# Sreyan88/audio-ssl

Hardware: AMD Instinct MI355X
Metric: upstream clips/sec (1s@16kHz, 64-mel) (higher is better)
Workload: dtype bf16; 1 GPU; delores-m upstream step (log-mel + 2 views + q/k conv encoders + MoCo + 3 Barlow heads + bwd + SGD), 1 s @ 16 kHz, 64 mel, batch 512/GPU, queue 65536; global_batch=512, parallelism=dp1

## Files before the change

### audio-ssl_amd/csrc/bnpool.hip

```cpp
#include "common.h"

namespace {

template <typename T_, bool SQ>
__global__ __launch_bounds__(256) void colstats_kernel(const T_* __restrict__ x, long M, int C, long ld, int rows_per_block,
                                                       double* __restrict__ sum, double* __restrict__ sumsq) {
    __shared__ float red[256][17];
    const int cg = threadIdx.x & 7, r0 = threadIdx.x >> 3;
    const int col0 = blockIdx.y * 64 + cg * 8;
    const long row_begin = (long)blockIdx.x * rows_per_block;
    const long row_end = min(M, row_begin + rows_per_block);
    x += (long)blockIdx.z * M * ld;
    sum += (long)blockIdx.z * C;
    if (SQ) sumsq += (long)blockIdx.z * C;
    float s[8], q[8];
#pragma unroll
    for (int i = 0; i < 8; ++i) { s[i] = 0.f; q[i] = 0.f; }
    if (col0 < C)
        for (long r = row_begin + r0; r < row_end; r += 32) {
            const Vec8<T_> v = Vec8<T_>::load(x + r * ld + col0);
#pragma unroll
            for (int i = 0; i < 8; ++i) { const float f = v.get(i); s[i] += f; if (SQ) q[i] += f * f; }
        }
#pragma unroll
    for (int i = 0; i < 8; ++i) { red[threadIdx.x][i] = s[i]; red[threadIdx.x][8 + i] = q[i]; }
    __syncthreads();
    if (threadIdx.x < 128) {
        const int g = threadIdx.x >> 4, k = threadIdx.x & 15;
        if (SQ || k < 8) {
            double t = 0.0;
            for (int r = 0; r < 32; ++r) t += (double)red[r * 8 + g][k];
            const int c = blockIdx.y * 64 + g * 8 + (k & 7);
            if (c < C) {
                if (k < 8) atomicAdd(&sum[c], t);
                else       atomicAdd(&sumsq[c], t);
            }
        }
    }
}

__global__ void bn_finalize_kernel(const double* __restrict__ sum, const double* __restrict__ sumsq, int groups, double count,
                                   int C, const float* __restrict__ gamma, const float* __restrict__ beta, float* running_mean,
                                   float* running_var, float momentum, float eps, float* scale, float* shift,
                                   float* save_mean, float* save_rstd) {
    const int c = blockIdx.x * blockDim.x + threadIdx.x;
    if (c >= C) return;
    const double g = gamma ? (double)gamma[c] : 1.0, b = beta ? (double)beta[c] : 0.0;
    float rm = running_mean ? running_mean[c] : 0.f, rv = running_mean ? running_var[c] : 0.f;
    for (int k = 0; k < groups; ++k) {
        const int o = k * C + c;
        const double mean = sum[o] / count;
        double var = sumsq[o] / count - mean * mean;
        var = var < 0.0 ? 0.0 : var;
        const double rstd = 1.0 / sqrt(var + (double)eps);
        scale[o] = (float)(g * rstd);
        shift[o] = (float)(b - mean * g * rstd);
        save_mean[o] = (float)mean;
        save_rstd[o] = (float)rstd;
        rm = (1.f - momentum) * rm + momentum * (float)mean;
        const double unb = count > 1.0 ? var * count / (count - 1.0) : var;
        rv = (1.f - momentum) * rv + momentum * (float)unb;
    }
    if (running_mean) { running_mean[c] = rm; running_var[c] = rv; }
}

template <typename TY, typename T_>
__global__ __launch_bounds__(256) void bn_relu_pool_fwd_kernel(const TY* __restrict__ Y, const float* __restrict__ scale,
                                                               const float* __restrict__ shift, T_* __restrict__ P,
                                                               int N, int Ti, int Fi) {
    const int To = Ti / 2, Fo = Fi / 2;
    const long total = (long)N * To * Fo * 8;
    const long idx = (long)blockIdx.x * 256 + threadIdx.x;
    if (idx >= total) return;
    const int c8 = (int)(idx & 7);
    long r = idx >> 3;
    const int fo = (int)(r % Fo); r /= Fo;
    const int to = (int)(r % To);
    const int n = (int)(r / To);
    float sc[8], sh[8], m[8];
#pragma unroll
    for (int i = 0; i < 8; ++i) { sc[i] = scale[c8 * 8 + i]; sh[i] = shift[c8 * 8 + i]; m[i] = 0.f; }
#pragma unroll
    for (int df = 0; df < 2; ++df)
#pragma unroll
        for (int dt = 0; dt < 2; ++dt) {
            const Vec8<TY> v = Vec8<TY>::load(Y + ((((long)n * Ti + 2 * to + dt) * Fi + 2 * fo + df) * 64 + c8 * 8));
#pragma unroll
            for (int i = 0; i < 8; ++i) m[i] = fmaxf(m[i], sc[i] * v.get(i) + sh[i]);
        }
    Vec8<T_> o;
#pragma unroll
    for (int i = 0; i < 8; ++i) o.set(i, m[i]);
    o.store(P + idx * 8);
}

template <typename TY, typename T_>
__global__ __launch_bounds__(256) void bn_relu_pool_train_fwd_kernel(const TY* __restrict__ Y, const double* __restrict__ sum,
                                                                     const double* __restrict__ sumsq, int stat_rep, double count,
                                                                     const float* __restrict__ gamma, const float* __restrict__ beta,
                                                                     float* running_mean, float* running_var, float momentum, float eps,
                                                                     T_* __restrict__ P, float* __restrict__ scale,
                                                                     float* __restrict__ shift, float* __restrict__ save_mean,
                                                                     float* __restrict__ save_rstd, int N, int Ti, int Fi) {
    __shared__ float sc_s[64], sh_s[64];
    if (threadIdx.x < 64) {
        const int c = threadIdx.x;
        const double g = (double)gamma[c], b = (double)beta[c];
        double s1 = 0.0, s2 = 0.0;
        for (int r = 0; r < stat_rep; ++r) { s1 += sum[r * 128 + c]; s2 += sumsq[r * 128 + c]; }
        const double mean = s1 / count;
        double var = s2 / count - mean * mean;
        var = var < 0.0 ? 0.0 : var;
        const double rstd = 1.0 / sqrt(var + (double)eps);
        const float sc = (float)(g * rstd), sh = (float)(b - mean * g * rstd);
        sc_s[c] = sc; sh_s[c] = sh;
        if (blockIdx.x == 0) {
            scale[c] = sc; shift[c] = sh; save_mean[c] = (float)mean; save_rstd[c] = (float)rstd;
            if (running_mean) {
                running_mean[c] = (1.f - momentum) * running_mean[c] + momentum * (float)mean;
                const double unb = count > 1.0 ? var * count / (count - 1.0) : var;
                running_var[c] = (1.f - momentum) * running_var[c] + momentum * (float)unb;
            }
        }
    }
    __syncthreads();
    const int To = Ti / 2, Fo = Fi / 2;
    const long total = (long)N * To * Fo * 8;
    const long idx = (long)blockIdx.x * 256 + threadIdx.x;
    if (idx >= total) return;
    const int c8 = (int)(idx & 7);
    long r = idx >> 3;
    const int fo = (int)(r % Fo); r /= Fo;
    const int to = (int)(r % To);
    const int n = (int)(r / To);
    float sc[8], sh[8], m[8];
#pragma unroll
    for (int i = 0; i < 8; ++i) { sc[i] = sc_s[c8 * 8 + i]; sh[i] = sh_s[c8 * 8 + i]; m[i] = 0.f; }
#pragma unroll
    for (int df = 0; df < 2; ++df)
#pragma unroll
        for (int dt = 0; dt < 2; ++dt) {
            const Vec8<TY> v = Vec8<TY>::load(Y + ((((long)n * Ti + 2 * to + dt) * Fi + 2 * fo + df) * 64 + c8 * 8));
#pragma unroll
            for (int i = 0; i < 8; ++i) m[i] = fmaxf(m[i], sc[i] * v.get(i) + sh[i]);
        }
    Vec8<T_> o;
#pragma unroll
    for (int i = 0; i < 8; ++i) o.set(i, m[i]);
    o.store(P + idx * 8);
}

template <typename T_, typename TO>
__device__ __forceinline__ void tmean_body(const T_* __restrict__ P, TO* __restrict__ xl, int N, int To, int Fo);

template <typename T_, typename TO>
__global__ __launch_bounds__(256) void tmean_fwd_kernel(const T_* __restrict__ P, TO* __restrict__ xl, int N, int To, int Fo) {
    tmean_body<T_, TO>(P, xl, N, To, Fo);
}
struct Tmean3 { const void* P[3]; void* xl[3]; int To[3], Fo[3]; const float* parts; };
template <typename T_, typename TO>
__global__ __launch_bounds__(256) void tmean3_fwd_kernel(Tmean3 a, int N) {
    const int l = blockIdx.z;
    if ((int)blockIdx.x * 64 >= a.Fo[l] * 8) return;
    if (!a.P[l]) {
        if (a.parts && l == 0) {
            const long row = (long)a.Fo[0] * 64, tot = (long)N * row;
            const long i = (long)blockIdx.y * row + blockIdx.x * 512 + threadIdx.x * 2;
            if (blockIdx.x * 512 + threadIdx.x * 2 < row) {
                float2 s = *reinterpret_cast<const float2*>(a.parts + i);
#pragma unroll
                for (int k = 1; k < 4; ++k) {
                    const float2 v = *reinterpret_cast<const float2*>(a.parts + k * tot + i);
                    s.x += v.x; s.y += v.y;
                }
                *reinterpret_cast<float2*>(static_cast<float*>(a.xl[0]) + i) = s;
            }
        }
        return;
    }
    tmean_body<T_, TO>(static_cast<const T_*>(a.P[l]), static_cast<TO*>(a.xl[l]), N, a.To[l], a.Fo[l]);
}

template <typename T_, typename TO>
__device__ __forceinline__ void tmean_body(const T_* __restrict__ P, TO* __restrict__ xl, int N, int To, int Fo) {
    __shared__ float red[4][64][9];
    const int lane = threadIdx.x & 63, w = threadIdx.x >> 6;
    const int nv = Fo * 8;
    const int v = blockIdx.x * 64 + lane;
    const int n = blockIdx.y;
    const bool live = v < nv;
    float s[8];
#pragma unroll
    for (int i = 0; i < 8; ++i) s[i] = 0.f;
    if (live) {
        const T_* p = P + ((long)n * To * nv + v) * 8;
#pragma unroll 4
        for (int t = w; t < To; t += 4) {
            const Vec8<T_> x = Vec8<T_>::load(p + (long)t * nv * 8);
#pragma unroll
            for (int i = 0; i < 8; ++i) s[i] += x.get(i);
        }
    }
#pragma unroll
    for (int i = 0; i < 8; ++i) red[w][lane][i] = s[i];
    __syncthreads();
    if (w == 0 && live) {
        Vec8<TO> o;
        const float inv = 1.f / (float)To;
#pragma unroll
        for (int i = 0; i < 8; ++i) o.set(i, (red[0][lane][i] + red[1][lane][i] + red[2][lane][i] + red[3][lane][i]) * inv);
        o.store(xl + ((long)n * nv + v) * 8);
    }
}

template <typename TY, bool APPLY, typename TG, typename T_>
__global__ __launch_bounds__(256) void bn_relu_pool_bwd_kernel(const TY* __restrict__ Y, const TG* __restrict__ dP,
                                                               const TG* __restrict__ dxl, float inv_To,
                                                               const float* __restrict__ scale, const float* __restrict__ shift,
                                                               const float* __restrict__ mean, const float* __restrict__ rstd,
                                                               float* __restrict__ stat, float inv_count,
                                                               T_* __restrict__ dY, int N, int Ti, int Fi, int fold,
                                                               float* dgamma, float* dbeta) {
    __shared__ float red[256][16];
    __shared__ float folded[128];
    if (APPLY && fold) {
        if (threadIdx.x < 128) {
            float t = 0.f;
            for (int r = 0; r < 32; ++r) t += stat[128 + r * 128 + threadIdx.x];
            folded[threadIdx.x] = t;
        }
        __syncthreads();
        if (blockIdx.x == 0 && threadIdx.x < 64 && dgamma) {
            dbeta[threadIdx.x] += folded[threadIdx.x];
            dgamma[threadIdx.x] += folded[64 + threadIdx.x];
        }
    }
    const int To = Ti / 2, Fo = Fi / 2;
    const int Tq = (Ti + 1) / 2;
    const long total = (long)N * Tq * Fo * 8;
    const long idx = (long)blockIdx.x * 256 + threadIdx.x;
    const bool live = idx < total;
    float db[8], dg[8];
#pragma unroll
    for (int i = 0; i < 8; ++i) { db[i] = 0.f; dg[i] = 0.f; }
    if (live) {
        const int c8 = (int)(idx & 7);
        long r = idx >> 3;
        const int fo = (int)(r % Fo); r /= Fo;
        const int tq = (int)(r % Tq);
        const int n = (int)(r / Tq);
        const bool pooled = tq < To;
        float sc[8], sh[8], mu[8], rs[8], g[8], cb[8], cg[8];
#pragma unroll
        for (int i = 0; i < 8; ++i) {
            const int c = c8 * 8 + i;
            sc[i] = scale[c]; sh[i] = shift[c]; mu[i] = mean[c]; rs[i] = rstd[c]; g[i] = 0.f;
            if (APPLY) { cb[i] = (fold ? folded[c] : stat[c]) * inv_count; cg[i] = (fold ? folded[64 + c] : stat[64 + c]) * inv_count; }
        }
        if (pooled) {
            const Vec8<TG> gp = Vec8<TG>::load(dP + ((((long)n * To + tq) * Fo + fo) * 64 + c8 * 8));
#pragma unroll
            for (int i = 0; i < 8; ++i) g[i] = gp.get(i);
            if (dxl) {
                const Vec8<TG> gx = Vec8<TG>::load(dxl + ((long)n * Fo * 64 + fo * 64 + c8 * 8));
#pragma unroll
                for (int i = 0; i < 8; ++i) g[i] += gx.get(i) * inv_To;
            }
        }
        Vec8<TY> y[4];
        int best[8];
        float bm[8];
#pragma unroll
        for (int i = 0; i < 8; ++i) { best[i] = 0; bm[i] = 0.f; }
#pragma unroll
        for (int p = 0; p < 4; ++p) {
            const int df = p >> 1, dt = p & 1;
            const int t = 2 * tq + dt;
            if (t < Ti) y[p] = Vec8<TY>::load(Y + ((((long)n * Ti + t) * Fi + 2 * fo + df) * 64 + c8 * 8));
            else y[p] = Vec8<TY>::zero();
#pragma unroll
            for (int i = 0; i < 8; ++i) {
                const float a = sc[i] * y[p].get(i) + sh[i];
                if (p == 0 || a > bm[i]) { bm[i] = a; best[i] = p; }
            }
        }
#pragma unroll
        for (int i = 0; i < 8; ++i) {
            const float da = (pooled && bm[i] > 0.f) ? g[i] : 0.f;
            g[i] = da;
            if (!APPLY) {
                float yb = y[0].get(i);
#pragma unroll
                for (int p = 1; p < 4; ++p) yb = best[i] == p ? y[p].get(i) : yb;
                db[i] = da;
                dg[i] = da * (yb - mu[i]) * rs[i];
            }
        }
        if (APPLY) {
#pragma unroll
            for (int p = 0; p < 4; ++p) {
                const int df = p >> 1, dt = p & 1;
                const int t = 2 * tq + dt;
                if (t >= Ti) continue;
                Vec8<T_> o;
#pragma unroll
                for (int i = 0; i < 8; ++i) {
                    const float xhat = (y[p].get(i) - mu[i]) * rs[i];
                    const float da = best[i] == p ? g[i] : 0.f;
                    o.set(i, sc[i] * (da - cb[i] - xhat * cg[i]));
                }
                o.store(dY + ((((long)n * Ti + t) * Fi + 2 * fo + df) * 64 + c8 * 8));
            }
        }
    }
    if (!APPLY) {
#pragma unroll
        for (int i = 0; i < 8; ++i) { red[threadIdx.x][i] = db[i]; red[threadIdx.x][8 + i] = dg[i]; }
        __syncthreads();
        if (threadIdx.x < 128) {
            const int kind = threadIdx.x >> 6, c = threadIdx.x & 63;
            float t = 0.f;
            for (int r = (c >> 3); r < 256; r += 8) t += red[r][kind * 8 + (c & 7)];
            atomicAdd(&stat[128 + (blockIdx.x & 31) * 128 + kind * 64 + c], t);
        }
    }
}

template <typename TP, typename TG>
__global__ __launch_bounds__(256) void bn_pool_bwd_stats_p_kernel(const TP* __restrict__ P, const TG* __restrict__ dP,
                                                                  const TG* __restrict__ dxl, float inv_To,
                                                                  const float* __restrict__ scale, const float* __restrict__ shift,
                                                                  const float* __restrict__ mean, const float* __restrict__ rstd,
                                                                  float* __restrict__ stat, int N, int To, int Fo) {
    __shared__ float red[256][16];
    const long total = (long)N * To * Fo * 8;
    float db[8], dg[8];
#pragma unroll
    for (int i = 0; i < 8; ++i) { db[i] = 0.f; dg[i] = 0.f; }
    const int c8 = threadIdx.x & 7;
    float k1[8], k0[8];
#pragma unroll
    for (int i = 0; i < 8; ++i) {
        const int c = c8 * 8 + i;
        const float sc = scale[c], inv = sc != 0.f ? 1.f / sc : 0.f;
        k1[i] = inv * rstd[c];
        k0[i] = sc != 0.f ? -(shift[c] * inv + mean[c]) * rstd[c] : 0.f;
    }
    for (long idx = (long)blockIdx.x * 256 + threadIdx.x; idx < total; idx += (long)gridDim.x * 256) {
        const long pos = idx >> 3;
        const Vec8<TP> pv = Vec8<TP>::load(P + pos * 64 + c8 * 8);
        const Vec8<TG> gp = Vec8<TG>::load(dP + pos * 64 + c8 * 8);
        float g[8];
#pragma unroll
        for (int i = 0; i < 8; ++i) g[i] = gp.get(i);
        if (dxl) {
            const long n = pos / ((long)To * Fo);
            const int fo = (int)(pos % Fo);
            const Vec8<TG> gx = Vec8<TG>::load(dxl + (n * Fo + fo) * 64 + c8 * 8);
#pragma unroll
            for (int i = 0; i < 8; ++i) g[i] += gx.get(i) * inv_To;
        }
#pragma unroll
        for (int i = 0; i < 8; ++i) {
            const float a = pv.get(i);
            const float da = a > 0.f ? g[i] : 0.f;
            db[i] += da;
            dg[i] += da * (a * k1[i] + k0[i]);
        }
    }
#pragma unroll
    for (int i = 0; i < 8; ++i) { red[threadIdx.x][i] = db[i]; red[threadIdx.x][8 + i] = dg[i]; }
    __syncthreads();
    if (threadIdx.x < 128) {
        const int kind = threadIdx.x >> 6, c = threadIdx.x & 63;
        float t = 0.f;
        for (int r = (c >> 3); r < 256; r += 8) t += red[r][kind * 8 + (c & 7)];
        atomicAdd(&stat[128 + (blockIdx.x & 31) * 128 + kind * 64 + c], t);
    }
}

__global__ void stat_reduce_kernel(float* stat) {
    const int i = threadIdx.x;
    if (i >= 128) return;
    float t = 0.f;
    for (int r = 0; r < 32; ++r) t += stat[128 + r * 128 + i];
    stat[i] = t;
}

template <typename T_>
__global__ __launch_bounds__(256) void im2col_kernel(const T_* __restrict__ X, T_* __restrict__ col, int N, int Ti, int Fi) {
    const long total = (long)N * Ti * Fi * 72;
    const long idx = (long)blockIdx.x * 256 + threadIdx.x;
    if (idx >= total) return;
    const int k8 = (int)(idx % 72);
    long pix = idx / 72;
    const int tap = k8 >> 3, c8 = k8 & 7;
    const int f = (int)(pix % Fi);
    const long r = pix / Fi;
    const int t = (int)(r % Ti);
    const long n = r / Ti;
    const int ff = f + tap / 3 - 1, tt = t + tap % 3 - 1;
    Vec8<T_> v = Vec8<T_>::zero();
    if (ff >= 0 && ff < Fi && tt >= 0 && tt < Ti) v = Vec8<T_>::load(X + (((n * Ti + tt) * Fi + ff) * 64 + c8 * 8));
    v.store(col + idx * 8);
}

template <typename T_>
__global__ void pack_conv_w_kernel(const float* __restrict__ W, T_* __restrict__ Wf, T_* __restrict__ Wd) {
    const int idx = blockIdx.x * 256 + threadIdx.x;
    if (idx >= 64 * 576) return;
    const int row = idx / 576, k = idx % 576, tap = k / 64, c = k % 64;
    Wf[idx] = from_f32<T_>(W[(row * 64 + c) * 9 + tap]);
    Wd[idx] = from_f32<T_>(W[(c * 64 + row) * 9 + (8 - tap)]);
}

template <typename T_>
__global__ void pack_conv_w2_kernel(const float* __restrict__ Wa, T_* __restrict__ Wfa, T_* __restrict__ Wda,
                                    const float* __restrict__ Wb, T_* __restrict__ Wfb, T_* __restrict__ Wdb) {
    const int idx = blockIdx.x * 256 + threadIdx.x;
    if (idx >= 64 * 576) return;
    const float* W = blockIdx.y ? Wb : Wa;
    T_* Wf = blockIdx.y ? Wfb : Wfa;
    T_* Wd = blockIdx.y ? Wdb : Wda;
    const int row = idx / 576, k = idx % 576, tap = k / 64, c = k % 64;
    Wf[idx] = from_f32<T_>(W[(row * 64 + c) * 9 + tap]);
    Wd[idx] = from_f32<T_>(W[(c * 64 + row) * 9 + (8 - tap)]);
}

__global__ void unpack_conv_dw_kernel(const float* __restrict__ dWp, float* __restrict__ dW) {
    const int idx = blockIdx.x * 256 + threadIdx.x;
    if (idx >= 64 * 576) return;
    const int co = idx / 576, k = idx % 576, tap = k / 64, ci = k % 64;
    dW[(co * 64 + ci) * 9 + tap] += dWp[idx];
}

}

#define DISPATCH_T(dtype, CALL_F32, CALL_BF16) do { if ((dtype) == 0) { CALL_F32; } else { CALL_BF16; } } while (0)

extern "C" int audiossl_colstats(int dtype, const void* x, int groups, long M, int C, long ld, int want_sq, double* sum,
                                 double* sumsq, void* stream) {
    ASSL_REQUIRE(x && sum && groups > 0 && M > 0 && C > 0 && (C % 8) == 0 && (ld % 8) == 0);
    ASSL_REQUIRE((dtype == 0 || dtype == 1) && (!want_sq || sumsq));
    hipStream_t s = static_cast<hipStream_t>(stream);
    const size_t nb = sizeof(double) * C * groups;
    if (want_sq && sumsq == sum + (size_t)C * groups) {
        ASSL_ZERO(sum, 2 * nb, s);
    } else {
        ASSL_ZERO(sum, nb, s);
        if (want_sq) ASSL_ZERO(sumsq, nb, s);
    }
    const int slabs = (C + 63) / 64;
    long it = (M * slabs * groups + 32L * 2048 - 1) / (32L * 2048);
    it = it < 1 ? 1 : (it > 128 ? 128 : it);
    const int rpb = 32 * (int)it;
    const dim3 grid(ceil_div(M, rpb), slabs, groups);
#define CS(TT, SQ) hipLaunchKernelGGL((colstats_kernel<TT, SQ>), grid, dim3(256), 0, s, static_cast<const TT*>(x), M, C, ld, rpb, sum, sumsq)
    if (dtype == 0) { if (want_sq) CS(float, true); else CS(float, false); }
    else            { if (want_sq) CS(bf16, true);  else CS(bf16, false); }
#undef CS
    ASSL_LAUNCH_CHECK();
}

extern "C" int audiossl_bn_finalize(const double* sum, const double* sumsq, int groups, double count, int C,
                                    const float* gamma, const float* beta, float* running_mean, float* running_var,
                                    float momentum, float eps, float* scale, float* shift, float* save_mean, float* save_rstd,
                                    void* stream) {
    ASSL_REQUIRE(sum && sumsq && scale && shift && save_mean && save_rstd && C > 0 && count > 0 && groups > 0);
    hipLaunchKernelGGL(bn_finalize_kernel, dim3(ceil_div(C, 256)), dim3(256), 0, static_cast<hipStream_t>(stream), sum, sumsq,
                       groups, count, C, gamma, beta, running_mean, running_var, momentum, eps, scale, shift, save_mean, save_rstd);
    ASSL_LAUNCH_CHECK();
}

extern "C" int audiossl_bn_relu_pool_fwd(int dtype, int ydtype, const void* Y, const float* scale, const float* shift, void* P,
                                         int N, int Ti, int Fi, void* stream) {
    ASSL_REQUIRE(Y && scale && shift && P && N > 0 && Ti >= 2 && Fi >= 2 && (Fi % 2) == 0 && (dtype == 0 || dtype == 1));
    ASSL_REQUIRE(ydtype == 0 || ydtype == dtype);
    const long total = (long)N * (Ti / 2) * (Fi / 2) * 8;
    hipStream_t s = static_cast<hipStream_t>(stream);
#define PF(TY, TO) hipLaunchKernelGGL((bn_relu_pool_fwd_kernel<TY, TO>), dim3(ceil_div(total, 256)), dim3(256), 0, s, \
        static_cast<const TY*>(Y), scale, shift, static_cast<TO*>(P), N, Ti, Fi)
    if (dtype == 0) PF(float, float); else if (ydtype == 0) PF(float, bf16); else PF(bf16, bf16);
#undef PF
    ASSL_LAUNCH_CHECK();
}

extern "C" int audiossl_bn_relu_pool_train_fwd(int dtype, int ydtype, const void* Y, const double* sum, const double* sumsq,
                                               int stat_replicas, double count,
                                               const float* gamma, const float* beta, float* running_mean, float* running_var,
                                               float momentum, float eps, void* P, float* scale, float* shift, float* save_mean,
                                               float* save_rstd, int N, int Ti, int Fi, void* stream) {
    ASSL_REQUIRE(Y && sum && sumsq && gamma && beta && P && scale && shift && save_mean && save_rstd && count > 0.0);
    ASSL_REQUIRE(stat_replicas >= 1 && (stat_replicas == 1 || sumsq == sum + 64));
    ASSL_REQUIRE(N > 0 && Ti >= 2 && Fi >= 2 && (Fi % 2) == 0 && (dtype == 0 || dtype == 1) && (ydtype == 0 || ydtype == dtype));
    const long total = (long)N * (Ti / 2) * (Fi / 2) * 8;
    hipStream_t s = static_cast<hipStream_t>(stream);
#define PF(TY, TO) hipLaunchKernelGGL((bn_relu_pool_train_fwd_kernel<TY, TO>), dim3(ceil_div(total, 256)), dim3(256), 0, s,          \
        static_cast<const TY*>(Y), sum, sumsq, stat_replicas, count, gamma, beta, running_mean, running_var, momentum, eps,      \
        static_cast<TO*>(P),                                                                                                      \
        scale, shift, save_mean, save_rstd, N, Ti, Fi)
    if (dtype == 0) PF(float, float); else if (ydtype == 0) PF(float, bf16); else PF(bf16, bf16);
#undef PF
    ASSL_LAUNCH_CHECK();
}

extern "C" int audiossl_tmean_fwd(int dtype, int out_f32, const void* P, void* xl, int N, int To, int Fo, void* stream) {
    ASSL_REQUIRE(P && xl && N > 0 && To > 0 && Fo > 0 && (dtype == 0 || dtype == 1));
    hipStream_t s = static_cast<hipStream_t>(stream);
#define TM(TI, TO_) hipLaunchKernelGGL((tmean_fwd_kernel<TI, TO_>), dim3(ceil_div(Fo * 8, 64), N), dim3(256), 0, s, \
        static_cast<const TI*>(P), static_cast<TO_*>(xl), N, To, Fo)
    if (dtype == 0) TM(float, float); else if (out_f32) TM(bf16, float); else TM(bf16, bf16);
#undef TM
    ASSL_LAUNCH_CHECK();
}

extern "C" int audiossl_tmean3_fwd(int dtype, int out_f32, const void* P1, void* x1, const float* x1_parts, int To1, int Fo1,
                                   const void* P2, void* x2, int To2, int Fo2, const void* P3, void* x3, int To3, int Fo3, int N,
                                   void* stream) {
    ASSL_REQUIRE(x1 && P2 && x2 && P3 && x3 && N > 0 && To1 > 0 && To2 > 0 && To3 > 0 && Fo1 > 0 && Fo2 > 0 && Fo3 > 0);
    ASSL_REQUIRE((P1 != nullptr) != (x1_parts != nullptr) && (!x1_parts || (out_f32 && dtype == 1)));
    ASSL_REQUIRE(dtype == 0 || dtype == 1);
    hipStream_t s = static_cast<hipStream_t>(stream);
    Tmean3 a{{P1, P2, P3}, {x1, x2, x3}, {To1, To2, To3}, {Fo1, Fo2, Fo3}, x1_parts};
    const int gx = ceil_div(max(Fo1, max(Fo2, Fo3)) * 8, 64);
#define TM3(TI, TO_) hipLaunchKernelGGL((tmean3_fwd_kernel<TI, TO_>), dim3(gx, N, 3), dim3(256), 0, s, a, N)
    if (dtype == 0) TM3(float, float); else if (out_f32) TM3(bf16, float); else TM3(bf16, bf16);
#undef TM3
    ASSL_LAUNCH_CHECK();
}

namespace {
__global__ void add_stat_kernel(const float* __restrict__ stat, float* dgamma, float* dbeta) {
    const int c = threadIdx.x;
    if (c < 64) { dbeta[c] += stat[c]; dgamma[c] += stat[64 + c]; }
}
}

static int bn_relu_pool_bwd_run(int phase, int dtype, int ydtype, int gdtype, const void* Y, const void* P, const void* dP, const void* dxl,
                                const float* scale, const float* shift, const float* mean, const float* rstd, float* stat,
                                const float* gstat, double count, void* dY, float* dgamma, float* dbeta, int N, int Ti, int Fi,
                                void* stream) {
    ASSL_REQUIRE(Y && dP && scale && shift && mean && rstd && stat);
    ASSL_REQUIRE(N > 0 && Ti >= 2 && Fi >= 2 && (Fi % 2) == 0 && (dtype == 0 || dtype == 1) && (gdtype == 0 || gdtype == dtype));
    ASSL_REQUIRE(ydtype == 0 || ydtype == dtype);
    ASSL_REQUIRE(phase == 1 || (dY && dgamma && dbeta));
    hipStream_t s = static_cast<hipStream_t>(stream);
    if (phase != 2) ASSL_ZERO(stat, sizeof(float) * 128 * 33, s);
    const long total = (long)N * ((Ti + 1) / 2) * (Fi / 2) * 8;
    const int grid = ceil_div(total, 256);
    const float inv_To = 1.f / (float)(Ti / 2);
    const float inv_count = (float)(1.0 / (phase == 2 ? count : (double)N * Ti * Fi));
    float* apply_stat = phase == 2 ? const_cast<float*>(gstat) : stat;
    const int fold = phase == 0;
#define BW(TY, AP, TG, TO, ST) hipLaunchKernelGGL((bn_relu_pool_bwd_kernel<TY, AP, TG, TO>), dim3(grid), dim3(256), 0, s,              \
        static_cast<const TY*>(Y), static_cast<const TG*>(dP), static_cast<const TG*>(dxl), inv_To, scale, shift, mean, rstd, ST, \
        inv_count, static_cast<TO*>(dY), N, Ti, Fi, (AP) ? fold : 0, dgamma, dbeta)
#define BWP(TG, TO) hipLaunchKernelGGL((bn_pool_bwd_stats_p_kernel<TO, TG>), dim3(pgrid), dim3(256), 0, s, static_cast<const TO*>(P),          \
        static_cast<const TG*>(dP), static_cast<const TG*>(dxl), inv_To, scale, shift, mean, rstd, stat, N, Ti / 2, Fi / 2)
#define BW2(TY, TG, TO) do { if (phase != 2) { if (P) BWP(TG, TO); else BW(TY, false, TG, TO, stat);                                       \
                                               if (!fold) hipLaunchKernelGGL(stat_reduce_kernel, dim3(1), dim3(128), 0, s, stat); }          \
                             if (phase != 1) BW(TY, true, TG, TO, apply_stat); } while (0)
    const long ptotal = (long)N * (Ti / 2) * (Fi / 2) * 8;
    const int pgrid = (int)min((long)2048, (ptotal + 255) / 256);
    if (dtype == 0) BW2(float, float, float);
    else if (ydtype == 0 && gdtype == 0) BW2(float, float, bf16);
    else if (ydtype == 0) BW2(float, bf16, bf16);
    else if (gdtype == 0) BW2(bf16, float, bf16);
    else BW2(bf16, bf16, bf16);
#undef BW2
#undef BWP
#undef BW
    if (phase == 2) hipLaunchKernelGGL(add_stat_kernel, dim3(1), dim3(64), 0, s, stat, dgamma, dbeta);
    ASSL_LAUNCH_CHECK();
}

extern "C" int audiossl_bn_relu_pool_bwd(int dtype, int ydtype, int gdtype, const void* Y, const void* dP, const void* dxl, const float* scale,
                                         const float* shift, const float* mean, const float* rstd, float* stat, void* dY,
                                         float* dgamma, float* dbeta, int N, int Ti, int Fi, void* stream) {
    return bn_relu_pool_bwd_run(0, dtype, ydtype, gdtype, Y, nullptr, dP, dxl, scale, shift, mean, rstd, stat, nullptr, 0.0, dY, dgamma, dbeta, N,
                                Ti, Fi, stream);
}
extern "C" int audiossl_bn_relu_pool_bwd_p(int dtype, int ydtype, int gdtype, const void* Y, const void* P, const void* dP, const void* dxl,
                                           const float* scale, const float* shift, const float* mean, const float* rstd, float* stat,
                                           void* dY, float* dgamma, float* dbeta, int N, int Ti, int Fi, void* stream) {
    ASSL_REQUIRE(P);
    return bn_relu_pool_bwd_run(0, dtype, ydtype, gdtype, Y, P, dP, dxl, scale, shift, mean, rstd, stat, nullptr, 0.0, dY, dgamma, dbeta, N,
                                Ti, Fi, stream);
}
extern "C" int audiossl_bn_relu_pool_bwd_stats(int dtype, int ydtype, int gdtype, const void* Y, const void* dP, const void* dxl,
                                               const float* scale, const float* shift, const float* mean, const float* rstd,
                                               float* stat, int N, int Ti, int Fi, void* stream) {
    return bn_relu_pool_bwd_run(1, dtype, ydtype, gdtype, Y, nullptr, dP, dxl, scale, shift, mean, rstd, stat, nullptr, 0.0, nullptr, nullptr,
                                nullptr, N, Ti, Fi, stream);
}
extern "C" int audiossl_bn_relu_pool_bwd_apply(int dtype, int ydtype, int gdtype, const void* Y, const void* dP, const void* dxl,
                                               const float* scale, const float* shift, const float* mean, const float* rstd,
                                               float* stat, const float* gstat, double count_global, void* dY, float* dgamma,
                                               float* dbeta, int N, int Ti, int Fi, void* stream) {
    ASSL_REQUIRE(gstat && count_global > 1.0);
    return bn_relu_pool_bwd_run(2, dtype, ydtype, gdtype, Y, nullptr, dP, dxl, scale, shift, mean, rstd, stat, gstat, count_global, dY, dgamma,
                                dbeta, N, Ti, Fi, stream);
}

extern "C" int audiossl_im2col3x3(int dtype, const void* X, void* col, int N, int Ti, int Fi, void* stream) {
    ASSL_REQUIRE(X && col && N > 0 && Ti > 0 && Fi > 0 && (dtype == 0 || dtype == 1));
    const long total = (long)N * Ti * Fi * 72;
    ASSL_REQUIRE((total + 255) / 256 < 2147483647L);
    hipStream_t s = static_cast<hipStream_t>(stream);
    DISPATCH_T(dtype,
        hipLaunchKernelGGL(im2col_kernel<float>, dim3(ceil_div(total, 256)), dim3(256), 0, s, static_cast<const float*>(X),
                           static_cast<float*>(col), N, Ti, Fi),
        hipLaunchKernelGGL(im2col_kernel<bf16>, dim3(ceil_div(total, 256)), dim3(256), 0, s, static_cast<const bf16*>(X),
                           static_cast<bf16*>(col), N, Ti, Fi));
    ASSL_LAUNCH_CHECK();
}

extern "C" int audiossl_pack_conv_w(int dtype, const float* W, void* Wf, void* Wd, void* stream) {
    ASSL_REQUIRE(W && Wf && Wd && (dtype == 0 || dtype == 1));
    hipStream_t s = static_cast<hipStream_t>(stream);
    DISPATCH_T(dtype,
        hipLaunchKernelGGL(pack_conv_w_kernel<float>, dim3(144), dim3(256), 0, s, W, static_cast<float*>(Wf), static_cast<float*>(Wd)),
        hipLaunchKernelGGL(pack_conv_w_kernel<bf16>, dim3(144), dim3(256), 0, s, W, static_cast<bf16*>(Wf), static_cast<bf16*>(Wd)));
    ASSL_LAUNCH_CHECK();
}

extern "C" int audiossl_pack_conv_w2(int dtype, const float* Wa, void* Wfa, void* Wda, const float* Wb, void* Wfb, void* Wdb, void* stream) {
    ASSL_REQUIRE(Wa && Wfa && Wda && Wb && Wfb && Wdb && (dtype == 0 || dtype == 1));
    hipStream_t s = static_cast<hipStream_t>(stream);
    DISPATCH_T(dtype,
        hipLaunchKernelGGL(pack_conv_w2_kernel<float>, dim3(144, 2), dim3(256), 0, s, Wa, static_cast<float*>(Wfa), static_cast<float*>(Wda),
                           Wb, static_cast<float*>(Wfb), static_cast<float*>(Wdb)),
        hipLaunchKernelGGL(pack_conv_w2_kernel<bf16>, dim3(144, 2), dim3(256), 0, s, Wa, static_cast<bf16*>(Wfa), static_cast<bf16*>(Wda),
                           Wb, static_cast<bf16*>(Wfb), static_cast<bf16*>(Wdb)));
    ASSL_LAUNCH_CHECK();
}

extern "C" int audiossl_unpack_conv_dw(const float* dWp, float* dW, void* stream) {
    ASSL_REQUIRE(dWp && dW);
    hipLaunchKernelGGL(unpack_conv_dw_kernel, dim3(144), dim3(256), 0, static_cast<hipStream_t>(stream), dWp, dW);
    ASSL_LAUNCH_CHECK();
}
```

### audio-ssl_amd/csrc/conv.hip

```cpp
#include <cstdlib>
#include "common.h"

namespace {

constexpr int CH = 64, KTOT = 576;
constexpr int WPITCH = KTOT + 8;
constexpr int PIXP = 72;
constexpr int PIXW = 96;

typedef __attribute__((address_space(3))) bf16x4* lds4_t;

struct ConvArgs {
    const bf16* X; const bf16* W; const float* bias; bf16* Y; double* sum; double* sumsq;
    int Ti, rows_total, tiles, out_f32, dbg, stat_rep;
};

template <int FI, int PITCH, int NTH = 256>
struct Halo {
    static constexpr int TT = 256 / FI;
    static constexpr int COLS = FI + 2;
    static constexpr int ELEMS = (TT + 2) * COLS * PITCH;
    static constexpr int NV = ((TT + 2) * FI * 8 + NTH - 1) / NTH;
    static constexpr int NVEC = (TT + 2) * FI * 8;
    Vec8<bf16> r[NV];
    __device__ __forceinline__ void load(const bf16* __restrict__ X, int g0, int rows_total) {
#pragma unroll
        for (int i = 0; i < NV; ++i) {
            const int v = threadIdx.x + i * NTH;
            const int row = v / (FI * 8), rem = v % (FI * 8);
            const int gr = g0 - 1 + row;
            r[i] = (v < NVEC && gr >= 0 && gr < rows_total) ? Vec8<bf16>::load(X + ((long)gr * FI) * CH + rem * 8) : Vec8<bf16>::zero();
        }
    }
    __device__ __forceinline__ void put(bf16* lds) const {
#pragma unroll
        for (int i = 0; i < NV; ++i) {
            const int v = threadIdx.x + i * NTH;
            const int row = v / (FI * 8), rem = v % (FI * 8);
            if (v < NVEC) r[i].store(lds + (row * COLS + (rem >> 3) + 1) * PITCH + (rem & 7) * 8);
        }
    }
    __device__ __forceinline__ static void zero_border(bf16* lds) {
        for (int i = threadIdx.x; i < (TT + 2) * 2 * 8; i += NTH) {
            const int row = i / 16, side = (i >> 3) & 1, c8 = i & 7;
            Vec8<bf16>::zero().store(lds + (row * COLS + side * (FI + 1)) * PITCH + c8 * 8);
        }
    }
};

template <int FI, int NW>
__global__ __launch_bounds__(64 * NW, 1) void conv3x3_kernel(ConvArgs a) {
    using H = Halo<FI, PIXP, 64 * NW>;
    constexpr int RT = 8 / NW;
    constexpr int TT = H::TT, COLS = H::COLS;
    extern __shared__ __attribute__((aligned(16))) char smem[];
    bf16* const wl = reinterpret_cast<bf16*>(smem);
    bf16* const hl = wl + CH * WPITCH;
    float* const red = reinterpret_cast<float*>(hl);

    const int lane = threadIdx.x & 63, wave = threadIdx.x >> 6;
    const int m = lane & 31, h = lane >> 5;
    for (int v = threadIdx.x; v < CH * KTOT / 8; v += 64 * NW) {
        const int row = v / (KTOT / 8), c = v % (KTOT / 8);
        Vec8<bf16>::load(a.W + row * KTOT + c * 8).store(wl + row * WPITCH + c * 8);
    }
    H::zero_border(hl);

    float ssum[2][16], ssq[2][16];
#pragma unroll
    for (int j = 0; j < 2; ++j)
#pragma unroll
        for (int r = 0; r < 16; ++r) { ssum[j][r] = 0.f; ssq[j][r] = 0.f; }
    f32x4 bias4[2][4];
#pragma unroll
    for (int j = 0; j < 2; ++j)
#pragma unroll
        for (int q = 0; q < 4; ++q)
            bias4[j][q] = a.bias ? *reinterpret_cast<const f32x4*>(a.bias + j * 32 + 8 * q + 4 * h) : f32x4{0.f, 0.f, 0.f, 0.f};
    H halo;
    int tile = blockIdx.x;
    if (tile < a.tiles) { halo.load(a.X, tile * TT, a.rows_total); halo.put(hl); }
    __syncthreads();

    for (; tile < a.tiles; tile += gridDim.x) {
        const int g0 = tile * TT;
        const int next = tile + gridDim.x;
        if (next < a.tiles && !(a.dbg & 2)) halo.load(a.X, next * TT, a.rows_total);

        int tl[RT], fcol[RT];
        bool ok[RT][3];
#pragma unroll
        for (int i = 0; i < RT; ++i) {
            const int rt = RT * wave + i;
            tl[i] = FI == 32 ? rt : 2 * rt + (m >> 4);
            fcol[i] = FI == 32 ? m : (m & 15);
            const int g = g0 + tl[i];
            const int ti = g % a.Ti;
#pragma unroll
            for (int dt = 0; dt < 3; ++dt) ok[i][dt] = g < a.rows_total && ti + dt - 1 >= 0 && ti + dt - 1 < a.Ti;
        }
        f32x16 acc[RT][2];
#pragma unroll
        for (int i = 0; i < RT; ++i)
#pragma unroll
            for (int j = 0; j < 2; ++j)
#pragma unroll
                for (int r = 0; r < 16; ++r) acc[i][j][r] = 0.f;

        if (!(a.dbg & 4))
#pragma unroll
        for (int tap = 0; tap < 9; ++tap) {
            const int dt = tap % 3, df = tap / 3;
#pragma unroll
            for (int cc = 0; cc < 4; ++cc) {
                Vec8<bf16> fa[RT], fb[2];
#pragma unroll
                for (int i = 0; i < RT; ++i) {
                    const bf16* p = hl + ((tl[i] + dt) * COLS + fcol[i] + df) * PIXP + cc * 16 + 8 * h;
                    fa[i] = ok[i][dt] ? Vec8<bf16>::load(p) : Vec8<bf16>::zero();
                }
#pragma unroll
                for (int j = 0; j < 2; ++j) fb[j] = Vec8<bf16>::load(wl + (j * 32 + m) * WPITCH + tap * 64 + cc * 16 + 8 * h);
#pragma unroll
                for (int i = 0; i < RT; ++i)
#pragma unroll
                    for (int j = 0; j < 2; ++j)
                        acc[i][j] = __builtin_amdgcn_mfma_f32_32x32x16_bf16(fb[j].v, fa[i].v, acc[i][j], 0, 0, 0);
            }
        }
#pragma unroll
        for (int i = 0; i < RT; ++i) {
            const int g = g0 + tl[i];
            if (g < a.rows_total && !(a.dbg & 1)) {
                const long o = ((long)g * FI + fcol[i]) * CH;
#pragma unroll
                for (int j = 0; j < 2; ++j)
#pragma unroll
                    for (int q = 0; q < 4; ++q) {
                        f32x4 v;
#pragma unroll
                        for (int e = 0; e < 4; ++e) {
                            v[e] = acc[i][j][4 * q + e] + bias4[j][q][e];
                            ssum[j][4 * q + e] += v[e];
                            ssq[j][4 * q + e] += v[e] * v[e];
                        }
                        const int co = j * 32 + 8 * q + 4 * h;
                        if (a.out_f32) *reinterpret_cast<f32x4*>(reinterpret_cast<float*>(a.Y) + o + co) = v;
                        else *reinterpret_cast<bf16x4*>(a.Y + o + co) = bf16x4{(bf16)v[0], (bf16)v[1], (bf16)v[2], (bf16)v[3]};
                    }
            }
        }
        __syncthreads();
        if (next < a.tiles) halo.put(hl);
        __syncthreads();
    }
    if (a.sum) {
#pragma unroll
        for (int j = 0; j < 2; ++j)
#pragma unroll
            for (int r = 0; r < 16; ++r) {
                float s = ssum[j][r], q = ssq[j][r];
#pragma unroll
                for (int o = 16; o > 0; o >>= 1) { s += __shfl_xor(s, o, 64); q += __shfl_xor(q, o, 64); }
                if (m == 0) {
                    const int co = j * 32 + (r & 3) + 8 * (r >> 2) + 4 * h;
                    red[(wave * 64 + co) * 2] = s; red[(wave * 64 + co) * 2 + 1] = q;
                }
            }
        __syncthreads();
        if (threadIdx.x < 128) {
            const int c = threadIdx.x >> 1, k = threadIdx.x & 1;
            double t = 0.0;
#pragma unroll
            for (int w = 0; w < NW; ++w) t += (double)red[(w * 64 + c) * 2 + k];
            const int rep = (blockIdx.x % a.stat_rep) * 128;
            atomicAdd(k == 0 ? &a.sum[rep + c] : &a.sumsq[rep + c], t);
        }
    }
}

template <int FI>
struct WsGeom {
    static constexpr int TT = 256 / FI, COLS = FI + 2, ROWS = TT + 2, SEGS = FI / 8;
    static constexpr int UNITS = ROWS * SEGS;
    static constexpr int UPW = (UNITS + 3) / 4;
    static constexpr int BYTES = ROWS * COLS * 128;
};

template <int FI, bool STATS, bool F32OUT, int PF = 2>
__global__ __launch_bounds__(256, 1) void conv3x3_ws_kernel(ConvArgs a) {
    using G = WsGeom<FI>;
    constexpr int TT = G::TT, COLS = G::COLS;
    typedef __attribute__((address_space(3))) void* lptr_t;
    extern __shared__ __attribute__((aligned(16))) char smem[];
    float* const biasl = reinterpret_cast<float*>(smem + 2 * G::BYTES);
    float* const red = biasl + 64;
    constexpr int OPIX = F32OUT ? 256 : 128;
    char* const stg = reinterpret_cast<char*>(red + 4 * 64 * 2) + (threadIdx.x >> 6) * 64 * OPIX;
    char* const zblk = reinterpret_cast<char*>(red + 4 * 64 * 2) + 4 * 64 * OPIX;
    if (threadIdx.x < 32) *reinterpret_cast<f32x4*>(zblk + threadIdx.x * 16) = f32x4{0.f, 0.f, 0.f, 0.f};

    const int lane = threadIdx.x & 63, wave = __builtin_amdgcn_readfirstlane(threadIdx.x >> 6);
    const int m = lane & 31, h = lane >> 5;
    long* const rts = (!STATS && (a.dbg & 16) && threadIdx.x == 0 && (blockIdx.x == 0 || blockIdx.x == gridDim.x - 1))
                          ? reinterpret_cast<long*>(a.sum) + 64 + (blockIdx.x ? 8 : 0) : nullptr;
    if (rts) rts[0] = __builtin_amdgcn_s_memrealtime();

    {
        bf16* const wl = reinterpret_cast<bf16*>(smem);
        Vec8<bf16> tmp[CH * KTOT / 8 / 256];
#pragma unroll
        for (int k = 0; k < CH * KTOT / 8 / 256; ++k) tmp[k] = Vec8<bf16>::load(a.W + (threadIdx.x + 256 * k) * 8);
#pragma unroll
        for (int k = 0; k < CH * KTOT / 8 / 256; ++k) {
            const int v = threadIdx.x + 256 * k, row = v / (KTOT / 8), c = v % (KTOT / 8);
            tmp[k].store(wl + row * WPITCH + c * 8);
        }
        __syncthreads();
    }
    Vec8<bf16> wr[2][36];
#pragma unroll
    for (int j = 0; j < 2; ++j)
#pragma unroll
        for (int ks = 0; ks < 36; ++ks)
            wr[j][ks] = Vec8<bf16>::load(reinterpret_cast<const bf16*>(smem) + (j * 32 + m) * WPITCH + ks * 16 + 8 * h);
#pragma unroll
    for (int ks = 0; ks < 36; ++ks) {
        asm volatile("" : "+v"(wr[0][ks].v));
        asm volatile("" : "+a"(wr[1][ks].v));
    }

    __syncthreads();
    for (int i = threadIdx.x; i < 2 * G::ROWS * 2 * 8; i += 256) {
        const int b = i / (G::ROWS * 16), r = (i / 16) % G::ROWS, side = (i >> 3) & 1, c8 = i & 7;
        *reinterpret_cast<f32x4*>(smem + b * G::BYTES + (r * COLS + side * (FI + 1)) * 128 + c8 * 16) = f32x4{0.f, 0.f, 0.f, 0.f};
    }
    if (threadIdx.x < 64) biasl[threadIdx.x] = a.bias ? a.bias[threadIdx.x] : 0.f;

    if (rts) { asm volatile("s_waitcnt vmcnt(0)" ::: "memory"); rts[3] = __builtin_amdgcn_s_memrealtime(); }
    const __amdgpu_buffer_rsrc_t rsrc = __builtin_amdgcn_make_buffer_rsrc(const_cast<bf16*>(a.X), 0, (unsigned)((long)a.rows_total * FI * 128), 0x00020000);
    const int pl = lane >> 3, cp = lane & 7;
    const int key0 = ((1 + pl) >> 1) & 7;
    const int voff0 = pl * 128 + ((cp ^ key0) << 4), voff1 = pl * 128 + ((cp ^ key0 ^ 4) << 4);
    auto dma_unit = [&](int g0, char* buf, int i) {
        {
            const int u = wave + 4 * i;
            if (u < G::UNITS) {
                const int row = u / G::SEGS, seg = u % G::SEGS;
                const int gr = g0 - 1 + row;
                const int so = (gr >= 0 && gr < a.rows_total) ? (gr * FI + 8 * seg) * 128 : 0x7FFFFF00;
                __builtin_amdgcn_raw_ptr_buffer_load_lds(rsrc, (lptr_t)(buf + (row * COLS + 1 + 8 * seg) * 128), 16, (seg & 1) ? voff1 : voff0, so, 0, 0);
            }
        }
    };
    auto dma_tile = [&](int g0, char* buf) {
#pragma unroll
        for (int i = 0; i < G::UPW; ++i) dma_unit(g0, buf, i);
    };

    int tl[2];
    const int fcol = FI == 32 ? m : (m & 15);
#pragma unroll
    for (int i = 0; i < 2; ++i) {
        const int rt = 2 * wave + i;
        tl[i] = FI == 32 ? rt : 2 * rt + (m >> 4);
    }
    int hs[3];
#pragma unroll
    for (int df = 0; df < 3; ++df) hs[df] = (h ^ (((fcol + df) >> 1) & 7)) << 4;

    constexpr int NS = F32OUT ? 4 : 8;
    float ssum[NS], ssq[NS];
    if (STATS) {
#pragma unroll
        for (int e = 0; e < NS; ++e) { ssum[e] = 0.f; ssq[e] = 0.f; }
    }

    int tile = blockIdx.x, cur = 0;
    if (tile < a.tiles) dma_tile(tile * TT, smem);
    asm volatile("s_waitcnt vmcnt(0) lgkmcnt(0)" ::: "memory");
    __builtin_amdgcn_s_barrier();

    long* const ts = (!STATS && (a.dbg & 16) && blockIdx.x == 0 && threadIdx.x == 0) ? reinterpret_cast<long*>(a.sum) : nullptr;
    int tsi = 0;
    if (rts) rts[1] = __builtin_amdgcn_s_memrealtime();
    for (; tile < a.tiles; tile += gridDim.x, cur ^= 1) {
        if (ts) ts[tsi++] = __builtin_amdgcn_s_memtime();
        const int g0 = tile * TT;
        const int next = tile + gridDim.x;
        if (next < a.tiles && !(a.dbg & 2)) dma_tile(next * TT, smem + (cur ^ 1) * G::BYTES);
        const char* const hl = smem + cur * G::BYTES;

        int bdt[2][3];
#pragma unroll
        for (int i = 0; i < 2; ++i) {
            const int g = g0 + tl[i];
            const int ti = g % a.Ti;
#pragma unroll
            for (int dt = 0; dt < 3; ++dt) {
                const bool ok = g < a.rows_total && ti + dt - 1 >= 0 && ti + dt - 1 < a.Ti;
                bdt[i][dt] = ok ? (int)(size_t)((lptr_t)const_cast<char*>(hl)) + ((tl[i] + dt) * COLS + fcol) * 128
                                : (int)(size_t)((lptr_t)zblk);
            }
        }
        f32x16 acc[2][2];
#pragma unroll
        for (int j = 0; j < 2; ++j)
#pragma unroll
            for (int q = 0; q < 4; ++q) {
                const f32x4 b4 = *reinterpret_cast<const f32x4*>(biasl + j * 32 + 8 * q + 4 * h);
#pragma unroll
                for (int e = 0; e < 4; ++e) { acc[0][j][4 * q + e] = b4[e]; acc[1][j][4 * q + e] = b4[e]; }
            }

        Vec8<bf16> fa[PF + 1][2];
        auto fetch = [&](int ks, Vec8<bf16> (&f)[2]) {
            const int tap = ks >> 2, cc = ks & 3, dt = tap % 3, df = tap / 3;
#pragma unroll
            for (int i = 0; i < 2; ++i)
                f[i] = Vec8<bf16>::load(reinterpret_cast<const bf16*>((const char*)(lptr_t)(size_t)(bdt[i][dt] + df * 128 + (hs[df] ^ (cc * 32)))));
        };
        if (!(a.dbg & 4)) {
#pragma unroll
        for (int ks = 0; ks < PF; ++ks) fetch(ks, fa[ks]);
#pragma unroll
        for (int ks = 0; ks < 36; ++ks) {
            if (ks + PF < 36) fetch(ks + PF, fa[(ks + PF) % (PF + 1)]);
            __builtin_amdgcn_sched_barrier(0);
            Vec8<bf16> (&f)[2] = fa[ks % (PF + 1)];
#pragma unroll
            for (int i = 0; i < 2; ++i) {
#pragma unroll
                for (int j = 0; j < 2; ++j)
                    acc[i][j] = __builtin_amdgcn_mfma_f32_32x32x16_bf16(wr[j][ks].v, f[i].v, acc[i][j], 0, 0, 0);
            }
            __builtin_amdgcn_sched_barrier(0);
        }
        }
        if (ts) ts[tsi++] = __builtin_amdgcn_s_memtime();
        asm volatile("s_waitcnt vmcnt(0)" ::: "memory");
        if (ts) ts[tsi++] = __builtin_amdgcn_s_memtime();
        if (!(a.dbg & 1)) {
#pragma unroll
            for (int i = 0; i < 2; ++i) {
                char* const st = stg + i * 32 * OPIX;
#pragma unroll
                for (int j = 0; j < 2; ++j)
#pragma unroll
                    for (int q = 0; q < 4; ++q) {
                        const int slot = j * 8 + 2 * q + h;
                        const f32x4 v = f32x4{acc[i][j][4 * q], acc[i][j][4 * q + 1], acc[i][j][4 * q + 2], acc[i][j][4 * q + 3]};
                        if (F32OUT) *reinterpret_cast<f32x4*>(st + m * 256 + ((slot ^ (m & 15)) << 4)) = v;
                        else *reinterpret_cast<bf16x4*>(st + m * 128 + ((slot ^ ((m >> 1) & 15)) << 3)) =
                                 bf16x4{(bf16)v[0], (bf16)v[1], (bf16)v[2], (bf16)v[3]};
                    }
            }
            asm volatile("s_waitcnt lgkmcnt(0)" ::: "memory");
#pragma unroll
            for (int i = 0; i < 2; ++i) {
                const char* const st = stg + i * 32 * OPIX;
                const int grow = g0 + (2 * wave + i) * (32 / FI);
                const int prow_ok = a.rows_total - grow;
                char* const yrow = reinterpret_cast<char*>(a.Y) + (long)grow * FI * 64 * (F32OUT ? 4 : 2);
                if (F32OUT) {
#pragma unroll
                    for (int it = 0; it < 8; ++it) {
                        const int p = it * 4 + (lane >> 4), c = lane & 15;
                        const f32x4 v = *reinterpret_cast<const f32x4*>(st + p * 256 + ((c ^ (p & 15)) << 4));
                        if ((p >> (FI == 32 ? 5 : 4)) < prow_ok) {
                            *reinterpret_cast<f32x4*>(yrow + p * 256 + c * 16) = v;
                            if (STATS) {
#pragma unroll
                                for (int e = 0; e < 4; ++e) { ssum[e] += v[e]; ssq[e] += v[e] * v[e]; }
                            }
                        }
                    }
                } else {
#pragma unroll
                    for (int it = 0; it < 4; ++it) {
                        const int p = it * 8 + (lane >> 3), c = lane & 7, k = (p >> 1) & 15;
                        f32x4 v = *reinterpret_cast<const f32x4*>(st + p * 128 + ((c ^ (k >> 1)) << 4));
                        if (k & 1) v = f32x4{v[2], v[3], v[0], v[1]};
                        if ((p >> (FI == 32 ? 5 : 4)) < prow_ok) {
                            *reinterpret_cast<f32x4*>(yrow + p * 128 + c * 16) = v;
                            if (STATS) {
                                const bf16x8 hv = __builtin_bit_cast(bf16x8, v);
#pragma unroll
                                for (int e = 0; e < 8; ++e) {
                                    const float x = (float)hv[e];
                                    ssum[e] += x; ssq[e] += x * x;
                                }
                            }
                        }
                    }
                }
            }
        }
        if (ts) ts[tsi++] = __builtin_amdgcn_s_memtime();
        asm volatile("s_waitcnt lgkmcnt(0)" ::: "memory");
        __builtin_amdgcn_s_barrier();
    }
    if (rts) rts[2] = __builtin_amdgcn_s_memrealtime();
    if (STATS) {
#pragma unroll
        for (int e = 0; e < NS; ++e) {
            float s = ssum[e], q = ssq[e];
#pragma unroll
            for (int o = 64 / NS; o < 64; o <<= 1) { s += __shfl_xor(s, o, 64); q += __shfl_xor(q, o, 64); }
            if (lane < 64 / NS) {
                const int co = lane * NS + e;
                red[(wave * 64 + co) * 2] = s; red[(wave * 64 + co) * 2 + 1] = q;
            }
        }
        __syncthreads();
        if (threadIdx.x < 128) {
            const int c = threadIdx.x >> 1, k = threadIdx.x & 1;
            double t = 0.0;
#pragma unroll
            for (int w = 0; w < 4; ++w) t += (double)red[(w * 64 + c) * 2 + k];
            const int rep = (blockIdx.x % a.stat_rep) * 128;
            atomicAdd(k == 0 ? &a.sum[rep + c] : &a.sumsq[rep + c], t);
        }
    }
}

__host__ __device__ __forceinline__ int wg_cot(int w, int n) { return n < 8 ? (n & 1) : (w & 1); }
__host__ __device__ __forceinline__ int wg_nt(int w, int n) { return n < 8 ? 4 * w + (n >> 1) : 16 + (w >> 1); }

struct WgradArgs {
    const bf16* dY; const bf16* X; float* dW; int Ti, rows_total, tiles;
    float* partial;
    int dbg;
};

template <int FI, int KG>
__global__ __launch_bounds__(256 * KG, 1) void conv3x3_wgrad_kernel(WgradArgs a) {
    using H = Halo<FI, PIXW, 256 * KG>;
    constexpr int TT = H::TT, COLS = H::COLS;
    constexpr int NTH = 256 * KG;
    constexpr int NVY = 256 * 8 / NTH;
    extern __shared__ __attribute__((aligned(16))) char smem[];
    bf16* const yl = reinterpret_cast<bf16*>(smem);
    bf16* const hl = yl + 256 * PIXW;

    const int lane = threadIdx.x & 63, wave = (threadIdx.x >> 6) & 3, grp = threadIdx.x >> 8;
    const int h = lane >> 5, half = (lane >> 4) & 1, q = (lane & 15) >> 2, p = lane & 3;
    H::zero_border(hl);

    f32x16 acc[9];
#pragma unroll
    for (int n = 0; n < 9; ++n)
#pragma unroll
        for (int r = 0; r < 16; ++r) acc[n][r] = 0.f;

    H halo;
    Vec8<bf16> ry[NVY];
    auto load_y = [&](int g0) {
#pragma unroll
        for (int i = 0; i < NVY; ++i) {
            const int v = threadIdx.x + i * NTH;
            const long pix = (long)g0 * FI + (v >> 3);
            ry[i] = pix < (long)a.rows_total * FI ? Vec8<bf16>::load(a.dY + pix * CH + (v & 7) * 8) : Vec8<bf16>::zero();
        }
    };
    auto put_y = [&]() {
#pragma unroll
        for (int i = 0; i < NVY; ++i) {
            const int v = threadIdx.x + i * NTH;
            ry[i].store(yl + (v >> 3) * PIXW + (v & 7) * 8);
        }
    };
    int tile = blockIdx.x;
    if (tile < a.tiles) { halo.load(a.X, tile * TT, a.rows_total); load_y(tile * TT); halo.put(hl); put_y(); }
    __syncthreads();

    for (; tile < a.tiles; tile += gridDim.x) {
        const int g0 = tile * TT;
        const int next = tile + gridDim.x;
        if (next < a.tiles && !(a.dbg & 2)) { halo.load(a.X, next * TT, a.rows_total); load_y(next * TT); }

#pragma unroll 1
        for (int ks = grp * (16 / KG); ks < (grp + 1) * (16 / KG) && !(a.dbg & 4); ++ks) {
            const int t_local = FI == 32 ? (ks >> 1) : ks;
            const int f0 = FI == 32 ? (ks & 1) * 16 : 0;
            const int g = g0 + t_local;
            if (g >= a.rows_total) break;
            const int ti = g % a.Ti;
            const bool okt[3] = {ti - 1 >= 0, true, ti + 1 < a.Ti};
            bf16x8 fa[2];
#pragma unroll
            for (int c2 = 0; c2 < 2; ++c2) {
                const bf16* ay = yl + (ks * 16 + 8 * h + q) * PIXW + c2 * 32 + 16 * half + 4 * p;
                const bf16x4 a0 = __builtin_amdgcn_ds_read_tr16_b64_v4bf16((lds4_t)ay);
                const bf16x4 a1 = __builtin_amdgcn_ds_read_tr16_b64_v4bf16((lds4_t)(ay + 4 * PIXW));
                fa[c2] = bf16x8{a0[0], a0[1], a0[2], a0[3], a1[0], a1[1], a1[2], a1[3]};
            }
            bf16x8 fb;
#pragma unroll
            for (int n = 0; n < 9; ++n) {
                if (n == 8 || (n & 1) == 0) {
                    const int nt = wg_nt(wave, n), tap = nt >> 1, cih = nt & 1;
                    const int dt = tap % 3, df = tap / 3;
                    const bf16* bx = hl + ((t_local + dt) * COLS + f0 + df + 8 * h + q) * PIXW + cih * 32 + 16 * half + 4 * p;
                    const bf16x4 b0 = __builtin_amdgcn_ds_read_tr16_b64_v4bf16((lds4_t)bx);
                    const bf16x4 b1 = __builtin_amdgcn_ds_read_tr16_b64_v4bf16((lds4_t)(bx + 4 * PIXW));
                    const bf16 z = (bf16)0.f;
                    fb = okt[dt] ? bf16x8{b0[0], b0[1], b0[2], b0[3], b1[0], b1[1], b1[2], b1[3]} : bf16x8{z, z, z, z, z, z, z, z};
                }
                const int c2 = wg_cot(wave, n);
                acc[n] = __builtin_amdgcn_mfma_f32_32x32x16_bf16(c2 ? fa[1] : fa[0], fb, acc[n], 0, 0, 0);
            }
        }
        __syncthreads();
        if (next < a.tiles) { halo.put(hl); put_y(); }
        __syncthreads();
    }
    if (a.partial) {
        if (KG == 2) {
            f32x4* xch = reinterpret_cast<f32x4*>(smem);
            __syncthreads();
            if (grp == 1) {
#pragma unroll
                for (int n = 0; n < 9; ++n)
#pragma unroll
                    for (int r4 = 0; r4 < 4; ++r4)
                        xch[((wave * 9 + n) * 4 + r4) * 64 + lane] = f32x4{acc[n][4 * r4], acc[n][4 * r4 + 1], acc[n][4 * r4 + 2], acc[n][4 * r4 + 3]};
            }
            __syncthreads();
            if (grp == 1) return;
            f32x4* part = reinterpret_cast<f32x4*>(a.partial + (long)blockIdx.x * (CH * KTOT));
#pragma unroll
            for (int n = 0; n < 9; ++n)
#pragma unroll
                for (int r4 = 0; r4 < 4; ++r4) {
                    const f32x4 o = xch[((wave * 9 + n) * 4 + r4) * 64 + lane];
                    part[((wave * 9 + n) * 4 + r4) * 64 + lane] = f32x4{acc[n][4 * r4] + o[0], acc[n][4 * r4 + 1] + o[1], acc[n][4 * r4 + 2] + o[2], acc[n][4 * r4 + 3] + o[3]};
                }
            return;
        }
        f32x4* part = reinterpret_cast<f32x4*>(a.partial + (long)blockIdx.x * (CH * KTOT));
#pragma unroll
        for (int n = 0; n < 9; ++n)
#pragma unroll
            for (int r4 = 0; r4 < 4; ++r4)
                part[((wave * 9 + n) * 4 + r4) * 64 + lane] = f32x4{acc[n][4 * r4], acc[n][4 * r4 + 1], acc[n][4 * r4 + 2], acc[n][4 * r4 + 3]};
        return;
    }
#pragma unroll
    for (int n = 0; n < 9; ++n) {
        const int nt = wg_nt(wave, n), tap = nt >> 1, cih = nt & 1;
        const int col = tap * 64 + cih * 32 + (lane & 31);
#pragma unroll
        for (int r = 0; r < 16; ++r) {
            const int co = wg_cot(wave, n) * 32 + (r & 3) + 8 * (r >> 2) + 4 * h;
            atomicAdd(&a.dW[co * KTOT + col], acc[n][r]);
        }
    }
}

__global__ __launch_bounds__(256) void wgrad_reduce_kernel(const float* __restrict__ partial, int nparts, float* __restrict__ dW) {
    const int i = blockIdx.x * 256 + threadIdx.x;
    if (i >= CH * KTOT) return;
    float s0 = 0.f, s1 = 0.f, s2 = 0.f, s3 = 0.f;
    int w = blockIdx.y;
    const int step = gridDim.y;
    for (; w + 3 * step < nparts; w += 4 * step) {
        s0 += partial[(long)w * (CH * KTOT) + i];
        s1 += partial[(long)(w + step) * (CH * KTOT) + i];
        s2 += partial[(long)(w + 2 * step) * (CH * KTOT) + i];
        s3 += partial[(long)(w + 3 * step) * (CH * KTOT) + i];
    }
    for (; w < nparts; w += step) s0 += partial[(long)w * (CH * KTOT) + i];
    const int e = i & 3, lane = (i >> 2) & 63, r4 = (i >> 8) & 3, wn = i >> 10;
    const int wave = wn / 9, n = wn - wave * 9;
    const int nt = wg_nt(wave, n), tap = nt >> 1, cih = nt & 1;
    const int col = tap * 64 + cih * 32 + (lane & 31);
    const int co = wg_cot(wave, n) * 32 + e + 8 * r4 + 4 * (lane >> 5);
    atomicAdd(&dW[co * KTOT + col], (s0 + s1) + (s2 + s3));
}

template <typename K>
int set_lds(K kernel, size_t bytes) {
    return hipFuncSetAttribute(reinterpret_cast<const void*>(kernel), hipFuncAttributeMaxDynamicSharedMemorySize, (int)bytes) ==
           hipSuccess ? 0 : -1;
}

}

extern "C" int audiossl_conv3x3_fwd(const void* X, const void* W, const float* bias, void* Y, int out_f32, double* sum,
                                    double* sumsq, int stat_replicas, int N, int Ti, int Fi, void* stream) {
    ASSL_REQUIRE(X && W && Y && N > 0 && Ti > 0 && (Fi == 32 || Fi == 16) && (!sum == !sumsq));
    ASSL_REQUIRE(stat_replicas >= 1 && stat_replicas <= 64 && (stat_replicas == 1 || !sum || sumsq == sum + 64));
    if (!ASSL_ALIGNED16(X) || !ASSL_ALIGNED16(W) || !ASSL_ALIGNED16(Y)) return ASSL_EALIGN;
    hipStream_t s = static_cast<hipStream_t>(stream);
#ifdef AUDIOSSL_ABLATE
    static const int conv_dbg = getenv("AUDIOSSL_CONV_DBG") ? atoi(getenv("AUDIOSSL_CONV_DBG")) : 0;
#else
    constexpr int conv_dbg = 0;
#endif
    if (sum && !(conv_dbg & 16)) {
        if (sumsq == sum + 64) {
            ASSL_ZERO(sum, sizeof(double) * 128 * stat_replicas, s);
        } else {
            ASSL_ZERO(sum, sizeof(double) * 64, s);
            ASSL_ZERO(sumsq, sizeof(double) * 64, s);
        }
    }
    const int rows = N * Ti, TT = 256 / Fi, tiles = (rows + TT - 1) / TT;
    ConvArgs a{static_cast<const bf16*>(X), static_cast<const bf16*>(W), bias, static_cast<bf16*>(Y), sum, sumsq, Ti, rows, tiles, out_f32, conv_dbg, stat_replicas};
    const int grid = tiles < 256 ? tiles : 256;
    static const int ws = getenv("AUDIOSSL_CONV_WS") ? atoi(getenv("AUDIOSSL_CONV_WS")) : 1;
    if (ws && (long)rows * Fi * 128 < 0x7FFFFF00L) {
        static bool wattr[8] = {false, false, false, false, false, false, false, false};
#define WS_LAUNCH(FI_, ST_, F32_, SLOT)                                                                    \
    do {                                                                                                  \
        const size_t lds = 2 * WsGeom<FI_>::BYTES + sizeof(float) * (64 + 4 * 64 * 2) + 4 * 64 * (F32_ ? 256 : 128) + 512; \
        if (!wattr[SLOT]) { if (set_lds(conv3x3_ws_kernel<FI_, ST_, F32_>, lds)) return ASSL_ELAUNCH; wattr[SLOT] = true; } \
        hipLaunchKernelGGL((conv3x3_ws_kernel<FI_, ST_, F32_>), dim3(grid), dim3(256), lds, s, a);       \
    } while (0)
        if (Fi == 32) {
            if (sum && !(conv_dbg & 16)) { if (out_f32) WS_LAUNCH(32, true, true, 0); else WS_LAUNCH(32, true, false, 1); }
            else     { if (out_f32) WS_LAUNCH(32, false, true, 2); else WS_LAUNCH(32, false, false, 3); }
        } else {
            if (sum) { if (out_f32) WS_LAUNCH(16, true, true, 4); else WS_LAUNCH(16, true, false, 5); }
            else     { if (out_f32) WS_LAUNCH(16, false, true, 6); else WS_LAUNCH(16, false, false, 7); }
        }
#undef WS_LAUNCH
        ASSL_LAUNCH_CHECK();
    }
    static const int nw = getenv("AUDIOSSL_CONV_WAVES") ? atoi(getenv("AUDIOSSL_CONV_WAVES")) : 8;
    static bool attr[4] = {false, false, false, false};
#define CONV_LAUNCH(FI_, NW_, SLOT)                                                                       \
    do {                                                                                                  \
        const size_t lds = sizeof(bf16) * (CH * WPITCH + Halo<FI_, PIXP>::ELEMS);                         \
        if (!attr[SLOT]) { if (set_lds(conv3x3_kernel<FI_, NW_>, lds)) return ASSL_ELAUNCH; attr[SLOT] = true; } \
        hipLaunchKernelGGL((conv3x3_kernel<FI_, NW_>), dim3(grid), dim3(64 * NW_), lds, s, a);           \
    } while (0)
    if (Fi == 32) { if (nw == 8) CONV_LAUNCH(32, 8, 0); else CONV_LAUNCH(32, 4, 1); }
    else          { if (nw == 8) CONV_LAUNCH(16, 8, 2); else CONV_LAUNCH(16, 4, 3); }
#undef CONV_LAUNCH
    ASSL_LAUNCH_CHECK();
}

extern "C" int audiossl_conv3x3_wgrad(const void* dY, const void* X, float* dWp, float* workspace, long workspace_floats, int N,
                                      int Ti, int Fi, void* stream) {
    ASSL_REQUIRE(dY && X && dWp && N > 0 && Ti > 0 && (Fi == 32 || Fi == 16));
    if (!ASSL_ALIGNED16(X) || !ASSL_ALIGNED16(dY)) return ASSL_EALIGN;
    hipStream_t s = static_cast<hipStream_t>(stream);
    const int rows = N * Ti, TT = 256 / Fi, tiles = (rows + TT - 1) / TT;
    const int grid = tiles < 256 ? tiles : 256;
    const bool two_stage = workspace != nullptr && workspace_floats >= (long)grid * CH * KTOT;
#ifdef AUDIOSSL_ABLATE
    static const int wg_dbg = getenv("AUDIOSSL_CONV_DBG") ? atoi(getenv("AUDIOSSL_CONV_DBG")) : 0;
#else
    constexpr int wg_dbg = 0;
#endif
    WgradArgs a{static_cast<const bf16*>(dY), static_cast<const bf16*>(X), dWp, Ti, rows, tiles, two_stage ? workspace : nullptr, wg_dbg};
    static const int kg_env = getenv("AUDIOSSL_WGRAD_KG") ? atoi(getenv("AUDIOSSL_WGRAD_KG")) : 0;
    const int kg = kg_env ? kg_env : (two_stage ? 2 : 1);
    static bool attr[4] = {false, false, false, false};
#define WGRAD_LAUNCH(FI_, KG_, SLOT)                                                                      \
    do {                                                                                                  \
        const size_t lds = max(sizeof(bf16) * (256 * PIXW + Halo<FI_, PIXW>::ELEMS), (size_t)(KG_ == 2 ? 4 * 9 * 16 * 64 * 4 : 0)); \
        if (!attr[SLOT]) { if (set_lds(conv3x3_wgrad_kernel<FI_, KG_>, lds)) return ASSL_ELAUNCH; attr[SLOT] = true; } \
        hipLaunchKernelGGL((conv3x3_wgrad_kernel<FI_, KG_>), dim3(grid), dim3(256 * KG_), lds, s, a);    \
    } while (0)
    if (Fi == 32) { if (kg == 2) WGRAD_LAUNCH(32, 2, 0); else WGRAD_LAUNCH(32, 1, 1); }
    else          { if (kg == 2) WGRAD_LAUNCH(16, 2, 2); else WGRAD_LAUNCH(16, 1, 3); }
#undef WGRAD_LAUNCH
    if (two_stage)
        hipLaunchKernelGGL(wgrad_reduce_kernel, dim3(CH * KTOT / 256, 8), dim3(256), 0, s, workspace, grid, dWp);
    ASSL_LAUNCH_CHECK();
}
```

### audio-ssl_amd/csrc/conv1.hip

```cpp
#include <cstdlib>
#include "common.h"

namespace {

constexpr int NMOM = 9 + 45;
constexpr int MOM_REPL = 16;

__device__ __forceinline__ int tri(int a, int b) {
    return a * 9 - a * (a - 1) / 2 + (b - a);
}

constexpr int MOM_SLOT = (1 + MOM_REPL) * NMOM;

constexpr int MOM_BAND = 16, MOM_TC = 128;
constexpr int MOM_TILE = (MOM_BAND + 2) * (MOM_TC + 2);
constexpr int MOM_PRE = (MOM_TILE + 255) / 256;
constexpr int MOM_RUN = 32;

typedef __attribute__((ext_vector_type(2))) float f32x2;
constexpr int MOM_NPK = 29;
__device__ __forceinline__ constexpr int mom_pk(int a, int j) {
    int base = 0;
    for (int r = 0; r < a; ++r) base += 5 - r / 2;
    return base + (j - a / 2);
}

struct MomItem { const float* im; int f0, rows, t0, tc; };
__device__ __forceinline__ MomItem mom_item(const float* __restrict__ img, int item, int F, int T, int nband, int nchunk) {
    const int per = nband * nchunk, n = item / per, rem = item - n * per, b = rem / nchunk, ch = rem - b * nchunk;
    MomItem it;
    it.im = img + (long)n * F * T;
    it.f0 = b * MOM_BAND; it.rows = min(MOM_BAND, F - it.f0);
    it.t0 = ch * MOM_TC;  it.tc = min(MOM_TC, T - it.t0);
    return it;
}
struct MomRegs {
    float v[MOM_PRE];
    __device__ __forceinline__ void fetch(const MomItem& it, int F, int T) {
        const int ld = it.tc + 2, total = (it.rows + 2) * ld;
        const float inv = 1.f / (float)ld;
#pragma unroll
        for (int k = 0; k < MOM_PRE; ++k) {
            const int i = threadIdx.x + k * 256;
            const int r = (int)(((float)i + 0.5f) * inv), f = it.f0 - 1 + r, t = it.t0 - 1 + (i - r * ld);
            v[k] = (i < total && f >= 0 && f < F && t >= 0 && t < T) ? it.im[f * T + t] : 0.f;
        }
    }
    __device__ __forceinline__ void put(float* tile, const MomItem& it) const {
        const int total = (it.rows + 2) * (it.tc + 2);
#pragma unroll
        for (int k = 0; k < MOM_PRE; ++k) {
            const int i = threadIdx.x + k * 256;
            if (i < total) tile[i] = v[k];
        }
    }
};

template <int H>
__device__ __forceinline__ void wave_transpose_sum(float (&v)[64], int lane) {
    const bool up = (lane & H) != 0;
#pragma unroll
    for (int k = 0; k < H; ++k) {
        const float send = up ? v[k] : v[k + H], keep = up ? v[k + H] : v[k];
        v[k] = keep + __shfl_xor(send, H, 64);
    }
    if constexpr (H > 1) wave_transpose_sum<H / 2>(v, lane);
}

__global__ __launch_bounds__(256, 4) void conv1_moments_kernel(const float* __restrict__ img_a, const float* __restrict__ img_b,
                                                               double* __restrict__ rep_a, double* __restrict__ rep_b,
                                                               int N, int F, int T, int nband, int nchunk) {
    __shared__ float tile[MOM_TILE];
    __shared__ float sh[4][64];
    const float* __restrict__ img = blockIdx.y ? img_b : img_a;
    double* __restrict__ rep = blockIdx.y ? rep_b : rep_a;
    const int items = N * nband * nchunk;
    f32x2 acc2[MOM_NPK];
#pragma unroll
    for (int i = 0; i < MOM_NPK; ++i) acc2[i] = f32x2{0.f, 0.f};
    MomRegs pre;
    MomItem cur = {}, nx = {};
    int item = blockIdx.x;
    if (item < items) { cur = mom_item(img, item, F, T, nband, nchunk); pre.fetch(cur, F, T); }
    while (item < items) {
        pre.put(tile, cur);
        __syncthreads();
        const int nxt = item + gridDim.x;
        if (nxt < items) { nx = mom_item(img, nxt, F, T, nband, nchunk); pre.fetch(nx, F, T); }
        const int ld = cur.tc + 2, npix = cur.rows * cur.tc;
        const float inv = 1.f / (float)cur.tc;
        for (int p = threadIdx.x; p < npix; p += 256) {
            const int f = (int)(((float)p + 0.5f) * inv), t = p - f * cur.tc;
            const float* c = tile + f * ld + t;
            float x[10];
#pragma unroll
            for (int kh = 0; kh < 3; ++kh)
#pragma unroll
                for (int kw = 0; kw < 3; ++kw) x[kh * 3 + kw] = c[kh * ld + kw];
            x[9] = 1.f;
#pragma unroll
            for (int a = 0; a < 9; ++a) {
                const f32x2 xa = {x[a], x[a]};
#pragma unroll
                for (int j = a / 2; j < 5; ++j)
                    acc2[mom_pk(a, j)] = __builtin_elementwise_fma(xa, f32x2{x[2 * j], x[2 * j + 1]}, acc2[mom_pk(a, j)]);
            }
        }
        __syncthreads();
        item = nxt; cur = nx;
    }
    float acc[64];
#pragma unroll
    for (int i = 0; i < 64; ++i) acc[i] = 0.f;
#pragma unroll
    for (int a = 0; a < 9; ++a) {
        acc[a] = acc2[mom_pk(a, 4)][1];
#pragma unroll
        for (int b = a; b < 9; ++b) acc[9 + tri(a, b)] = acc2[mom_pk(a, b / 2)][b & 1];
    }
    const int lane = threadIdx.x & 63, w = threadIdx.x >> 6;
    wave_transpose_sum<32>(acc, lane);
    sh[w][lane] = acc[0];
    __syncthreads();
    if (threadIdx.x < NMOM) {
        const double v = (double)sh[0][threadIdx.x] + (double)sh[1][threadIdx.x] + (double)sh[2][threadIdx.x] +
                         (double)sh[3][threadIdx.x];
        atomicAdd(&rep[(blockIdx.x & (MOM_REPL - 1)) * NMOM + threadIdx.x], v);
    }
}

struct StemBnLds {
    double tot[NMOM], cov[81], rowv[64 * 9];
    float sc[64], sh[64];
};
struct StemBn {
    double* slot;
    const float *gamma, *beta;
    float *running_mean, *running_var;
    float momentum, eps;
    double count;
    float *scale, *shift, *save_mean, *save_rstd;
};
template <int NT>
__device__ __forceinline__ void stem_bn_finalize(StemBnLds& L, const double* rep, int repl, double* tot_out,
                                                 const float* __restrict__ w, const float* __restrict__ bias, const StemBn& bn,
                                                 bool publish) {
    const double count = bn.count;
    for (int i = threadIdx.x; i < NMOM; i += NT) {
        double t = 0.0;
        for (int r = 0; r < repl; ++r) t += rep[r * NMOM + i];
        L.tot[i] = t;
    }
    __syncthreads();
    if (tot_out)
        for (int i = threadIdx.x; i < NMOM; i += NT) tot_out[i] = L.tot[i];
    for (int i = threadIdx.x; i < 81; i += NT) {
        const int a = i / 9, bb = i - a * 9;
        const double s2 = L.tot[9 + (a <= bb ? tri(a, bb) : tri(bb, a))] / count;
        L.cov[i] = s2 - (L.tot[a] / count) * (L.tot[bb] / count);
    }
    __syncthreads();
    for (int i = threadIdx.x; i < 576; i += NT) {
        const int c = i / 9, a = i - c * 9;
        double r = 0.0;
        for (int bb = 0; bb < 9; ++bb) r += (double)w[c * 9 + bb] * L.cov[a * 9 + bb];
        L.rowv[i] = (double)w[c * 9 + a] * r;
    }
    __syncthreads();
    for (int c = threadIdx.x; c < 64; c += NT) {
        double mean = 0.0, var = 0.0;
        {
#pragma clang fp contract(off)
            for (int k = 0; k < 9; ++k) { mean += (double)w[c * 9 + k] * L.tot[k]; var += L.rowv[c * 9 + k]; }
        }
        mean = mean / count;
        var = var < 0.0 ? 0.0 : var;
        mean += (double)bias[c];
        const double rstd = 1.0 / sqrt(var + (double)bn.eps);
        const float sc = (float)((double)bn.gamma[c] * rstd);
        const float sh = (float)((double)bn.beta[c] - mean * (double)bn.gamma[c] * rstd);
        L.sc[c] = sc;
        L.sh[c] = sh;
        if (publish) {
            bn.scale[c] = sc;
            bn.shift[c] = sh;
            bn.save_mean[c] = (float)mean;
            bn.save_rstd[c] = (float)rstd;
            if (bn.running_mean) {
                bn.running_mean[c] = (1.f - bn.momentum) * bn.running_mean[c] + bn.momentum * (float)mean;
                bn.running_var[c] = (1.f - bn.momentum) * bn.running_var[c] + bn.momentum * (float)(var * count / (count - 1.0));
            }
        }
    }
    __syncthreads();
}

__global__ __launch_bounds__(576) void conv1_finalize_kernel(double* __restrict__ momr, const float* __restrict__ w,
                                                             const float* __restrict__ bias, StemBn bn, int repl) {
    __shared__ StemBnLds L;
    stem_bn_finalize<576>(L, momr, repl, momr, w, bias, bn, true);
}

__device__ __forceinline__ void load_patch(float* patch, const float* __restrict__ img, int n, int tp, int F, int T) {
    const float* im = img + (long)n * F * T;
    for (int i = threadIdx.x; i < (F + 2) * 4; i += 256) {
        const int f = (i >> 2) - 1, t = 2 * tp - 1 + (i & 3);
        patch[i] = (f >= 0 && f < F && t >= 0 && t < T) ? im[f * T + t] : 0.f;
    }
}

struct PatchRegs {
    float v[2];
    __device__ __forceinline__ void fetch(const float* __restrict__ img, int n, int tp, int F, int T) {
        const float* im = img + (long)n * F * T;
#pragma unroll
        for (int j = 0; j < 2; ++j) {
            const int i = threadIdx.x + j * 256;
            const int f = (i >> 2) - 1, t = 2 * tp - 1 + (i & 3);
            v[j] = (i < (F + 2) * 4 && f >= 0 && f < F && t >= 0 && t < T) ? im[f * T + t] : 0.f;
        }
    }
    __device__ __forceinline__ void put(float* patch, int F) const {
#pragma unroll
        for (int j = 0; j < 2; ++j) {
            const int i = threadIdx.x + j * 256;
            if (i < (F + 2) * 4) patch[i] = v[j];
        }
    }
};

__device__ __forceinline__ void conv4(const float* patch, int fp, const float* w, float bias, float* y, float (*x)[4]) {
#pragma unroll
    for (int r = 0; r < 4; ++r) {
        const f32x4 row = *reinterpret_cast<const f32x4*>(patch + (2 * fp + r) * 4);
#pragma unroll
        for (int k = 0; k < 4; ++k) x[r][k] = row[k];
    }
#pragma unroll
    for (int df = 0; df < 2; ++df)
#pragma unroll
        for (int dt = 0; dt < 2; ++dt) {
            float s = bias;
#pragma unroll
            for (int kh = 0; kh < 3; ++kh)
#pragma unroll
                for (int kw = 0; kw < 3; ++kw) s += w[kh * 3 + kw] * x[df + kh][dt + kw];
            y[2 * df + dt] = s;
        }
}

template <typename T_>
__global__ __launch_bounds__(256) void conv1_fwd_kernel(const float* __restrict__ img, const float* __restrict__ w,
                                                        const float* __restrict__ bias, const float* __restrict__ scale,
                                                        const float* __restrict__ shift, T_* __restrict__ out,
                                                        int N, int F, int T) {
    extern __shared__ __attribute__((aligned(16))) float patch[];
    const int lane = threadIdx.x & 63, wv = threadIdx.x >> 6;
    const int To = T / 2, Fo = F / 2;
    float wr[9];
#pragma unroll
    for (int i = 0; i < 9; ++i) wr[i] = w[lane * 9 + i];
    const float b = bias[lane], sc = scale[lane], sh = shift[lane];
    PatchRegs pre;
    int item = blockIdx.x;
    if (item < N * To) { pre.fetch(img, item / To, item % To, F, T); pre.put(patch, F); }
    __syncthreads();
    for (; item < N * To; item += gridDim.x) {
        const int n = item / To, tp = item - n * To;
        const int nxt = item + gridDim.x;
        if (nxt < N * To) pre.fetch(img, nxt / To, nxt % To, F, T);
        for (int fp = wv; fp < Fo; fp += 4) {
            float y[4], x[4][4];
            conv4(patch, fp, wr, b, y, x);
            float m = fmaxf(sc * y[0] + sh, 0.f);
#pragma unroll
            for (int p = 1; p < 4; ++p) m = fmaxf(m, fmaxf(sc * y[p] + sh, 0.f));
            out[(((long)n * To + tp) * Fo + fp) * 64 + lane] = from_f32<T_>(m);
        }
        __syncthreads();
        if (nxt < N * To) pre.put(patch, F);
        __syncthreads();
    }
}

template <typename T_>
__global__ __launch_bounds__(256) void conv1_bwd_kernel(const float* __restrict__ img, const float* __restrict__ w,
                                                        const float* __restrict__ bias, const float* __restrict__ scale,
                                                        const float* __restrict__ shift, const float* __restrict__ mean,
                                                        const float* __restrict__ rstd, const T_* __restrict__ dP,
                                                        const T_* __restrict__ dxl, float inv_To, float* __restrict__ acc,
                                                        int N, int F, int T) {
    extern __shared__ __attribute__((aligned(16))) float patch[];
    __shared__ float red[4][64][11];
    const int lane = threadIdx.x & 63, wv = threadIdx.x >> 6;
    const int To = T / 2, Fo = F / 2;
    float wr[9], G[9];
#pragma unroll
    for (int i = 0; i < 9; ++i) { wr[i] = w[lane * 9 + i]; G[i] = 0.f; }
    const float b = bias[lane], sc = scale[lane], sh = shift[lane], mu = mean[lane], rs = rstd[lane];
    float dbeta = 0.f, dgamma = 0.f;
    PatchRegs pre;
    int item = blockIdx.x;
    if (item < N * To) { pre.fetch(img, item / To, item % To, F, T); pre.put(patch, F); }
    __syncthreads();
    for (; item < N * To; item += gridDim.x) {
        const int n = item / To, tp = item - n * To;
        const int nxt = item + gridDim.x;
        if (nxt < N * To) pre.fetch(img, nxt / To, nxt % To, F, T);
        float gin[8];
#pragma unroll
        for (int i = 0; i < 8; ++i) {
            const int fp = wv + 4 * i;
            gin[i] = 0.f;
            if (fp < Fo) {
                gin[i] = to_f32(dP[(((long)n * To + tp) * Fo + fp) * 64 + lane]);
                if (dxl) gin[i] += to_f32(dxl[(long)n * Fo * 64 + fp * 64 + lane]) * inv_To;
            }
        }
#pragma unroll
        for (int i = 0; i < 8; ++i) {
            const int fp = wv + 4 * i;
            if (fp >= Fo) break;
            float y[4], x[4][4];
            conv4(patch, fp, wr, b, y, x);
            int best = 0;
            float m = sc * y[0] + sh;
#pragma unroll
            for (int p = 1; p < 4; ++p) { const float a = sc * y[p] + sh; if (a > m) { m = a; best = p; } }
            const float g = gin[i];
            const float da = m > 0.f ? g : 0.f;
            const float ybest = best == 0 ? y[0] : best == 1 ? y[1] : best == 2 ? y[2] : y[3];
            dbeta += da;
            dgamma += da * (ybest - mu) * rs;
#pragma unroll
            for (int p = 0; p < 4; ++p) {
                const float dm = (best == p) ? da : 0.f;
                const int df = p >> 1, dt = p & 1;
#pragma unroll
                for (int kh = 0; kh < 3; ++kh)
#pragma unroll
                    for (int kw = 0; kw < 3; ++kw) G[kh * 3 + kw] += dm * x[df + kh][dt + kw];
            }
        }
        __syncthreads();
        if (nxt < N * To) pre.put(patch, F);
        __syncthreads();
    }
#pragma unroll
    for (int i = 0; i < 9; ++i) red[wv][lane][i] = G[i];
    red[wv][lane][9] = dbeta;
    red[wv][lane][10] = dgamma;
    __syncthreads();
    for (int i = threadIdx.x; i < 64 * 11; i += 256) {
        const int c = i / 11, k = i - c * 11;
        atomicAdd(&acc[(blockIdx.x & 31) * 704 + i], red[0][c][k] + red[1][c][k] + red[2][c][k] + red[3][c][k]);
    }
}

__device__ __forceinline__ Vec8<bf16> stem_taps(const float* patch, int f, int dt, int half) {
    Vec8<bf16> a;
    if (half == 0) {
        a.v[0] = (bf16)patch[(f + 0) * 4 + dt + 0]; a.v[1] = (bf16)patch[(f + 0) * 4 + dt + 1]; a.v[2] = (bf16)patch[(f + 0) * 4 + dt + 2];
        a.v[3] = (bf16)patch[(f + 1) * 4 + dt + 0]; a.v[4] = (bf16)patch[(f + 1) * 4 + dt + 1]; a.v[5] = (bf16)patch[(f + 1) * 4 + dt + 2];
        a.v[6] = (bf16)patch[(f + 2) * 4 + dt + 0]; a.v[7] = (bf16)patch[(f + 2) * 4 + dt + 1];
    } else {
        a = Vec8<bf16>::zero();
        a.v[0] = (bf16)patch[(f + 2) * 4 + dt + 2];
    }
    return a;
}
__device__ __forceinline__ Vec8<bf16> stem_weights(const float* w, int c, int half) {
    Vec8<bf16> b = Vec8<bf16>::zero();
    if (half == 0) {
#pragma unroll
        for (int jj = 0; jj < 8; ++jj) b.v[jj] = (bf16)w[c * 9 + jj];
    } else {
        b.v[0] = (bf16)w[c * 9 + 8];
    }
    return b;
}

template <bool TRAIN>
__global__ __launch_bounds__(256) void conv1_fwd_mfma_kernel(const float* __restrict__ img, const float* __restrict__ w,
                                                             const float* __restrict__ bias, const float* __restrict__ scale,
                                                             const float* __restrict__ shift, bf16* __restrict__ out,
                                                             float* __restrict__ xl, int XS, int N, int F, int T, StemBn bn) {
    extern __shared__ __attribute__((aligned(16))) float patch[];
    const int lane = threadIdx.x & 63, wv = threadIdx.x >> 6, half = lane >> 5, l31 = lane & 31;
    const int To = T / 2, Fo = F / 2;
    bf16* const stage = reinterpret_cast<bf16*>(patch + (((F + 2) * 4 + 3) & ~3));
    Vec8<bf16> wb[2];
    float b[2], sc[2], sh[2];
    if (TRAIN) {
        StemBnLds& L = *reinterpret_cast<StemBnLds*>(patch);
        stem_bn_finalize<256>(L, bn.slot + NMOM, MOM_REPL, blockIdx.x == 0 ? bn.slot : nullptr, w, bias, bn, blockIdx.x == 0);
#pragma unroll
        for (int j = 0; j < 2; ++j) { sc[j] = L.sc[32 * j + l31]; sh[j] = L.sh[32 * j + l31]; }
        __syncthreads();
    }
#pragma unroll
    for (int j = 0; j < 2; ++j) {
        const int c = 32 * j + l31;
        wb[j] = stem_weights(w, c, half);
        b[j] = bias[c];
        if (!TRAIN) { sc[j] = scale[c]; sh[j] = shift[c]; }
    }
    const int pp = l31 >> 2, df = (l31 >> 1) & 1, dt = l31 & 1;
    PatchRegs pre;
    int item, step, end;
    if (xl) {
        const int n = blockIdx.x / XS, s4 = blockIdx.x - n * XS, per = (To + XS - 1) / XS;
        item = n * To + s4 * per; step = 1; end = n * To + min(To, (s4 + 1) * per);
    } else {
        item = blockIdx.x; step = gridDim.x; end = N * To;
    }
    float xs[2][2][4];
#pragma unroll
    for (int u = 0; u < 2; ++u)
#pragma unroll
        for (int j = 0; j < 2; ++j)
#pragma unroll
            for (int q = 0; q < 4; ++q) xs[u][j][q] = 0.f;
    if (item < end) { pre.fetch(img, item / To, item % To, F, T); pre.put(patch, F); }
    __syncthreads();
    for (; item < end; item += step) {
        const int n = item / To, tp = item - n * To;
        const int nxt = item + step;
        if (nxt < end) pre.fetch(img, nxt / To, nxt % To, F, T);
#pragma unroll
        for (int u = 0; u < 2; ++u) {
            const int tile = wv + 4 * u;
            if (tile * 8 >= Fo) break;
            const int fp = min(tile * 8 + pp, Fo - 1);
            const Vec8<bf16> a = stem_taps(patch, 2 * fp + df, dt, half);
#pragma unroll
            for (int j = 0; j < 2; ++j) {
                f32x16 acc;
#pragma unroll
                for (int r = 0; r < 16; ++r) acc[r] = 0.f;
                acc = __builtin_amdgcn_mfma_f32_32x32x16_bf16(a.v, wb[j].v, acc, 0, 0, 0);
#pragma unroll
                for (int q = 0; q < 4; ++q) {
                    float m = 0.f;
#pragma unroll
                    for (int r3 = 0; r3 < 4; ++r3) m = fmaxf(m, sc[j] * (acc[4 * q + r3] + b[j]) + sh[j]);
                    const int fpo = tile * 8 + 2 * q + half;
                    if (fpo < Fo) {
                        const bf16 mb = (bf16)m;
                        stage[fpo * 64 + 32 * j + l31] = mb;
                        xs[u][j][q] += (float)mb;
                    }
                }
            }
        }
        __syncthreads();
        if (nxt < end) pre.put(patch, F);
        bf16* o = out + (((long)n * To + tp) * Fo) * 64;
        for (int v = threadIdx.x; v < Fo * 8; v += 256) Vec8<bf16>::load(stage + v * 8).store(o + v * 8);
        __syncthreads();
    }
    if (xl) {
        const int n = blockIdx.x / XS, s4 = blockIdx.x - n * XS;
        const float inv = 1.f / (float)To;
#pragma unroll
        for (int u = 0; u < 2; ++u)
#pragma unroll
            for (int j = 0; j < 2; ++j)
#pragma unroll
                for (int q = 0; q < 4; ++q) {
                    const int fpo = (wv + 4 * u) * 8 + 2 * q + half;
                    if (fpo < Fo) {
                        xl[((long)s4 * N + n) * Fo * 64 + fpo * 64 + 32 * j + l31] = xs[u][j][q] * inv;
                    }
                }
    }
}

template <bool SLAB, typename TP>
__global__ __launch_bounds__(256, 3) void conv1_bwd_mfma_kernel(const float* __restrict__ img, const float* __restrict__ w,
                                                             const float* __restrict__ bias, const float* __restrict__ scale,
                                                             const float* __restrict__ shift, const float* __restrict__ mean,
                                                             const float* __restrict__ rstd, const TP* __restrict__ dP,
                                                             const float* __restrict__ dxl, float inv_To, float* __restrict__ accg,
                                                             int N, int F, int T) {
    extern __shared__ __attribute__((aligned(1024))) float dyn[];
    float* const patch = dyn + (SLAB ? 2 * 2048 : 0);
    __shared__ float red[4][64][11];
    const int lane = threadIdx.x & 63, wv = threadIdx.x >> 6, half = lane >> 5, l31 = lane & 31;
    const int To = T / 2, Fo = F / 2;
    Vec8<bf16> wb[2];
    float b[2], sc[2], sh[2], mu[2], rs[2], dbeta[2] = {0.f, 0.f}, dgamma[2] = {0.f, 0.f};
    f32x16 G[2];
    auto slab_dma = [&](int it, int slot) {
        typedef __attribute__((address_space(1))) const void* gptr_t;
        typedef __attribute__((address_space(3))) void* lptr_t;
        const char* src = reinterpret_cast<const char*>(dP + (long)it * Fo * 64);
        char* dst = reinterpret_cast<char*>(dyn + slot * 2048);
#pragma unroll
        for (int k = 0; k < (int)sizeof(TP) / 2; ++k)
            __builtin_amdgcn_global_load_lds((gptr_t)(src + ((k * 4 + wv) * 64 + lane) * 16),
                                             (lptr_t)(dst + (k * 4 + wv) * 1024), 16, 0, 0);
    };
#pragma unroll
    for (int j = 0; j < 2; ++j) {
        const int c = 32 * j + l31;
        wb[j] = stem_weights(w, c, half);
        b[j] = bias[c]; sc[j] = scale[c]; sh[j] = shift[c]; mu[j] = mean[c]; rs[j] = rstd[c];
#pragma unroll
        for (int r = 0; r < 16; ++r) G[j][r] = 0.f;
    }
    const int pp = l31 >> 2, df = (l31 >> 1) & 1, dt = l31 & 1;
    const int tap = l31, kh = tap / 3, kw = tap - 3 * kh;
    const float dxs = dxl ? inv_To : 0.f;
    auto fetch_dxl = [&](int it, int tile, float (&gx)[2][4]) {
        const int n = it / To;
#pragma unroll
        for (int q = 0; q < 4; ++q) {
            const int fpo = min(tile * 8 + 2 * q + half, Fo - 1);
#pragma unroll
            for (int j = 0; j < 2; ++j) gx[j][q] = dxl ? dxl[(long)n * Fo * 64 + fpo * 64 + 32 * j + l31] : 0.f;
        }
    };
    auto fetch_gp = [&](int it, int tile, int slot, const float (&gx)[2][4], float (&gp)[2][4]) {
        const int n = it / To, tp = it - n * To;
#pragma unroll
        for (int q = 0; q < 4; ++q) {
            const int fpo = tile * 8 + 2 * q + half;
#pragma unroll
            for (int j = 0; j < 2; ++j) {
                float g = 0.f;
                if (fpo < Fo)
                    g = (float)(SLAB ? reinterpret_cast<const TP*>(dyn + slot * 2048)[fpo * 64 + 32 * j + l31]
                                     : dP[(((long)n * To + tp) * Fo + fpo) * 64 + 32 * j + l31]) + gx[j][q] * dxs;
                gp[j][q] = g;
            }
        }
    };
    PatchRegs pre;
    int item = blockIdx.x;
    float gp[2][4], gx[2][4], gxn[2][4];
    if (item < N * To) {
        pre.fetch(img, item / To, item % To, F, T);
        pre.put(patch, F);
        if (SLAB) { fetch_dxl(item, wv, gx); slab_dma(item, 0); }
    }
    __syncthreads();
    int slot = 0;
    for (; item < N * To; item += gridDim.x, slot ^= 1) {
        const int nxt = item + gridDim.x;
        if (nxt < N * To) {
            pre.fetch(img, nxt / To, nxt % To, F, T);
            if (SLAB) { fetch_dxl(nxt, wv, gxn); slab_dma(nxt, slot ^ 1); }
        }
        for (int tile = wv; tile * 8 < Fo; tile += 4) {
            if (!SLAB) fetch_dxl(item, tile, gx);
            fetch_gp(item, tile, slot, gx, gp);
            const int fp = min(tile * 8 + pp, Fo - 1);
            const Vec8<bf16> a = stem_taps(patch, 2 * fp + df, dt, half);
            Vec8<bf16> xh[2];
#pragma unroll
            for (int st = 0; st < 2; ++st) {
                xh[st] = Vec8<bf16>::zero();
                if (tap < 9) {
#pragma unroll
                    for (int jj = 0; jj < 8; ++jj) {
                        const int pix = 16 * st + (jj & 3) + 8 * (jj >> 2) + 4 * half;
                        const int fpx = min(tile * 8 + (pix >> 2), Fo - 1), wp = pix & 3;
                        xh[st].v[jj] = (bf16)patch[(2 * fpx + (wp >> 1) + kh) * 4 + (wp & 1) + kw];
                    }
                }
            }
#pragma unroll
            for (int j = 0; j < 2; ++j) {
                f32x16 acc;
#pragma unroll
                for (int r = 0; r < 16; ++r) acc[r] = 0.f;
                acc = __builtin_amdgcn_mfma_f32_32x32x16_bf16(a.v, wb[j].v, acc, 0, 0, 0);
#pragma unroll
                for (int q = 0; q < 4; ++q) {
                    int best = 0;
                    float ybest = acc[4 * q] + b[j];
                    float m = sc[j] * ybest + sh[j];
#pragma unroll
                    for (int r3 = 1; r3 < 4; ++r3) {
                        const float y = acc[4 * q + r3] + b[j], z = sc[j] * y + sh[j];
                        if (z > m) { m = z; best = r3; ybest = y; }
                    }
                    const float da = m > 0.f ? gp[j][q] : 0.f;
                    dbeta[j] += da;
                    dgamma[j] += da * (ybest - mu[j]) * rs[j];
#pragma unroll
                    for (int r3 = 0; r3 < 4; ++r3) acc[4 * q + r3] = (r3 == best) ? da : 0.f;
                }
#pragma unroll
                for (int st = 0; st < 2; ++st) {
                    Vec8<bf16> gh;
#pragma unroll
                    for (int jj = 0; jj < 8; ++jj) gh.v[jj] = (bf16)acc[8 * st + jj];
                    G[j] = __builtin_amdgcn_mfma_f32_32x32x16_bf16(xh[st].v, gh.v, G[j], 0, 0, 0);
                }
            }
        }
        __syncthreads();
        if (nxt < N * To) pre.put(patch, F);
        if (SLAB) {
#pragma unroll
            for (int j = 0; j < 2; ++j)
#pragma unroll
                for (int q = 0; q < 4; ++q) gx[j][q] = gxn[j][q];
        }
        __syncthreads();
    }
#pragma unroll
    for (int j = 0; j < 2; ++j) {
        const int c = 32 * j + l31;
#pragma unroll
        for (int r = 0; r < 16; ++r) {
            const int t = (r & 3) + 8 * (r >> 2) + 4 * half;
            if (t < 9) red[wv][c][t] = G[j][r];
        }
        const float db = dbeta[j] + __shfl_xor(dbeta[j], 32, 64), dg = dgamma[j] + __shfl_xor(dgamma[j], 32, 64);
        if (half == 0) { red[wv][c][9] = db; red[wv][c][10] = dg; }
    }
    __syncthreads();
    for (int i = threadIdx.x; i < 64 * 11; i += 256) {
        const int c = i / 11, k = i - c * 11;
        atomicAdd(&accg[(blockIdx.x & 31) * 704 + i], red[0][c][k] + red[1][c][k] + red[2][c][k] + red[3][c][k]);
    }
}

__global__ __launch_bounds__(704) void conv1_bwd_finalize_kernel(const float* __restrict__ acc, const double* __restrict__ mom,
                                          const float* __restrict__ w, const float* __restrict__ bias,
                                          const float* __restrict__ gamma, const float* __restrict__ mean,
                                          const float* __restrict__ rstd, double count, float* dW, float* dbias,
                                          float* dgamma, float* dbeta, const float* __restrict__ gstat, float* lstat) {
    __shared__ double s11[704];
    const int i = threadIdx.x;
    if (i < 704) {
        double t = 0.0;
        for (int r = 0; r < 32; ++r) t += (double)acc[r * 704 + i];
        s11[i] = t;
    }
    __syncthreads();
    if (lstat) {
        if (i < 64) { lstat[i] = (float)s11[i * 11 + 9]; lstat[64 + i] = (float)s11[i * 11 + 10]; }
        return;
    }
    if (i < 576) {
        const int c = i / 9, t = i - c * 9;
        const double db = gstat ? (double)gstat[c] : s11[c * 11 + 9], dg = gstat ? (double)gstat[64 + c] : s11[c * 11 + 10];
        const double rs = rstd[c], mu = mean[c], gm = gamma[c];
        double wS2 = 0.0;
        for (int a = 0; a < 9; ++a) wS2 += (double)w[c * 9 + a] * mom[9 + (a <= t ? tri(a, t) : tri(t, a))];
        const double yhat_x = rs * (wS2 + ((double)bias[c] - mu) * mom[t]);
        const double v = gm * rs * (s11[c * 11 + t] - db / count * mom[t] - dg / count * yhat_x);
        dW[c * 9 + t] += (float)v;
    }
    if (i < 64) {
        dgamma[i] += (float)s11[i * 11 + 10];
        dbeta[i] += (float)s11[i * 11 + 9];
    }
    (void)dbias;
}

int launch_moments(const float* img_a, const float* img_b, double* rep_a, double* rep_b, int N, int F, int T, hipStream_t s) {
    const int nband = ceil_div(F, MOM_BAND), nchunk = ceil_div(T, MOM_TC), items = N * nband * nchunk, views = img_b ? 2 : 1;
    static const int resident = getenv("AUDIOSSL_MOM_GRID") ? atoi(getenv("AUDIOSSL_MOM_GRID")) : 1024;
    const int grid = min(items, max(max(resident / views, 1), ceil_div(items, MOM_RUN)));
    hipLaunchKernelGGL(conv1_moments_kernel, dim3(grid, views), dim3(256), 0, s, img_a, img_b, rep_a, rep_b, N, F, T, nband, nchunk);
    return hipGetLastError() == hipSuccess ? ASSL_OK : ASSL_ELAUNCH;
}

bool moments_shape_ok(int N, int F, int T) {
    return N > 0 && F >= 2 && F <= 120 && T >= 2 && (long)N * F * T < 0x7FFFFFFFL - 0x1000000L;
}

}

extern "C" int audiossl_conv1_stats(const float* img, int N, int F, int T, const float* w, const float* bias,
                                    const float* gamma, const float* beta, float* running_mean, float* running_var,
                                    float momentum, float eps, double* mom, float* scale, float* shift,
                                    float* save_mean, float* save_rstd, void* stream) {
    ASSL_REQUIRE(img && w && bias && gamma && beta && mom && scale && shift && save_mean && save_rstd);
    ASSL_REQUIRE(moments_shape_ok(N, F, T));
    hipStream_t s = static_cast<hipStream_t>(stream);
    ASSL_ZERO(mom, sizeof(double) * NMOM * MOM_REPL, s);
    if (launch_moments(img, nullptr, mom, nullptr, N, F, T, s) != ASSL_OK) return ASSL_ELAUNCH;
    const StemBn bn = {nullptr, gamma, beta, running_mean, running_var, momentum, eps, (double)((long)N * F * T),
                       scale, shift, save_mean, save_rstd};
    hipLaunchKernelGGL(conv1_finalize_kernel, dim3(1), dim3(576), 0, s, mom, w, bias, bn, MOM_REPL);
    ASSL_LAUNCH_CHECK();
}

extern "C" int audiossl_conv1_moments_pair(const float* img_a, const float* img_b, int N, int F, int T, double* mom, void* stream) {
    ASSL_REQUIRE(img_a && mom && moments_shape_ok(N, F, T));
    hipStream_t s = static_cast<hipStream_t>(stream);
    ASSL_ZERO(mom, sizeof(double) * MOM_SLOT * (img_b ? 2 : 1), s);
    return launch_moments(img_a, img_b, mom + NMOM, mom + MOM_SLOT + NMOM, N, F, T, s);
}

__global__ void conv1_fold_kernel(double* __restrict__ momr) {
    __shared__ double tot[NMOM];
    const int c = threadIdx.x;
    if (c < NMOM) {
        double t = 0.0;
        for (int r = 0; r < MOM_REPL; ++r) t += momr[r * NMOM + c];
        tot[c] = t;
    }
    __syncthreads();
    if (c < NMOM) momr[c] = tot[c];
}
extern "C" int audiossl_conv1_moments(const float* img, int N, int F, int T, double* mom, void* stream) {
    ASSL_REQUIRE(img && mom && moments_shape_ok(N, F, T));
    hipStream_t s = static_cast<hipStream_t>(stream);
    ASSL_ZERO(mom, sizeof(double) * NMOM * MOM_REPL, s);
    if (launch_moments(img, nullptr, mom, nullptr, N, F, T, s) != ASSL_OK) return ASSL_ELAUNCH;
    hipLaunchKernelGGL(conv1_fold_kernel, dim3(1), dim3(64), 0, s, mom);
    ASSL_LAUNCH_CHECK();
}
extern "C" int audiossl_conv1_finalize(double* mom_totals, const float* w, const float* bias, const float* gamma, const float* beta,
                                       float* running_mean, float* running_var, float momentum, float eps, double count,
                                       float* scale, float* shift, float* save_mean, float* save_rstd, void* stream) {
    ASSL_REQUIRE(mom_totals && w && bias && gamma && beta && scale && shift && save_mean && save_rstd && count > 1.0);
    const StemBn bn = {nullptr, gamma, beta, running_mean, running_var, momentum, eps, count, scale, shift, save_mean, save_rstd};
    hipLaunchKernelGGL(conv1_finalize_kernel, dim3(1), dim3(576), 0, static_cast<hipStream_t>(stream), mom_totals, w, bias, bn, 1);
    ASSL_LAUNCH_CHECK();
}

extern "C" int audiossl_conv1_fwd(int dtype, const float* img, int N, int F, int T, const float* w, const float* bias,
                                  const float* scale, const float* shift, void* out, float* xl, void* stream) {
    ASSL_REQUIRE(img && w && bias && scale && shift && out && N > 0 && F >= 2 && F <= 126 && T >= 2 && (F % 2) == 0);
    ASSL_REQUIRE(dtype == 0 || dtype == 1 || dtype == 2);
    ASSL_REQUIRE(!xl || dtype == 1);
    hipStream_t s = static_cast<hipStream_t>(stream);
    const int xs_split = 4;
    const int grid = xl ? N * xs_split : min(N * (T / 2), 2048);
    size_t lds = sizeof(float) * (F + 2) * 4;
    if (dtype == 1) lds = sizeof(float) * (((F + 2) * 4 + 3) & ~3) + sizeof(bf16) * (F / 2) * 64;
    if (dtype == 0)
        hipLaunchKernelGGL(conv1_fwd_kernel<float>, dim3(grid), dim3(256), lds, s, img, w, bias, scale, shift,
                           static_cast<float*>(out), N, F, T);
    else if (dtype == 2)
        hipLaunchKernelGGL(conv1_fwd_kernel<bf16>, dim3(grid), dim3(256), lds, s, img, w, bias, scale, shift,
                           static_cast<bf16*>(out), N, F, T);
    else
        hipLaunchKernelGGL(conv1_fwd_mfma_kernel<false>, dim3(grid), dim3(256), lds, s, img, w, bias, scale, shift,
                           static_cast<bf16*>(out), xl, xs_split, N, F, T, StemBn{});
    ASSL_LAUNCH_CHECK();
}

extern "C" int audiossl_conv1_fwd_train(const float* img, int N, int F, int T, double* mom, double count, const float* w,
                                        const float* bias, const float* gamma, const float* beta, float* running_mean,
                                        float* running_var, float momentum, float eps, float* scale, float* shift,
                                        float* save_mean, float* save_rstd, void* out, float* xl, void* stream) {
    ASSL_REQUIRE(img && mom && w && bias && gamma && beta && scale && shift && save_mean && save_rstd && out && count > 1.0);
    ASSL_REQUIRE(N > 0 && F >= 2 && F <= 126 && T >= 2 && (F % 2) == 0 && (!running_mean == !running_var));
    hipStream_t s = static_cast<hipStream_t>(stream);
    const int xs_split = 4;
    const int grid = xl ? N * xs_split : min(N * (T / 2), 2048);
    const size_t lds = max(sizeof(float) * (((F + 2) * 4 + 3) & ~3) + sizeof(bf16) * (F / 2) * 64, sizeof(StemBnLds));
    const StemBn bn = {mom, gamma, beta, running_mean, running_var, momentum, eps, count, scale, shift, save_mean, save_rstd};
    hipLaunchKernelGGL(conv1_fwd_mfma_kernel<true>, dim3(grid), dim3(256), lds, s, img, w, bias, (const float*)nullptr,
                       (const float*)nullptr, static_cast<bf16*>(out), xl, xs_split, N, F, T, bn);
    ASSL_LAUNCH_CHECK();
}

static int conv1_bwd_main(int dtype, int conv_dtype, const float* img, int N, int F, int T, const float* w, const float* bias,
                                  const float* gamma, const float* scale, const float* shift, const float* mean,
                                  const float* rstd, const double* mom, const void* dP, const void* dxl, float* acc,
                                  void* stream) {
    ASSL_REQUIRE(img && w && bias && gamma && scale && shift && mean && rstd && mom && dP && acc);
    ASSL_REQUIRE(N > 0 && F >= 2 && F <= 64 && T >= 2 && (F % 2) == 0 && (dtype == 0 || dtype == 1));
    hipStream_t s = static_cast<hipStream_t>(stream);
    ASSL_ZERO(acc, sizeof(float) * 32 * 64 * 11, s);
    static const int bwd_grid = getenv("AUDIOSSL_CONV1_BWD_GRID") ? atoi(getenv("AUDIOSSL_CONV1_BWD_GRID")) : 2048;
    const int grid = min(N * (T / 2), bwd_grid);
    const size_t lds = sizeof(float) * (F + 2) * 4;
    const float inv_To = 1.f / (float)(T / 2);
    if (conv_dtype == 1 && F == 64 && dtype == 0)
        hipLaunchKernelGGL((conv1_bwd_mfma_kernel<true, float>), dim3(grid), dim3(256), lds + 2 * 2048 * sizeof(float), s, img, w, bias, scale,
                           shift, mean, rstd, static_cast<const float*>(dP), static_cast<const float*>(dxl), inv_To, acc, N, F, T);
    else if (conv_dtype == 1 && F == 64)
        hipLaunchKernelGGL((conv1_bwd_mfma_kernel<true, bf16>), dim3(grid), dim3(256), lds + 2 * 2048 * sizeof(float), s, img, w, bias, scale,
                           shift, mean, rstd, static_cast<const bf16*>(dP), static_cast<const float*>(dxl), inv_To, acc, N, F, T);
    else if (conv_dtype == 1 && dtype == 0)
        hipLaunchKernelGGL((conv1_bwd_mfma_kernel<false, float>), dim3(grid), dim3(256), lds, s, img, w, bias, scale, shift, mean, rstd,
                           static_cast<const float*>(dP), static_cast<const float*>(dxl), inv_To, acc, N, F, T);
    else if (conv_dtype == 1)
        hipLaunchKernelGGL((conv1_bwd_mfma_kernel<false, bf16>), dim3(grid), dim3(256), lds, s, img, w, bias, scale, shift, mean, rstd,
                           static_cast<const bf16*>(dP), static_cast<const float*>(dxl), inv_To, acc, N, F, T);
    else if (dtype == 0)
        hipLaunchKernelGGL(conv1_bwd_kernel<float>, dim3(grid), dim3(256), lds, s, img, w, bias, scale, shift, mean, rstd,
                           static_cast<const float*>(dP), static_cast<const float*>(dxl), inv_To, acc, N, F, T);
    else
        hipLaunchKernelGGL(conv1_bwd_kernel<bf16>, dim3(grid), dim3(256), lds, s, img, w, bias, scale, shift, mean, rstd,
                           static_cast<const bf16*>(dP), static_cast<const bf16*>(dxl), inv_To, acc, N, F, T);
    return ASSL_OK;
}

extern "C" int audiossl_conv1_bwd(int dtype, int conv_dtype, const float* img, int N, int F, int T, const float* w, const float* bias,
                                  const float* gamma, const float* scale, const float* shift, const float* mean,
                                  const float* rstd, const double* mom, const void* dP, const void* dxl, float* acc,
                                  float* dW, float* dbias, float* dgamma, float* dbeta, void* stream) {
    ASSL_REQUIRE(dW && dgamma && dbeta);
    const int rc = conv1_bwd_main(dtype, conv_dtype, img, N, F, T, w, bias, gamma, scale, shift, mean, rstd, mom, dP, dxl, acc, stream);
    if (rc != ASSL_OK) return rc;
    hipLaunchKernelGGL(conv1_bwd_finalize_kernel, dim3(1), dim3(704), 0, static_cast<hipStream_t>(stream), acc, mom, w, bias, gamma, mean,
                       rstd, (double)N * F * T, dW, dbias, dgamma, dbeta, (const float*)nullptr, (float*)nullptr);
    ASSL_LAUNCH_CHECK();
}

extern "C" int audiossl_conv1_bwd_sums(int dtype, int conv_dtype, const float* img, int N, int F, int T, const float* w,
                                       const float* bias, const float* gamma, const float* scale, const float* shift,
                                       const float* mean, const float* rstd, const double* mom, const void* dP, const void* dxl,
                                       float* acc, float* lstat, void* stream) {
    ASSL_REQUIRE(lstat);
    const int rc = conv1_bwd_main(dtype, conv_dtype, img, N, F, T, w, bias, gamma, scale, shift, mean, rstd, mom, dP, dxl, acc, stream);
    if (rc != ASSL_OK) return rc;
    hipLaunchKernelGGL(conv1_bwd_finalize_kernel, dim3(1), dim3(704), 0, static_cast<hipStream_t>(stream), acc, mom, w, bias, gamma, mean,
                       rstd, 1.0, (float*)nullptr, (float*)nullptr, (float*)nullptr, (float*)nullptr, (const float*)nullptr, lstat);
    ASSL_LAUNCH_CHECK();
}
extern "C" int audiossl_conv1_bwd_finalize(const float* acc, const double* mom, const float* w, const float* bias, const float* gamma,
                                           const float* mean, const float* rstd, double count_global, const float* gstat, float* dW,
                                           float* dbias, float* dgamma, float* dbeta, void* stream) {
    ASSL_REQUIRE(acc && mom && w && bias && gamma && mean && rstd && gstat && dW && dgamma && dbeta && count_global > 1.0);
    hipLaunchKernelGGL(conv1_bwd_finalize_kernel, dim3(1), dim3(704), 0, static_cast<hipStream_t>(stream), acc, mom, w, bias, gamma, mean,
                       rstd, count_global, dW, dbias, dgamma, dbeta, gstat, (float*)nullptr);
    ASSL_LAUNCH_CHECK();
}
```

### audio-ssl_amd/src/engine.py

```python
import os

import torch

from src import _native as N

import os as _os
_STEM_VALU = _os.environ.get("AUDIOSSL_STEM_VALU") == "1"
BN_MOMENTUM = 0.1
BN_EPS = 1e-5
_BN_FUSED = _os.environ.get("AUDIOSSL_BN_FUSED", "1") != "0"


ONE_STREAM = os.environ.get("AUDIOSSL_ONE_STREAM", "0") == "1"


_CAPTURE_ORIGIN = []


class capture_scope:

    def __enter__(self):
        _CAPTURE_ORIGIN.append(torch.cuda.current_stream())
        return self

    def __exit__(self, *exc):
        _CAPTURE_ORIGIN.pop()
        return False


def fork(side, parent=None, device=None):
    parent = parent if parent is not None else torch.cuda.current_stream(device)
    if _CAPTURE_ORIGIN and parent.cuda_stream != _CAPTURE_ORIGIN[-1].cuda_stream and side.cuda_stream != _CAPTURE_ORIGIN[-1].cuda_stream \
            and os.environ.get("AUDIOSSL_ALLOW_NESTED_FORK", "0") != "1":
        raise RuntimeError("nested stream fork inside a hipGraph capture: a side stream may only be forked from the capture's origin "
                           "stream (a fork from an already forked stream crashed hipStreamEndCapture on ROCm 7.2 - engine.py, "
                           "DESIGN.md section 7); restructure the step or set AUDIOSSL_ALLOW_NESTED_FORK=1 to experiment")
    side.wait_stream(parent)


class SideStream:

    def __init__(self):
        self._streams = {}

    def stream(self, device):
        if ONE_STREAM:
            return torch.cuda.current_stream(device)
        key = str(device)
        if key not in self._streams:
            self._streams[key] = torch.cuda.Stream(device=device)
        return self._streams[key]

    def run(self, device, fn):
        if ONE_STREAM:
            return fn()
        s = self.stream(device)
        fork(s, torch.cuda.current_stream(device))
        with torch.cuda.stream(s):
            return fn()

    def join(self, device):
        if not ONE_STREAM:
            torch.cuda.current_stream(device).wait_stream(self.stream(device))


WGRAD = SideStream()


def _empty(shape, dtype, like=None, device=None):
    return torch.empty(shape, dtype=dtype, device=device if device is not None else like.device)


class ZeroArena:

    def __init__(self, nbytes=8 << 20):
        self.nbytes, self.buf, self.off, self.active = nbytes, None, 0, False

    def step(self, device):
        arena = self

        class _Ctx:
            def __enter__(self_):
                if arena.buf is None or arena.buf.device != device:
                    arena.buf = torch.empty(arena.nbytes, dtype=torch.uint8, device=device)
                arena.off, arena.active = 0, True
                arena.buf.zero_()
                N.call_host("set_prezeroed", 1)

            def __exit__(self_, *exc):
                arena.active = False
                N.call_host("set_prezeroed", 0)
                return False
        return _Ctx()

    def zeros(self, shape, dtype, like=None, device=None):
        dev = device if device is not None else like.device
        if self.active and self.buf.device == dev:
            n = 1
            for d in (shape if isinstance(shape, (tuple, list)) else (shape,)):
                n *= int(d)
            nb = n * torch.empty((), dtype=dtype).element_size()
            if self.off + nb <= self.nbytes:
                t = self.buf[self.off:self.off + nb].view(dtype).view(shape)
                self.off += (nb + 255) // 256 * 256
                return t
        return torch.zeros(shape, dtype=dtype, device=dev)

    def scratch(self, shape, dtype, like):
        return self.zeros(shape, dtype, like=like) if self.active else _empty(shape, dtype, like=like)


ARENA = ZeroArena()


def fast_copy(dst, src):
    n = src.numel()
    if src.dtype == torch.float32 and dst.dtype == torch.float32 and src.is_contiguous() and dst.is_contiguous() and n % 1024 == 0 \
            and n // 1024 < (1 << 31) and src.data_ptr() % 16 == 0 and dst.data_ptr() % 16 == 0:
        N.call("tile_rows", src, dst, n // 1024, n // 1024, 1, 1.0, 1024)
    else:
        dst.copy_(src)
    return dst


def _ksplit(M, Nn, K, target=512):
    tiles = ((M + 127) // 128) * ((Nn + 127) // 128)
    return int(max(1, min(target // max(tiles, 1), (K // 64) // 32)))


def gemm(dtype, ta, tb, M, Nn, K, A, lda, B, ldb, C, ldc, alpha=1.0, bias=None, relu=0, keep=None, ldk=0, keep_scale=1.0,
         gate=None, ldg=0, out_f32=0, atomic=0, ksplit=1, resid=None, ldr=0):
    N.call("gemm", dtype, ta, tb, M, Nn, K, float(alpha), A, lda, B, ldb, C, ldc, bias, relu, keep, ldk, float(keep_scale),
           gate, ldg, out_f32, atomic, ksplit, resid, ldr)


def linear_fwd(dtype, X, W, M, Nout, K, bias=None, relu=0, keep=None, keep_scale=1.0, out=None, out_f32=0):
    if out is None and dtype == N.BF16 and out_f32 and not relu and keep is None and M * Nout <= (1 << 16) and K >= 1024 and K % 512 == 0:
        out = ARENA.zeros((M, Nout), torch.float32, like=X)
        gemm(dtype, 0, 0, M, Nout, K, X, K, W, K, out, Nout, bias=bias, out_f32=1, atomic=1, ksplit=min(8, K // 256))
        return out
    if out is None:
        out = _empty((M, Nout), torch.float32 if (out_f32 or dtype == 0) else torch.bfloat16, like=X)
    gemm(dtype, 0, 0, M, Nout, K, X, K, W, K, out, Nout, bias=bias, relu=relu, keep=keep, ldk=Nout, keep_scale=keep_scale,
         out_f32=out_f32)
    return out


def linear_bwd_w(dtype, dY, X, dW, M, Nout, K, dw_zero=False):
    ks = _ksplit(Nout, K, M)
    atomic = 1 if (ks > 1 or dtype != N.BF16) else (0 if dw_zero else 2)
    gemm(dtype, 1, 1, Nout, K, M, dY, Nout, X, K, dW, K, out_f32=1, atomic=atomic, ksplit=ks)


def linear_bwd_x(dtype, dY, W, M, Nout, K, alpha=1.0, gate=None, out=None, out_f32=0):
    if out is None:
        out = _empty((M, K), torch.float32 if (out_f32 or dtype == N.F32) else torch.bfloat16, like=dY)
    gemm(dtype, 0, 1, M, K, Nout, dY, Nout, W, K, out, K, alpha=alpha, gate=gate, ldg=K, out_f32=out_f32)
    return out


GD = N.F32

HP = False


def set_high_precision(flag):
    global HP
    HP = bool(flag)


SYNC_BN = None


class SyncBN:
    def __init__(self, group=None):
        import torch.distributed as dist
        self.dist, self.group = dist, group
        self.world = dist.get_world_size(group)

    def all_reduce(self, t):
        self.dist.all_reduce(t, group=self.group)
        return t


def set_sync_bn(sync):
    global SYNC_BN
    SYNC_BN = sync if (sync is not None and sync.world > 1) else None


def _ad(dtype):
    return N.F32 if (HP or dtype == N.F32) else dtype


def pooled_dtype(dtype):
    return torch.float32


def center_cast(Y, groups, B):
    C = Y.shape[1]
    yc = _empty((groups * B, C), torch.bfloat16, like=Y)
    cmean = _empty((groups, C), torch.float32, like=Y)
    N.call("center_cast", Y, yc, cmean, groups, B, C)
    return yc, cmean


def colsum_add(dtype, X, M, C, dst, tmp=None):
    tmp = tmp if tmp is not None else ARENA.scratch((C,), torch.float64, X)
    N.call("colstats", dtype, X, 1, M, C, C, 0, tmp, None)
    N.call("add_d2f", tmp, dst, C)


def cast(dtype, src, n=None):
    if dtype == N.F32:
        return src
    out = torch.empty(src.shape, dtype=torch.bfloat16, device=src.device)
    N.call("cast", dtype, src, out, src.numel())
    return out


class EncoderCtx:
    pass


def _bn_train(dtype, Y, M, C, gamma, beta, rm, rv, update_running, groups=1):
    sq = ARENA.scratch((2, groups * C), torch.float64, Y)
    N.call("colstats", dtype, Y, groups, M, C, C, 1, sq[0], sq[1])
    if SYNC_BN is not None:
        SYNC_BN.all_reduce(sq)
        M = M * SYNC_BN.world
    st = _empty((4, groups * C), torch.float32, like=Y)
    N.call("bn_finalize", sq[0], sq[1], groups, float(M), C, gamma, beta, rm if update_running else None,
           rv if update_running else None, BN_MOMENTUM, BN_EPS, st[0], st[1], st[2], st[3])
    return st[0], st[1], st[2], st[3]


def bn_train_apply(dtype, ad, a, M, C, gamma, beta, rm, rv, update_running, groups, relu, out):
    if M <= 1024 and C % 32 == 0 and _BN_FUSED and SYNC_BN is None:
        st = _empty((4, groups * C), torch.float32, like=a)
        N.call("colbn_train_fwd", dtype, ad, a, gamma, beta, rm if update_running else None, rv if update_running else None,
               BN_MOMENTUM, BN_EPS, relu, groups, M, C, out, st[0], st[1], st[2], st[3])
        return st[0], st[1], st[2], st[3]
    st = _bn_train(ad, a, M, C, gamma, beta, rm, rv, update_running, groups)
    N.call("colbn_fwd", dtype, ad, a, st[0], st[1], relu, out, groups, M, C)
    return st


def _bn_eval(like, C, gamma, beta, rm, rv):
    scale, shift = _empty((C,), torch.float32, like=like), _empty((C,), torch.float32, like=like)
    N.call("bn_eval_affine", gamma, beta, rm, rv, BN_EPS, C, scale, shift)
    return scale, shift


_WGRAD_WS = {}


def _wgrad_workspace(device):
    key = device.index if device.index is not None else torch.cuda.current_device()
    ws = _WGRAD_WS.get(key)
    if ws is None:
        ws = _WGRAD_WS[key] = torch.empty(256 * 64 * 576, dtype=torch.float32, device=device)
    return ws


STAT_REPLICAS = 8
LOSS_REPLICAS = 32
_BN_STATS_P = os.environ.get("AUDIOSSL_BN_STATS_P", "1") != "0"
_DP1_BF16 = os.environ.get("AUDIOSSL_DP1_BF16", "1") != "0"


def _conv_block_fwd(dtype, Pin, Nimg, Ti, Fi, W, bias, bn, train, update_running, col, packed=None):
    td = N.torch_dtype(dtype)
    if packed is not None:
        Wf, Wd = packed
    else:
        Wf, Wd = _empty((64, 576), td, like=Pin), _empty((64, 576), td, like=Pin)
        N.call("pack_conv_w", dtype, W, Wf, Wd)
    M = Nimg * Ti * Fi
    ad = _ad(dtype)
    Y = _empty((M, 64), N.torch_dtype(ad), like=Pin)
    gamma, beta, rm, rv = bn
    fused = dtype == N.BF16 and Fi in (16, 32)
    rep = STAT_REPLICAS if (fused and train and SYNC_BN is None) else 1
    sq = ARENA.scratch((rep, 2, 64), torch.float64, Pin) if (fused and train) else None
    if fused:
        N.call("conv3x3_fwd", Pin, Wf, bias, Y, int(ad == N.F32), None if sq is None else sq[0, 0], None if sq is None else sq[0, 1],
               rep, Nimg, Ti, Fi)
    else:
        N.call("im2col3x3", dtype, Pin, col, Nimg, Ti, Fi)
        gemm(dtype, 0, 0, M, 64, 576, col, 576, Wf, 576, Y, 64, bias=bias, out_f32=int(ad == N.F32))
    Pout = _empty((Nimg, Ti // 2, Fi // 2, 64), td, like=Pin)
    if train and fused and SYNC_BN is None:
        st = _empty((4, 64), torch.float32, like=Pin)
        N.call("bn_relu_pool_train_fwd", dtype, ad, Y, sq[0, 0], sq[0, 1], rep, float(M), gamma, beta, rm if update_running else None,
               rv if update_running else None, BN_MOMENTUM, BN_EPS, Pout, st[0], st[1], st[2], st[3], Nimg, Ti, Fi)
        return Y, Pout, (st[0], st[1], st[2], st[3]), Wf, Wd
    if train and fused:
        st = _empty((4, 64), torch.float32, like=Pin)
        sq = sq[0]
        SYNC_BN.all_reduce(sq)
        N.call("bn_finalize", sq[0], sq[1], 1, float(M * SYNC_BN.world), 64, gamma, beta, rm if update_running else None,
               rv if update_running else None, BN_MOMENTUM, BN_EPS, st[0], st[1], st[2], st[3])
        scale, shift, mean, rstd = st[0], st[1], st[2], st[3]
    elif train:
        scale, shift, mean, rstd = _bn_train(ad, Y, M, 64, gamma, beta, rm, rv, update_running)
    else:
        scale, shift = _bn_eval(Y, 64, gamma, beta, rm, rv)
        mean = rstd = None
    N.call("bn_relu_pool_fwd", dtype, ad, Y, scale, shift, Pout, Nimg, Ti, Fi)
    return Y, Pout, (scale, shift, mean, rstd), Wf, Wd


def _col_buffer(dtype, Nimg, T1, F1, like):
    if dtype == N.BF16 and F1 in (16, 32):
        return None
    return _empty((Nimg * T1 * F1, 576), N.torch_dtype(dtype), like=like)


MOM_SLOT = 17 * 54


def stem_fused(dtype, train=True):
    return bool(train) and dtype == N.BF16 and not HP and not _STEM_VALU and SYNC_BN is None


def stem_moments_pair(xa, xb=None):
    Nimg, _, F, T = xa.shape
    assert xb is None or xb.shape == xa.shape
    mom = ARENA.scratch((1 if xb is None else 2, MOM_SLOT), torch.float64, xa)
    N.call("conv1_moments_pair", xa.reshape(Nimg, F, T).contiguous(), None if xb is None else xb.reshape(Nimg, F, T).contiguous(),
           Nimg, F, T, mom)
    return mom


def encoder_forward(P, x, dtype, keep=None, p_drop=0.3, train=True, update_running=True, want_layers=True, Wc=None,
                    layer_out=None, before_fc=None, stem_moments=None):
    Nimg, _, F, T = x.shape
    assert F == 64, "the HIP encoder is built for n_mels = 64 (the reference's only setting)"
    td = N.torch_dtype(dtype)
    c = EncoderCtx()
    c.P = P
    c.dtype, c.N, c.F, c.T, c.train, c.p_drop = dtype, Nimg, F, T, train, p_drop
    img = x.reshape(Nimg, F, T).contiguous()
    c.img = img
    w1 = P["features_1.0.weight"].reshape(64, 9)
    b1 = P["features_1.0.bias"]
    g1, be1 = P["features_1.1.weight"], P["features_1.1.bias"]
    c.stem_mfma = dtype == N.BF16 and not HP and not _STEM_VALU
    fused = stem_fused(dtype, train)
    assert stem_moments is None or fused, "precomputed stem moments are for the fused bf16 training stem only"
    rm1 = rv1 = None
    if train:
        c.sc1, c.sh1, c.mean1, c.rstd1 = (_empty((64,), torch.float32, like=x) for _ in range(4))
        rm1 = P["features_1.1.running_mean"] if update_running else None
        rv1 = P["features_1.1.running_var"] if update_running else None
    if fused:
        c.mom1 = stem_moments if stem_moments is not None else stem_moments_pair(x)[0]
    elif train:
        c.mom1 = ARENA.scratch((16 * 54,), torch.float64, x)
        if SYNC_BN is None:
            N.call("conv1_stats", img, Nimg, F, T, w1, b1, g1, be1, rm1, rv1, BN_MOMENTUM, BN_EPS, c.mom1, c.sc1, c.sh1, c.mean1, c.rstd1)
        else:
            N.call("conv1_moments", img, Nimg, F, T, c.mom1)
            mom_g = SYNC_BN.all_reduce(c.mom1[:54].clone())
            N.call("conv1_finalize", mom_g, w1, b1, g1, be1, rm1, rv1, BN_MOMENTUM, BN_EPS, float(Nimg * F * T * SYNC_BN.world),
                   c.sc1, c.sh1, c.mean1, c.rstd1)
    else:
        c.sc1, c.sh1 = _bn_eval(x, 64, g1, be1, P["features_1.1.running_mean"], P["features_1.1.running_var"])
    T1, F1 = T // 2, F // 2
    c.P1 = _empty((Nimg, T1, F1, 64), td, like=x)
    x1 = x2 = x3 = None
    if want_layers:
        x1, x2, x3 = layer_out if layer_out is not None else (_empty((Nimg, f * 64), td, like=x) for f in (F // 2, F // 4, F // 8))
    x1_fused = c.stem_mfma and x1 is not None and x1.dtype == torch.float32 and x1.is_contiguous()
    x1_parts = _empty((4, Nimg, (F // 2) * 64), torch.float32, like=x) if x1_fused else None
    if fused:
        N.call("conv1_fwd_train", img, Nimg, F, T, c.mom1, float(Nimg * F * T), w1, b1, g1, be1, rm1, rv1, BN_MOMENTUM, BN_EPS,
               c.sc1, c.sh1, c.mean1, c.rstd1, c.P1, x1_parts)
    else:
        N.call("conv1_fwd", dtype if (dtype == N.F32 or c.stem_mfma) else 2, img, Nimg, F, T, w1, b1, c.sc1, c.sh1, c.P1, x1_parts)
    col = _col_buffer(dtype, Nimg, T1, F1, x)
    bn2 = (P["features_2.1.weight"], P["features_2.1.bias"], P["features_2.1.running_mean"], P["features_2.1.running_var"])
    packs = [_empty((64, 576), td, like=x) for _ in range(4)]
    N.call("pack_conv_w2", dtype, P["features_2.0.weight"], packs[0], packs[1], P["features_3.0.weight"], packs[2], packs[3])
    c.Y2, c.P2, c.st2, c.W2f, c.W2d = _conv_block_fwd(dtype, c.P1, Nimg, T1, F1, P["features_2.0.weight"],
                                                       P["features_2.0.bias"], bn2, train, update_running, col, packed=packs[:2])
    T2, F2 = T1 // 2, F1 // 2
    bn3 = (P["features_3.1.weight"], P["features_3.1.bias"], P["features_3.1.running_mean"], P["features_3.1.running_var"])
    c.Y3, c.P3, c.st3, c.W3f, c.W3d = _conv_block_fwd(dtype, c.P2, Nimg, T2, F2, P["features_3.0.weight"],
                                                       P["features_3.0.bias"], bn3, train, update_running, col, packed=packs[2:])
    del col
    T3, F3 = T2 // 2, F2 // 2
    c.dims = (T1, F1, T2, F2, T3, F3)
    if want_layers:
        o32 = int(x1.dtype == torch.float32)
        N.call("tmean3_fwd", dtype, o32, None if x1_fused else c.P1, x1, x1_parts, T1, F1, c.P2, x2, T2, F2, c.P3, x3, T3, F3, Nimg)
    d = P["fc.0.weight"].shape[0]
    kin = F3 * 64
    M = Nimg * T3
    c.d, c.kin, c.M = d, kin, M
    if before_fc is not None:
        before_fc()
    if Wc is not None:
        c.fw1, c.fw2 = Wc["fc.0.weight"], Wc["fc.3.weight"]
    else:
        c.fw1, c.fw2 = cast(dtype, P["fc.0.weight"]), cast(dtype, P["fc.3.weight"])
    if keep is not None and not isinstance(keep, torch.Tensor) and (dtype != N.BF16 or not train):
        keep = keep.materialise()
    c.keep = keep if train else None
    scale = 1.0 / (1.0 - p_drop) if c.keep is not None else 1.0
    if c.keep is not None and not isinstance(c.keep, torch.Tensor):
        vk = c.keep
        c.H1 = torch.empty(M, d, dtype=torch.bfloat16, device=c.P3.device)
        N.call("gemm_dropout", 0, 0, M, d, kin, 1.0, c.P3, kin, c.fw1, kin, c.H1, d, P["fc.0.bias"], 1, vk.seed, float(vk.p), vk.counter,
               float(scale))
    else:
        c.H1 = linear_fwd(dtype, c.P3, c.fw1, M, d, kin, bias=P["fc.0.bias"], relu=1, keep=c.keep, keep_scale=scale)
    c.H2 = linear_fwd(dtype, c.H1, c.fw2, M, d, d, bias=P["fc.3.bias"], relu=1)
    return x1, x2, x3, c.H2.view(Nimg, T3, d), c


def _conv_block_bwd(dtype, Y, dP, dxl, st, Nimg, Ti, Fi, Pin, Wd, G_w, G_gamma, G_beta, need_dx, col, keep, dx_bf16=False, Pout=None):
    td = N.torch_dtype(dtype)
    scale, shift, mean, rstd = st
    M = Nimg * Ti * Fi
    dY = torch.empty((M, 64), dtype=td, device=Y.device)
    stat = ARENA.scratch((33 * 128,), torch.float32, Y)
    yd = N.F32 if Y.dtype == torch.float32 else dtype
    if SYNC_BN is None and Pout is not None and _BN_STATS_P and Pout.dtype == td:
        N.call("bn_relu_pool_bwd_p", dtype, yd, GD, Y, Pout, dP, dxl, scale, shift, mean, rstd, stat, dY, G_gamma, G_beta, Nimg, Ti, Fi)
    elif SYNC_BN is None:
        N.call("bn_relu_pool_bwd", dtype, yd, GD, Y, dP, dxl, scale, shift, mean, rstd, stat, dY, G_gamma, G_beta, Nimg, Ti, Fi)
    else:
        N.call("bn_relu_pool_bwd_stats", dtype, yd, GD, Y, dP, dxl, scale, shift, mean, rstd, stat, Nimg, Ti, Fi)
        gstat = SYNC_BN.all_reduce(stat[:128].clone())
        N.call("bn_relu_pool_bwd_apply", dtype, yd, GD, Y, dP, dxl, scale, shift, mean, rstd, stat, gstat, float(M * SYNC_BN.world), dY,
               G_gamma, G_beta, Nimg, Ti, Fi)
    fused = dtype == N.BF16 and Fi in (16, 32)
    if fused:
        def wg():
            dWp = ARENA.zeros((64, 576), torch.float32, device=Y.device)
            ws = _wgrad_workspace(Y.device)
            N.call("conv3x3_wgrad", dY, Pin, dWp, ws, ws.numel(), Nimg, Ti, Fi)
            N.call("unpack_conv_dw", dWp, G_w)
            return dWp
        keep.append((dY, WGRAD.run(Y.device, wg)))
    else:
        dWp = ARENA.zeros((64, 576), torch.float32, device=Y.device)
        N.call("im2col3x3", dtype, Pin, col, Nimg, Ti, Fi)
        gemm(dtype, 1, 1, 64, 576, M, dY, 64, col, 576, dWp, 576, out_f32=1, atomic=1, ksplit=_ksplit(64, 576, M, 1024))
        N.call("unpack_conv_dw", dWp, G_w)
    if not need_dx:
        return None
    dx_bf16 = dx_bf16 and fused
    dPin = _empty((Nimg, Ti, Fi, 64), torch.bfloat16 if dx_bf16 else torch.float32, like=Y)
    if fused:
        N.call("conv3x3_fwd", dY, Wd, None, dPin, 0 if dx_bf16 else 1, None, None, 1, Nimg, Ti, Fi)
    else:
        N.call("im2col3x3", dtype, dY, col, Nimg, Ti, Fi)
        gemm(dtype, 0, 0, M, 64, 576, col, 576, Wd, 576, dPin, 64)
    return dPin


def encoder_backward(c, G, dA2=None, dH2=None, dx1=None, dx2=None, dx3=None, dx_late=None, grads_zero=False):
    dtype, Nimg, M, d, kin = c.dtype, c.N, c.M, c.d, c.kin
    T1, F1, T2, F2, T3, F3 = c.dims
    td = N.torch_dtype(dtype)
    assert c.train, "backward needs a train-mode forward (batch statistics)"
    if dA2 is None:
        dA2 = _empty((M, d), td, like=c.H2)
        N.call("relu_bwd", dtype, dH2.contiguous(), c.H2, dA2, M * d)
    dev = c.H2.device
    def w2():
        linear_bwd_w(dtype, dA2, c.H1, G["fc.3.weight"], M, d, d, dw_zero=grads_zero)
        colsum_add(dtype, dA2, M, d, G["fc.3.bias"])
    WGRAD.run(dev, w2)
    scale = 1.0 / (1.0 - c.p_drop) if c.keep is not None else 1.0
    dA1 = linear_bwd_x(dtype, dA2, c.fw2, M, d, d, alpha=scale, gate=c.H1)
    def w1():
        linear_bwd_w(dtype, dA1, c.P3, G["fc.0.weight"], M, d, kin, dw_zero=grads_zero)
        colsum_add(dtype, dA1, M, d, G["fc.0.bias"])
    WGRAD.run(dev, w1)
    dP3 = linear_bwd_x(dtype, dA1, c.fw1, M, d, kin, out_f32=1)
    if dx_late is not None:
        dx1, dx2, dx3 = dx_late()
    col = _col_buffer(dtype, Nimg, T1, F1, c.H2)
    keep = []
    dP2 = _conv_block_bwd(dtype, c.Y3, dP3, dx3, c.st3, Nimg, T2, F2, c.P2, c.W3d, G["features_3.0.weight"],
                          G["features_3.1.weight"], G["features_3.1.bias"], True, col, keep, Pout=c.P3)
    dP1 = _conv_block_bwd(dtype, c.Y2, dP2, dx2, c.st2, Nimg, T1, F1, c.P1, c.W2d, G["features_2.0.weight"],
                          G["features_2.1.weight"], G["features_2.1.bias"], True, col, keep, dx_bf16=bool(c.stem_mfma) and _DP1_BF16,
                          Pout=c.P2)
    gd1 = N.BF16 if dP1.dtype == torch.bfloat16 else GD
    acc = ARENA.scratch((32 * 64 * 11,), torch.float32, c.H2)
    P = c.P
    w1, b1, g1 = P["features_1.0.weight"].reshape(64, 9), P["features_1.0.bias"], P["features_1.1.weight"]
    gw, gb = G["features_1.0.weight"].view(64, 9), G["features_1.0.bias"]
    if SYNC_BN is None:
        N.call("conv1_bwd", gd1, int(c.stem_mfma), c.img, Nimg, c.F, c.T, w1, b1, g1, c.sc1, c.sh1, c.mean1, c.rstd1, c.mom1, dP1, dx1,
               acc, gw, gb, G["features_1.1.weight"], G["features_1.1.bias"])
    else:
        lstat = _empty((128,), torch.float32, like=c.H2)
        N.call("conv1_bwd_sums", gd1, int(c.stem_mfma), c.img, Nimg, c.F, c.T, w1, b1, g1, c.sc1, c.sh1, c.mean1, c.rstd1, c.mom1, dP1,
               dx1, acc, lstat)
        gstat = SYNC_BN.all_reduce(lstat.clone())
        N.call("conv1_bwd_finalize", acc, c.mom1, w1, b1, g1, c.mean1, c.rstd1, float(Nimg * c.F * c.T * SYNC_BN.world), gstat, gw, gb,
               G["features_1.1.weight"], G["features_1.1.bias"])
    WGRAD.join(dev)


def maxmean_forward(dtype, H2, out=None):
    Nimg, T3, d = H2.shape
    y = out if out is not None else _empty((Nimg, d), N.torch_dtype(dtype), like=H2)
    arg = _empty((Nimg, d), torch.uint8, like=H2)
    N.call("maxmean_fwd", dtype, int(y.dtype == torch.float32), H2, y, arg, Nimg, T3, d)
    return y, arg


def maxmean_backward(dtype, dy, arg, H2):
    Nimg, T3, d = H2.shape
    dA2 = _empty((Nimg * T3, d), N.torch_dtype(dtype), like=H2)
    N.call("maxmean_bwd", dtype, GD, dy, arg, H2, dA2, Nimg, T3, d)
    return dA2


class ProjCtx:
    pass


def projector_forward(PP, Y, dtype, groups, B, update_running=True, Wc=None):
    kin = Y.shape[1]
    c = ProjCtx()
    c.dtype, c.B, c.groups, c.kin, c.y = dtype, B, groups, kin, Y
    W = Wc if Wc is not None else tuple(cast(dtype, PP[f"projector.{i}.weight"]) for i in (0, 3, 6))
    c.W = W
    D = W[0].shape[0]
    c.D = D
    M = groups * B

    def bn(a, prefix, affine, relu, out, adt=None):
        g = PP[prefix + ".weight"] if affine else None
        b = PP[prefix + ".bias"] if affine else None
        return bn_train_apply(dtype, ad if adt is None else adt, a, B, D, g, b, PP[prefix + ".running_mean"], PP[prefix + ".running_var"],
                              update_running, groups, relu, out)
    td = N.torch_dtype(dtype)
    ad = _ad(dtype)
    c.ad = ad
    o32 = int(ad == N.F32)
    c.cmean = None
    if dtype == N.BF16 and Y.dtype == torch.float32 and not HP and B <= 1024 and kin % 32 == 0 and SYNC_BN is None:
        c.y_hi, c.cmean = center_cast(Y, groups, B)
        c.y_lo = None
        c.a1 = linear_fwd(dtype, c.y_hi, W[0], M, D, kin, out_f32=o32)
    elif dtype == N.BF16 and Y.dtype == torch.float32:
        c.y_hi, c.y_lo = _empty((M, kin), td, like=Y), _empty((M, kin), td, like=Y)
        N.call("split_bf16", Y, c.y_hi, c.y_lo, M * kin)
        c.a1 = torch.zeros(M, D, dtype=torch.float32, device=Y.device)
        gemm(dtype, 0, 0, M, D, kin, c.y_hi, kin, W[0], kin, c.a1, D, out_f32=1, atomic=1)
        gemm(dtype, 0, 0, M, D, kin, c.y_lo, kin, W[0], kin, c.a1, D, out_f32=1, atomic=1)
    else:
        c.y_hi, c.y_lo = Y, None
        c.a1 = linear_fwd(dtype, Y, W[0], M, D, kin, out_f32=o32)
    c.ad1 = N.F32 if c.a1.dtype == torch.float32 else ad
    c.h1 = _empty((M, D), td, like=Y)
    c.st1 = bn(c.a1, "projector.1", True, 1, c.h1, adt=c.ad1)
    if c.cmean is not None and update_running:
        N.call("shift_running_mean", W[0], c.cmean, PP["projector.1.running_mean"], D, kin, groups, BN_MOMENTUM)
    c.a2 = linear_fwd(dtype, c.h1, W[1], M, D, D, out_f32=o32)
    c.h2 = _empty((M, D), td, like=Y)
    c.st2 = bn(c.a2, "projector.4", True, 1, c.h2)
    c.z = linear_fwd(dtype, c.h2, W[2], M, D, D, out_f32=o32)
    c.zn = _empty((M, D), td, like=Y)
    c.st0 = bn(c.z, "bn", False, 0, c.zn)
    return c.zn, c


def projector_backward(c, PP, G, dzn, dy_rows=None):
    dtype, B, D, kin, groups = c.dtype, c.B, c.D, c.kin, c.groups
    M = groups * B
    td = N.torch_dtype(dtype)

    def bn_bwd(a, dh, st, relu, da, g_gamma, g_beta, adt=None):
        adt = c.ad if adt is None else adt
        """BatchNorm1d(train) backward per group (view).  SyncBatchNorm (`extras/delores-s/main.py:79` converts every BatchNorm of
        the model, the projector's included): the two means of the backward are over the GLOBAL batch of the view - this rank's
        sums are all-reduced between the statistics pass and the apply pass; the parameter gradients stay this rank's own sums
        (the data-parallel gradient all-reduce adds the ranks up afterwards)."""
        t = ARENA.scratch((2 * groups * D,), torch.float64, dzn)
        if SYNC_BN is None:
            N.call("colbn_bwd", dtype, adt, GD, a, dh, *st, relu, groups, B, D, t, da, g_gamma, g_beta)
            return
        N.call("colbn_bwd_stats", dtype, adt, GD, a, dh, *st, relu, groups, B, D, t)
        tg = SYNC_BN.all_reduce(t.clone())
        N.call("colbn_bwd_apply", dtype, adt, GD, a, dh, *st, relu, groups, B, D, tg, float(B * SYNC_BN.world), da)
        if g_gamma is not None:
            for g in range(groups):
                N.call("add_d2f", t[g * D:(g + 1) * D], g_beta, D)
                N.call("add_d2f", t[(groups + g) * D:(groups + g + 1) * D], g_gamma, D)
    dz = _empty((M, D), td, like=c.zn)
    bn_bwd(c.z, dzn, c.st0, 0, dz, None, None)
    linear_bwd_w(dtype, dz, c.h2, G["projector.6.weight"], M, D, D)
    dh2 = linear_bwd_x(dtype, dz, c.W[2], M, D, D, out_f32=1)
    da2 = _empty((M, D), td, like=c.zn)
    bn_bwd(c.a2, dh2, c.st2, 1, da2, G["projector.4.weight"], G["projector.4.bias"])
    linear_bwd_w(dtype, da2, c.h1, G["projector.3.weight"], M, D, D)
    dh1 = linear_bwd_x(dtype, da2, c.W[1], M, D, D, out_f32=1)
    da1 = _empty((M, D), td, like=c.zn)
    bn_bwd(c.a1, dh1, c.st1, 1, da1, G["projector.1.weight"], G["projector.1.bias"], adt=c.ad1)
    linear_bwd_w(dtype, da1, c.y_hi, G["projector.0.weight"], M, D, kin)
    if c.y_lo is not None:
        linear_bwd_w(dtype, da1, c.y_lo, G["projector.0.weight"], M, D, kin)
    rows = M if dy_rows is None else dy_rows
    if rows == 0:
        return None
    return linear_bwd_x(dtype, da1, c.W[0], rows, D, kin, out_f32=1)


def barlow_forward_backward(PP, G, Y, dtype, lambd, scale_loss, loss_out, need_dy1=True, need_dy2=True,
                            update_running=True, all_reduce=None, global_batch=None, backward=True, Wc=None):
    B = Y.shape[0] // 2
    zn, c = projector_forward(PP, Y, dtype, 2, B, update_running, Wc)
    D = c.D
    zn1, zn2 = zn[:B], zn[B:]
    denom = float(global_batch if global_batch else B)
    cmat = _empty((D, D), torch.float32, like=Y)
    gemm(dtype, 1, 1, D, D, B, zn1, D, zn2, D, cmat, D, alpha=1.0 / denom, out_f32=1)
    if all_reduce is not None:
        all_reduce(cmat)
    coef = (lambd if lambd else 1.0) * scale_loss
    dc = _empty((D, D), N.torch_dtype(dtype), like=Y)
    N.call("barlow_loss", dtype, cmat, D, coef, 2.0 * coef / denom, dc, loss_out)
    if not backward:
        return None
    dzn = _empty((2 * B, D), torch.float32, like=Y)
    gemm(dtype, 0, 0, B, D, D, zn2, D, dc, D, dzn[:B], D, out_f32=1)
    gemm(dtype, 0, 1, B, D, D, zn1, D, dc, D, dzn[B:], D, out_f32=1)
    rows = 2 * B if need_dy2 else (B if need_dy1 else 0)
    return projector_backward(c, PP, G, dzn, rows)


def _harr(ctype, xs):
    import ctypes
    vals = [x.data_ptr() if isinstance(x, torch.Tensor) else x for x in xs]
    return (ctype * len(vals))(*vals)


def _multi_check(*lists):
    for ts in lists:
        for t in ts:
            if t is not None and (not t.is_cuda or not t.is_contiguous()):
                raise RuntimeError("multi-problem launches need contiguous device tensors")


def gemm_multi(ta, tb, M, Nn, Ks, As, ldas, Bs, ldbs, Cs, ldc, alpha=1.0, out_f32=0, atomic=0, ksplit=1):
    import ctypes
    n = len(As)
    _multi_check(As, Bs, Cs)
    Ns = [Nn] * n if isinstance(Nn, int) else list(Nn)
    ldcs = [ldc] * n if isinstance(ldc, int) else list(ldc)
    adr = ctypes.addressof
    arrs = (_harr(ctypes.c_int, Ns), _harr(ctypes.c_int, Ks), _harr(ctypes.c_void_p, As), _harr(ctypes.c_long, ldas),
            _harr(ctypes.c_void_p, Bs), _harr(ctypes.c_long, ldbs), _harr(ctypes.c_void_p, Cs), _harr(ctypes.c_long, ldcs))
    N_, K_, A_, la_, B_, lb_, C_, lc_ = arrs
    if N.PROFILE is not None:
        N.PROFILE_NOTE = float(sum(2.0 * M * nn * kk for nn, kk in zip(Ns, Ks)))
    N.call("gemm_multi", n, ta, tb, M, adr(N_), adr(K_), float(alpha), adr(A_), adr(la_), adr(B_), adr(lb_), adr(C_), adr(lc_),
           out_f32, atomic, ksplit)


def gemm_multi_sgd(ta, tb, M, Nn, Ks, As, ldas, Bs, ldbs, Ps, Moms, Shadows, ldp, hyper, alpha=1.0):
    import ctypes
    n = len(As)
    _multi_check(As, Bs, Ps, Moms, [] if Shadows is None else Shadows)
    Ns = [Nn] * n if isinstance(Nn, int) else list(Nn)
    ldps = [ldp] * n if isinstance(ldp, int) else list(ldp)
    adr = ctypes.addressof
    vp = ctypes.c_void_p
    arrs = (_harr(ctypes.c_int, Ns), _harr(ctypes.c_int, Ks), _harr(vp, As), _harr(ctypes.c_long, ldas), _harr(vp, Bs),
            _harr(ctypes.c_long, ldbs), _harr(vp, Ps), _harr(vp, Moms), _harr(vp, Shadows if Shadows is not None else [None] * n),
            _harr(ctypes.c_long, ldps))
    if N.PROFILE is not None:
        N.PROFILE_NOTE = (float(sum(2.0 * M * nn * kk for nn, kk in zip(Ns, Ks))),
                          float(sum(2.0 * kk * (M + nn) + M * nn * (16.0 + (2.0 if Shadows is not None else 0.0)) for nn, kk in zip(Ns, Ks))))
    lr, mu, wd, gs, gs_dev = hyper
    N.call("gemm_multi_sgd", n, ta, tb, M, adr(arrs[0]), adr(arrs[1]), float(alpha), adr(arrs[2]), adr(arrs[3]), adr(arrs[4]), adr(arrs[5]),
           adr(arrs[6]), adr(arrs[7]), adr(arrs[8]), adr(arrs[9]), float(lr), float(mu), float(wd), float(gs), gs_dev)


def _heads_wgrad_split(D, kmax, M, nh):
    return _ksplit(D, kmax, M, max(256 // nh, 1))


def heads_wgrads_store(D, kins, M, grads_zero=True):
    nh = len(kins)
    return bool(grads_zero) and all(_heads_wgrad_split(D, k, M, nh) == 1 for k in (D, max(kins)))


def barlow_heads_forward_backward(PPs, Gs, Ys, dtype, lambds, scale_losses, loss_outs, update_running=True, backward=True,
                                  Wcs=None, grads_zero=False, dy_ready=None, sgd=None):
    import ctypes
    nh = len(Ys)
    B = Ys[0].shape[0] // 2
    M = 2 * B
    td = N.torch_dtype(dtype)
    dev = Ys[0].device
    W = Wcs if Wcs is not None else [tuple(cast(dtype, PP[f"projector.{i}.weight"]) for i in (0, 3, 6)) for PP in PPs]
    D = W[0][0].shape[0]
    kins = [Y.shape[1] for Y in Ys]
    ad = _ad(dtype)
    if dtype != N.BF16 or ad != N.BF16 or B > 1024 or D % 32:
        raise RuntimeError("grouped Barlow heads: bf16 path with B <= 1024 only")
    H = range(nh)
    vp, fl, adr = ctypes.c_void_p, ctypes.c_float, ctypes.addressof
    new = lambda rows, cols, t: [torch.empty(rows, cols, dtype=t, device=dev) for _ in H]

    def layer(xs, ws, ks, prefix, affine, relu):
        a = new(M, D, td)
        gemm_multi(0, 0, M, D, ks, xs, ks, ws, ks, a, D)
        out, st = new(M, D, td), new(4, 2 * D, torch.float32)
        par = lambda suffix, on=True: _harr(vp, [PP[prefix + suffix] if on else None for PP in PPs])
        arrs = (_harr(vp, a), par(".weight", affine), par(".bias", affine), par(".running_mean", update_running),
                par(".running_var", update_running), _harr(vp, out), _harr(vp, st))
        _multi_check(a, out, st)
        N.call("colbn_train_fwd_multi", nh, ad, adr(arrs[0]), adr(arrs[1]), adr(arrs[2]), adr(arrs[3]), adr(arrs[4]),
               BN_MOMENTUM, BN_EPS, relu, 2, B, D, adr(arrs[5]), adr(arrs[6]))
        return a, st, out
    ycs = [torch.empty(M, k, dtype=torch.bfloat16, device=dev) for k in kins]
    cms = [torch.empty(2, k, dtype=torch.float32, device=dev) for k in kins]
    _multi_check(list(Ys), ycs, cms)
    if any(Y.dtype != torch.float32 or k % 32 for Y, k in zip(Ys, kins)):
        raise RuntimeError("grouped Barlow heads: fp32 inputs with width % 32 == 0")
    arrs = (_harr(vp, list(Ys)), _harr(vp, ycs), _harr(vp, cms), _harr(ctypes.c_int, kins))
    N.call("center_cast_multi", nh, adr(arrs[0]), adr(arrs[1]), adr(arrs[2]), adr(arrs[3]), 2, B)
    a1, st1, h1 = layer(ycs, [W[h][0] for h in H], kins, "projector.1", True, 1)

    def shift_running():
        rms = [PP["projector.1.running_mean"] for PP in PPs]
        w0 = [W[h][0] for h in H]
        _multi_check(w0, rms)
        arrs = (_harr(vp, w0), _harr(vp, cms), _harr(vp, rms), _harr(ctypes.c_int, kins))
        N.call("shift_running_mean_multi", nh, adr(arrs[0]), adr(arrs[1]), adr(arrs[2]), D, adr(arrs[3]), 2, BN_MOMENTUM)
    shift_late = update_running and backward and dy_ready is not None
    if update_running and not shift_late:
        shift_running()
    a2, st2, h2 = layer(h1, [W[h][1] for h in H], [D] * nh, "projector.4", True, 1)
    z, st0, zn = layer(h2, [W[h][2] for h in H], [D] * nh, "bn", False, 0)
    dc = new(D, D, td)
    coefs = [(lambds[h] if lambds[h] else 1.0) * scale_losses[h] for h in H]
    dsc = [2.0 * c / B for c in coefs]
    if all(l.numel() == LOSS_REPLICAS for l in loss_outs) and D % 64 == 0:
        _multi_check([zn[h] for h in H], dc, list(loss_outs))
        arrs = (_harr(ctypes.c_int, [B] * nh), _harr(vp, [zn[h][:B] for h in H]), _harr(ctypes.c_long, [D] * nh),
                _harr(vp, [zn[h][B:] for h in H]), _harr(ctypes.c_long, [D] * nh), _harr(vp, dc), _harr(fl, coefs), _harr(fl, dsc),
                _harr(vp, list(loss_outs)))
        if N.PROFILE is not None:
            N.PROFILE_NOTE = float(nh * 2.0 * D * D * B)
        N.call("gemm_multi_barlow", nh, D, adr(arrs[0]), 1.0 / B, adr(arrs[1]), adr(arrs[2]), adr(arrs[3]), adr(arrs[4]), adr(arrs[5]),
               adr(arrs[6]), adr(arrs[7]), adr(arrs[8]))
    else:
        cm = new(D, D, torch.float32)
        gemm_multi(1, 1, D, D, [B] * nh, [zn[h][:B] for h in H], [D] * nh, [zn[h][B:] for h in H], [D] * nh, cm, D,
                   alpha=1.0 / B, out_f32=1)
        arrs = (_harr(vp, cm), _harr(fl, coefs), _harr(fl, dsc), _harr(vp, dc), _harr(vp, list(loss_outs)))
        _multi_check(list(loss_outs))
        N.call("barlow_loss_multi", nh, adr(arrs[0]), D, adr(arrs[1]), adr(arrs[2]), adr(arrs[3]), adr(arrs[4]))
    if not backward:
        return [None] * nh
    dzn = new(M, D, torch.float32)
    gemm_multi(0, 0, B, D, [D] * nh, [zn[h][B:] for h in H], [D] * nh, dc, [D] * nh, [dzn[h][:B] for h in H], D, out_f32=1)
    gemm_multi(0, 1, B, D, [D] * nh, [zn[h][:B] for h in H], [D] * nh, dc, [D] * nh, [dzn[h][B:] for h in H], D, out_f32=1)

    def bn_bwd(a, dh, st, relu, names):
        out = new(M, D, td)
        grads = lambda k: _harr(vp, [Gs[h][names[k]] if names else None for h in H])
        arrs = (_harr(vp, a), _harr(vp, dh), _harr(vp, st), _harr(vp, out), grads(0), grads(1))
        _multi_check(a, dh, st)
        N.call("colbn_bwd_multi", nh, ad, GD, adr(arrs[0]), adr(arrs[1]), adr(arrs[2]), relu, 2, B, D, adr(arrs[3]),
               adr(arrs[4]), adr(arrs[5]))
        return out

    def wgrad(dys, xs, name, ks):
        split = _heads_wgrad_split(D, max(ks), M, nh)
        if sgd is not None:
            if split != 1 or Wcs is None:
                raise RuntimeError("fused SGD needs unsplit weight gradients and the flat weight shadows")
            li = {"projector.0.weight": 0, "projector.3.weight": 1, "projector.6.weight": 2}[name]
            gemm_multi_sgd(1, 1, D, ks, [M] * nh, dys, [D] * nh, xs, ks, [PPs[h][name] for h in H], [sgd["momentum"][h][name] for h in H],
                           [W[h][li] for h in H], ks, sgd["hyper"])
            return
        gemm_multi(1, 1, D, ks, [M] * nh, dys, [D] * nh, xs, ks, [Gs[h][name] for h in H], ks, out_f32=1,
                   atomic=1 if split > 1 else (0 if grads_zero else 2), ksplit=split)

    def dgrad(dys, ws, Ks, rows):
        out = [torch.empty(rows, k, dtype=torch.float32, device=dev) for k in Ks]
        gemm_multi(0, 1, rows, Ks, [D] * nh, [dy[:rows] for dy in dys], [D] * nh, ws, Ks, out, Ks, out_f32=1)
        return out
    later = []
    defer = (lambda fn: later.append(fn)) if dy_ready is not None else (lambda fn: fn())
    dz = bn_bwd(z, dzn, st0, 0, None)
    defer(lambda: wgrad(dz, h2, "projector.6.weight", [D] * nh))
    dh2 = dgrad(dz, [W[h][2] for h in H], [D] * nh, M)
    da2 = bn_bwd(a2, dh2, st2, 1, ("projector.4.weight", "projector.4.bias"))
    defer(lambda: wgrad(da2, h1, "projector.3.weight", [D] * nh))
    dh1 = dgrad(da2, [W[h][1] for h in H], [D] * nh, M)
    da1 = bn_bwd(a1, dh1, st1, 1, ("projector.1.weight", "projector.1.bias"))
    defer(lambda: wgrad(da1, ycs, "projector.0.weight", kins))
    dy = dgrad(da1, [W[h][0] for h in H], kins, B)
    if dy_ready is not None:
        dy_ready()
    if shift_late:
        shift_running()
    for fn in later:
        fn()
    return dy


def moco_forward_backward(dtype, q, k, queue, queue_shadow, temperature, loss_out, backward=True):
    B, dim = q.shape
    K = queue.shape[1]
    td = N.torch_dtype(dtype)
    qn, kn = _empty((B, dim), td, like=q), _empty((B, dim), td, like=q)
    qn32, kn32 = _empty((B, dim), torch.float32, like=q), _empty((B, dim), torch.float32, like=q)
    qinv, kinv = _empty((B,), torch.float32, like=q), _empty((B,), torch.float32, like=q)
    lpos = _empty((B,), torch.float32, like=q)
    N.call("moco_prep", dtype, q, k, B, dim, 1.0 / temperature, qn, qn32, qinv, kn, kn32, kinv, lpos)
    lse = _empty((B,), torch.float32, like=q)
    dlpos = _empty((B,), torch.float32, like=q)
    Pm = None
    if dtype == N.BF16 and K % 8 == 0 and dim % 8 == 0:
        nslot = (K + 63) // 64
        part = _empty((B, nslot, 2), torch.float32, like=q)
        N.call("moco_logits", 1, qn, queue_shadow, B, K, dim, 1.0 / temperature, part, None, 0.0, None)
        N.call("moco_lse_merge", lpos, part, B, nslot, 1.0 / (B * temperature), lse, loss_out, dlpos)
        if not backward:
            return None, kn32
        Pm = _empty((B, K), td, like=q)
        N.call("moco_logits", 2, qn, queue_shadow, B, K, dim, 1.0 / temperature, None, lse, 1.0 / (B * temperature), Pm)
    else:
        lneg = _empty((B, K), torch.float32, like=q)
        gemm(dtype, 0, 1, B, K, dim, qn, dim, queue_shadow, K, lneg, K, alpha=1.0 / temperature, out_f32=1)
        N.call("moco_ce_fwd", lpos, lneg, B, K, lse, loss_out)
        if not backward:
            return None, kn32
        Pm = _empty((B, K), td, like=q)
        N.call("moco_ce_bwd", dtype, lpos, lneg, lse, B, K, 1.0 / (B * temperature), Pm, dlpos)
    dqn = ARENA.zeros((B, dim), torch.float32, device=q.device)
    gemm(dtype, 0, 0, B, dim, K, Pm, K, queue_shadow, K, dqn, dim, out_f32=1, atomic=1, ksplit=_ksplit(B, dim, K, 256))
    dq = _empty((B, dim), td, like=q)
    N.call("l2norm_bwd", dtype, dqn, dlpos, kn32, qn32, qinv, B, dim, dq)
    return dq, kn32
```

### include/audiossl_hip.h

```cpp
#ifndef AUDIOSSL_HIP_H
#define AUDIOSSL_HIP_H

#include <stdint.h>

#ifdef __cplusplus
extern "C" {
#endif

#define AUDIOSSL_OK 0
#define AUDIOSSL_EINVAL (-1)
#define AUDIOSSL_ELAUNCH (-2)
#define AUDIOSSL_EALIGN (-3)

int audiossl_logmel_fwd(const float* wave, float* out, int B, int L, int T, int n_fft, int hop, int n_mels, int taps,
                        const float* win, const float* tw, const float* melw, const int* mel_start, float eps_pow,
                        float eps_log, int apply_log, void* stream);

int audiossl_fbank_fwd(const float* wave, const int* lens, const int* partner, const float* lam, float* clip_mean,
                       const int* bands, const int* bands_host, float* out, int B, int Lmax, int win_len, int shift, int n_fft, int n_mels,
                       int taps, int T_target, const float* win, const float* tw, const float* melw, const int* mel_start,
                       float preemph, float eps_log, float mean, float std, int skip_norm, int time_major, void* stream);

int audiossl_clip_moments(const float* x, double* mom, int B, int n, void* stream);
int audiossl_runnorm_scan(const double* mom, int B, int n_elem, long long* state_i, float* state_f, float* mu_out,
                          float* sd_out, void* stream);
int audiossl_aug_normalize(const float* x, const float* mu, const float* sd, float* bank, long slot0, int R, int B, int n,
                           void* stream);
int audiossl_aug_views(const float* bank, int R, const int* ip, const float* fp, float* out1, float* out2, int B, int F,
                       int T, int canvas_h, int canvas_w, int log_mix, void* stream);
int audiossl_aug_plan_host(uint32_t* np_key, int* np_pos, uint32_t* py_key, int* py_pos, int B, int F, int T,
                           long long clips_seen, long long* n_entries, int R, int n_memory, int use_mix, double ratio,
                           int use_rrc, double fs_lo, double fs_hi, double ts_lo, double ts_hi, int canvas_h,
                           int canvas_w, int use_spec, int spec_F, int spec_T, int spec_nf, int spec_nt, const int* lens,
                           int unit, int* starts, int* ip, float* fp, int* masks);

int audiossl_resample_sinc(const float* x, float* y, int clips, int n_orig, int n_out, const int* n, const int* off_l,
                           const int* off_r, const double* eta_l, const double* eta_r, const double* win, const double* delta,
                           int nwin, int index_step, void* stream);

int audiossl_pcm_window(const void* pcm, long pcm_bytes, const long long* tab, const long long* tab_host, float* out, int B,
                        int unit, int align, void* stream);

int audiossl_kmix_cluster(const float* views, const float* centroids, int n_views, int F, int T, int K, int* cluster,
                          void* stream);
int audiossl_kmix_apply(const float* views, const float* ring, const int* slot, const float* coef, int n_views, int n,
                        int log_mix, float* out, void* stream);
int audiossl_mask_fill(float* x, const int* tab, int n_img, int max_masks, int F, int T, int zero_fill, void* stream);

int audiossl_conv1_stats(const float* img, int N, int F, int T, const float* w, const float* bias, const float* gamma,
                         const float* beta, float* running_mean, float* running_var, float momentum, float eps,
                         double* mom, float* scale, float* shift, float* save_mean, float* save_rstd, void* stream);
#define AUDIOSSL_CONV1_XL_PARTS 4
int audiossl_conv1_fwd(int dtype, const float* img, int N, int F, int T, const float* w, const float* bias,
                       const float* scale, const float* shift, void* out, float* xl, void* stream);
#define AUDIOSSL_CONV1_MOM_SLOT (17 * 54)
int audiossl_conv1_moments_pair(const float* img_a, const float* img_b, int N, int F, int T, double* mom, void* stream);
int audiossl_conv1_fwd_train(const float* img, int N, int F, int T, double* mom, double count, const float* w, const float* bias,
                             const float* gamma, const float* beta, float* running_mean, float* running_var, float momentum,
                             float eps, float* scale, float* shift, float* save_mean, float* save_rstd, void* out, float* xl,
                             void* stream);
int audiossl_conv1_bwd(int dtype, int conv_dtype, const float* img, int N, int F, int T, const float* w, const float* bias,
                       const float* gamma, const float* scale, const float* shift, const float* mean, const float* rstd,
                       const double* mom, const void* dP, const void* dxl, float* acc, float* dW, float* dbias,
                       float* dgamma, float* dbeta, void* stream);

int audiossl_colstats(int dtype, const void* x, int groups, long M, int C, long ld, int want_sq, double* sum,
                      double* sumsq, void* stream);
int audiossl_bn_finalize(const double* sum, const double* sumsq, int groups, double count, int C, const float* gamma,
                         const float* beta, float* running_mean, float* running_var, float momentum, float eps,
                         float* scale, float* shift, float* save_mean, float* save_rstd, void* stream);
int audiossl_bn_relu_pool_fwd(int dtype, int ydtype, const void* Y, const float* scale, const float* shift, void* P, int N,
                              int Ti, int Fi, void* stream);
int audiossl_bn_relu_pool_train_fwd(int dtype, int ydtype, const void* Y, const double* sum, const double* sumsq, int stat_replicas,
                                    double count, const float* gamma, const float* beta, float* running_mean, float* running_var,
                                    float momentum, float eps, void* P, float* scale, float* shift, float* save_mean, float* save_rstd,
                                    int N, int Ti, int Fi, void* stream);
int audiossl_tmean_fwd(int dtype, int out_f32, const void* P, void* xl, int N, int To, int Fo, void* stream);
int audiossl_tmean3_fwd(int dtype, int out_f32, const void* P1, void* x1, const float* x1_parts, int To1, int Fo1, const void* P2,
                        void* x2, int To2, int Fo2, const void* P3, void* x3, int To3, int Fo3, int N, void* stream);
int audiossl_bn_relu_pool_bwd(int dtype, int ydtype, int gdtype, const void* Y, const void* dP, const void* dxl, const float* scale,
                              const float* shift, const float* mean, const float* rstd, float* stat, void* dY,
                              float* dgamma, float* dbeta, int N, int Ti, int Fi, void* stream);
int audiossl_bn_relu_pool_bwd_p(int dtype, int ydtype, int gdtype, const void* Y, const void* P, const void* dP, const void* dxl,
                                const float* scale, const float* shift, const float* mean, const float* rstd, float* stat, void* dY,
                                float* dgamma, float* dbeta, int N, int Ti, int Fi, void* stream);
int audiossl_conv1_moments(const float* img, int N, int F, int T, double* mom, void* stream);
int audiossl_conv1_finalize(double* mom_totals, const float* w, const float* bias, const float* gamma, const float* beta,
                            float* running_mean, float* running_var, float momentum, float eps, double count, float* scale,
                            float* shift, float* save_mean, float* save_rstd, void* stream);
int audiossl_conv1_bwd_sums(int dtype, int conv_dtype, const float* img, int N, int F, int T, const float* w, const float* bias,
                            const float* gamma, const float* scale, const float* shift, const float* mean, const float* rstd,
                            const double* mom, const void* dP, const void* dxl, float* acc, float* lstat, void* stream);
int audiossl_conv1_bwd_finalize(const float* acc, const double* mom, const float* w, const float* bias, const float* gamma,
                                const float* mean, const float* rstd, double count_global, const float* gstat, float* dW,
                                float* dbias, float* dgamma, float* dbeta, void* stream);
int audiossl_bn_relu_pool_bwd_stats(int dtype, int ydtype, int gdtype, const void* Y, const void* dP, const void* dxl,
                                    const float* scale, const float* shift, const float* mean, const float* rstd, float* stat,
                                    int N, int Ti, int Fi, void* stream);
int audiossl_bn_relu_pool_bwd_apply(int dtype, int ydtype, int gdtype, const void* Y, const void* dP, const void* dxl,
                                    const float* scale, const float* shift, const float* mean, const float* rstd, float* stat,
                                    const float* gstat, double count_global, void* dY, float* dgamma, float* dbeta, int N, int Ti,
                                    int Fi, void* stream);
int audiossl_colbn_bwd_stats(int dtype, int adtype, int gdtype, const void* a, const void* dh, const float* scale,
                             const float* shift, const float* mean, const float* rstd, int relu, int groups, long M, int C,
                             double* tmp, void* stream);
int audiossl_colbn_bwd_apply(int dtype, int adtype, int gdtype, const void* a, const void* dh, const float* scale,
                             const float* shift, const float* mean, const float* rstd, int relu, int groups, long M, int C,
                             const double* sums, double count, void* da, void* stream);
int audiossl_im2col3x3(int dtype, const void* X, void* col, int N, int Ti, int Fi, void* stream);
int audiossl_pack_conv_w(int dtype, const float* W, void* Wf, void* Wd, void* stream);
int audiossl_pack_conv_w2(int dtype, const float* Wa, void* Wfa, void* Wda, const float* Wb, void* Wfb, void* Wdb, void* stream);
int audiossl_unpack_conv_dw(const float* dWp, float* dW, void* stream);

int audiossl_conv3x3_fwd(const void* X, const void* W, const float* bias, void* Y, int out_f32, double* sum,
                         double* sumsq, int stat_replicas, int N, int Ti, int Fi, void* stream);
int audiossl_conv3x3_wgrad(const void* dY, const void* X, float* dWp, float* workspace, long workspace_floats, int N, int Ti,
                           int Fi, void* stream);

int audiossl_gemm(int dtype, int trans_a, int trans_b, int M, int N, int K, float alpha, const void* A, long lda,
                  const void* B, long ldb, void* C, long ldc, const float* bias, int relu, const uint8_t* keep, long ldk,
                  float keep_scale, const void* gate, long ldg, int out_f32, int atomic, int ksplit, const float* resid,
                  long ldr, void* stream);

int audiossl_gemm_dropout(int trans_a, int trans_b, int M, int N, int K, float alpha, const void* A, long lda, const void* B,
                          long ldb, void* C, long ldc, const float* bias, int relu, unsigned long long seed, float p,
                          const long long* counter, float keep_scale, void* stream);

int audiossl_gemm_multi(int count, int trans_a, int trans_b, int M, const int* N, const int* K, float alpha,
                        const void* const* A, const long* lda, const void* const* B, const long* ldb, void* const* C,
                        const long* ldc, int out_f32, int atomic, int ksplit, void* stream);
int audiossl_gemm_multi_sgd(int count, int trans_a, int trans_b, int M, const int* Nv, const int* K, float alpha,
                            const void* const* A, const long* lda, const void* const* B, const long* ldb, float* const* P,
                            float* const* Mom, void* const* Shadow, const long* ldp, float lr, float momentum, float weight_decay,
                            float grad_scale, const float* grad_scale_dev, void* stream);
int audiossl_gemm_multi_barlow(int count, int D, const int* K, float alpha, const void* const* A, const long* lda,
                               const void* const* B, const long* ldb, void* const* dc, const float* coef, const float* dscale,
                               float* const* loss_rep, void* stream);

int audiossl_maxmean_fwd(int dtype, int out_f32, const void* H, void* y, uint8_t* arg, int N, int Tt, int D, void* stream);
int audiossl_maxmean_bwd(int dtype, int gdtype, const void* dy, const uint8_t* arg, const void* H, void* dA, int N, int Tt,
                         int D, void* stream);

int audiossl_colbn_fwd(int dtype, int adtype, const void* a, const float* scale, const float* shift, int relu, void* h,
                       int groups, long M, int C, void* stream);
int audiossl_colbn_train_fwd(int dtype, int adtype, const void* a, const float* gamma, const float* beta,
                             float* running_mean, float* running_var, float momentum, float eps, int relu, int groups,
                             long M, int C, void* h, float* scale, float* shift, float* save_mean, float* save_rstd,
                             void* stream);
int audiossl_colbn_bwd(int dtype, int adtype, int gdtype, const void* a, const void* dh, const float* scale, const float* shift, const float* mean,
                       const float* rstd, int relu, int groups, long M, int C, double* tmp, void* da, float* dgamma,
                       float* dbeta, void* stream);
int audiossl_colbn_train_fwd_multi(int count, int adtype, const void* const* a, const float* const* gamma,
                                   const float* const* beta, float* const* running_mean, float* const* running_var,
                                   float momentum, float eps, int relu, int groups, long M, int C, void* const* h,
                                   float* const* stats, void* stream);
int audiossl_colbn_bwd_multi(int count, int adtype, int gdtype, const void* const* a, const void* const* dh,
                             const float* const* stats, int relu, int groups, long M, int C, void* const* da,
                             float* const* dgamma, float* const* dbeta, void* stream);
int audiossl_barlow_loss_multi(int count, const float* const* c, int D, const float* coef, const float* dscale,
                               void* const* dc, float* const* loss_out, void* stream);
int audiossl_add_d2f(const double* src, float* dst, int n, void* stream);
int audiossl_barlow_loss(int dtype, const float* c, int D, float coef, float dscale, void* dc, float* loss_out,
                         void* stream);

int audiossl_l2norm_fwd(int dtype, const float* q, int B, int D, void* qn, float* qn32, float* inv_norm, void* stream);
int audiossl_moco_prep(int dtype, const float* q, const float* k, int B, int D, float scale, void* qn, float* qn32, float* qinv,
                       void* kn, float* kn32, float* kinv, float* lpos, void* stream);
int audiossl_rowdot(const float* a, const float* b, int B, int D, float scale, float* out, void* stream);
int audiossl_moco_ce_fwd(const float* lpos, const float* lneg, int B, int K, float* lse, float* loss_out, void* stream);
int audiossl_moco_ce_bwd(int dtype, const float* lpos, const float* lneg, const float* lse, int B, int K, float gscale,
                         void* P, float* dlpos, void* stream);
int audiossl_moco_logits(int mode, const void* qn, const void* queue, int B, int K, int dim, float inv_t, float* part,
                         const float* lse, float gscale, void* P, void* stream);
int audiossl_moco_lse_merge(const float* lpos, const float* part, int B, int nslot, float gscale, float* lse,
                            float* loss_out, float* dlpos, void* stream);
int audiossl_l2norm_bwd(int dtype, const float* dqn, const float* dlpos, const float* kn32, const float* qn32,
                        const float* inv_norm, int B, int D, void* dq, void* stream);
int audiossl_enqueue(int dtype, const float* keys, int B, int D, int K, int ptr, long long* ptr_dev, float* queue, void* shadow,
                     void* stream);
int audiossl_ema_update(float* pk, const float* pq, long n, float m, void* shadow, void* stream);

int audiossl_set_prezeroed(int on);
int audiossl_last_kernel(char* name, int capacity);

int audiossl_sgd_momentum(float* p, float* g, float* buf, long n, float lr, float momentum, float weight_decay,
                          int first, float grad_scale, const float* grad_scale_dev, void* shadow_bf16, int zero_grad,
                          void* stream);
int audiossl_sgd_momentum_segments(float* p, float* g, float* buf, const long* segs, int nseg, long max_n, float lr, float momentum,
                                   float weight_decay, int first, float grad_scale, const float* grad_scale_dev, void* shadow_bf16,
                                   int zero_grad, void* stream);
int audiossl_zero_segments(float* g, const long* segs, int nseg, long max_n, void* stream);
int audiossl_cast(int dtype, const float* src, void* dst, long n, void* stream);
int audiossl_cast_back(int dtype, const void* src, float* dst, long n, void* stream);
int audiossl_dropout_mask(uint8_t* keep, long n, unsigned long long seed, float p, const long long* counter, void* stream);
int audiossl_relu_bwd(int dtype, const void* g, const void* h, void* out, long n, void* stream);
int audiossl_bn_eval_affine(const float* gamma, const float* beta, const float* running_mean, const float* running_var,
                            float eps, int C, float* scale, float* shift, void* stream);
int audiossl_axpy(float* y, const float* x, float a, long n, void* stream);
int audiossl_split_bf16(const float* x, void* hi, void* lo, long n, void* stream);
int audiossl_center_cast(const float* y, void* yc, float* cmean, int groups, long M, int C, void* stream);
int audiossl_shift_running_mean(const void* W, const float* cmean, float* running_mean, int D, int K, int groups,
                                float momentum, void* stream);
int audiossl_center_cast_multi(int count, const float* const* y, void* const* yc, float* const* cmean, const int* C, int groups,
                               long M, void* stream);
int audiossl_shift_running_mean_multi(int count, const void* const* W, const float* const* cmean, float* const* running_mean,
                                      int D, const int* K, int groups, float momentum, void* stream);

int audiossl_ntxent_fwd(const float* sim, int N, int B, float* lse, float* loss_out, void* stream);
int audiossl_ntxent_bwd(int dtype, const float* sim, const float* lse, int N, int B, float gscale, void* dsim, void* stream);

int audiossl_row_argmax(const float* dot, long N, int K, long long* assign, void* stream);
int audiossl_kmeans_accumulate(const float* x, const long long* assign, long N, int K, int D, float* sums, int* counts,
                               void* stream);
int audiossl_kmeans_update(const float* sums, const int* counts, int K, int D, float* centroids, void* stream);
int audiossl_kmeans_update_mean(const float* sums, const int* counts, int K, int D, float* centroids, void* stream);
int audiossl_row_sqnorm(const float* x, int rows, int D, float scale, float* out, void* stream);
int audiossl_ce_rows(int dtype, const float* logits, const long long* target, int B, int K, int ignore_index, int* cnt,
                     float* loss_out, void* dlogits, void* stream);

int audiossl_softmax_rows_fwd(const float* x, float* y, int M, int C, void* stream);
int audiossl_softmax_rows_bwd(const float* y, const float* gy, float* gx, int M, int C, void* stream);

int audiossl_attn_fwd(const void* qkv, void* out, float* lse, int B, int S, int H, float scale, void* stream);
int audiossl_attn_bwd(const void* qkv, const void* out, const void* dout, const float* lse, void* dqkv, int B, int S, int H,
                      float scale, void* stream);
int audiossl_layernorm_fwd(const float* x, const float* gamma, const float* beta, void* y, float* y32, float* mean, float* rstd,
                           int M, int C, float eps, void* stream);
int audiossl_layernorm_bwd(const float* dy, const float* x, const float* mean, const float* rstd, const float* gamma,
                           float* dres, float* dgamma, float* dbeta, int M, int C, void* stream);
int audiossl_gelu_fwd(const void* a, void* h, long n, void* stream);
int audiossl_gelu_bwd(const void* a, const void* dh, void* da, long n, void* stream);
int audiossl_patch_unfold(const float* x, void* out, int B, int F, int T, int fstride, int tstride, void* stream);
int audiossl_tile_rows(const float* src, float* out, long rows, int period, int group, float scale, int C, void* stream);
int audiossl_adamw(float* p, const float* g, float* m, float* v, long n, float lr, float beta1, float beta2, float eps,
                   float weight_decay, float grad_scale, const long long* step, void* stream);

int audiossl_mvit_pool_fwd(const void* qkv, int ldq, int col0, const float* w, const float* gamma, const float* beta, float* out,
                           float* z, float* mean, float* rstd, int B, int heads, int d, int H, int W, int Ho, int Wo, int sh, int sw,
                           float eps, void* stream);
int audiossl_mvit_pool_bwd(const void* qkv, int ldq, int col0, const float* w, const float* gamma, const float* dout, const float* z,
                           const float* mean, const float* rstd, float* dz, float* dw, float* dgamma, float* dbeta, void* dqkv, int B,
                           int heads, int d, int H, int W, int Ho, int Wo, int sh, int sw, void* stream);
int audiossl_mvit_attn_fwd(const float* q, const float* k, const float* v, const float* rh, const float* rw, const int* ih,
                           const int* iw, void* out, float* lse, int B, int heads, int d, int qh, int qw, int kh, int kw, int nrh,
                           int nrw, int residual, float scale, void* stream);
int audiossl_mvit_attn_bwd(const float* q, const float* k, const float* v, const float* rh, const float* rw, const int* ih,
                           const int* iw, const void* dout, const float* lse, float* dq, float* dk, float* dv, float* drh, float* drw,
                           int B, int heads, int d, int qh, int qw, int kh, int kw, int nrh, int nrw, int residual, float scale,
                           void* stream);
int audiossl_tokpool_max_fwd(const float* x, float* y, void* arg, int B, int H, int W, int C, int kh, int kw, int sh, int sw,
                             void* stream);
int audiossl_tokpool_max_bwd(const float* dy, const void* arg, float* dx, int B, int H, int W, int C, int kh, int kw, int sh, int sw,
                             void* stream);

int audiossl_lars_step(float* p, const float* g, float* mu, const void* seg, int n_seg, const float* lr, float weight_decay,
                       float momentum, float eta, float grad_scale, double* norms, void* stream);
int audiossl_larc_step(float* p, const float* g, float* mu, const void* seg, int n_seg, float lr, float weight_decay,
                       float momentum, float trust_coefficient, float eps, int clip, float grad_scale, double* norms,
                       void* stream);

#ifdef __cplusplus
}
#endif
#endif
```

Before: 273,900 clips/s.

## Fold BN backward stats into conv dgrad epilogue and fuse stem bwd finalize

The third-block dgrad conv kernel gains an epilogue that computes the BatchNorm-backward sums for the layer below. It reads the pooled activations and the extra dxl gradient while the fp32 data gradient is still in LDS. The second block then runs a new apply-only BN/ReLU/pool backward kernel that skips its own statistics pass. Separately, the stem conv1 backward kernel uses a last-block ticket counter to run the finalize step itself, removing a single-block kernel launch. These changes trade extra register and LDS pressure in the conv kernel, plus a global atomic handshake, for fewer memory passes and launches.

```diff
diff --git a/audio-ssl_amd/csrc/bnpool.hip b/audio-ssl_amd/csrc/bnpool.hip
--- a/audio-ssl_amd/csrc/bnpool.hip
+++ b/audio-ssl_amd/csrc/bnpool.hip
@@ -587,6 +587,29 @@
     return bn_relu_pool_bwd_run(0, dtype, ydtype, gdtype, Y, P, dP, dxl, scale, shift, mean, rstd, stat, nullptr, 0.0, dY, dgamma, dbeta, N,
                                 Ti, Fi, stream);
 }
+extern "C" int audiossl_bn_relu_pool_bwd_apply_folded(int dtype, int ydtype, int gdtype, const void* Y, const void* dP, const void* dxl,
+                                                      const float* scale, const float* shift, const float* mean, const float* rstd,
+                                                      float* stat, void* dY, float* dgamma, float* dbeta, int N, int Ti, int Fi,
+                                                      void* stream) {
+    ASSL_REQUIRE(Y && dP && scale && shift && mean && rstd && stat && dY && dgamma && dbeta);
+    ASSL_REQUIRE(N > 0 && Ti >= 2 && Fi >= 2 && (Fi % 2) == 0 && (dtype == 0 || dtype == 1) && (gdtype == 0 || gdtype == dtype));
+    ASSL_REQUIRE(ydtype == 0 || ydtype == dtype);
+    hipStream_t s = static_cast<hipStream_t>(stream);
+    const long total = (long)N * ((Ti + 1) / 2) * (Fi / 2) * 8;
+    const int grid = ceil_div(total, 256);
+    const float inv_To = 1.f / (float)(Ti / 2);
+    const float inv_count = (float)(1.0 / ((double)N * Ti * Fi));
+#define BWA(TY, TG, TO) hipLaunchKernelGGL((bn_relu_pool_bwd_kernel<TY, true, TG, TO>), dim3(grid), dim3(256), 0, s,                     \
+        static_cast<const TY*>(Y), static_cast<const TG*>(dP), static_cast<const TG*>(dxl), inv_To, scale, shift, mean, rstd, stat, \
+        inv_count, static_cast<TO*>(dY), N, Ti, Fi, 1, dgamma, dbeta)
+    if (dtype == 0) BWA(float, float, float);
+    else if (ydtype == 0 && gdtype == 0) BWA(float, float, bf16);
+    else if (ydtype == 0) BWA(float, bf16, bf16);
+    else if (gdtype == 0) BWA(bf16, float, bf16);
+    else BWA(bf16, bf16, bf16);
+#undef BWA
+    ASSL_LAUNCH_CHECK();
+}
 extern "C" int audiossl_bn_relu_pool_bwd_stats(int dtype, int ydtype, int gdtype, const void* Y, const void* dP, const void* dxl,
                                                const float* scale, const float* shift, const float* mean, const float* rstd,
                                                float* stat, int N, int Ti, int Fi, void* stream) {
diff --git a/audio-ssl_amd/csrc/conv.hip b/audio-ssl_amd/csrc/conv.hip
--- a/audio-ssl_amd/csrc/conv.hip
+++ b/audio-ssl_amd/csrc/conv.hip
@@ -1,4 +1,5 @@
 #include <cstdlib>
+#include <type_traits>
 #include "common.h"
 
 namespace {
@@ -13,6 +14,10 @@
 struct ConvArgs {
     const bf16* X; const bf16* W; const float* bias; bf16* Y; double* sum; double* sumsq;
     int Ti, rows_total, tiles, out_f32, dbg, stat_rep;
+};
+
+struct BnBwdArgs {
+    const bf16* P; const float* dxl; const float *scale, *shift, *mean, *rstd; float* stat; float inv_To;
 };
 
 template <int FI, int PITCH, int NTH = 256>
@@ -187,8 +192,9 @@
     static constexpr int BYTES = ROWS * COLS * 128;
 };
 
-template <int FI, bool STATS, bool F32OUT, int PF = 2>
-__global__ __launch_bounds__(256, 1) void conv3x3_ws_kernel(ConvArgs a) {
+template <int FI, bool STATS, bool F32OUT, int PF = 2, bool BNBWD = false>
+__global__ __launch_bounds__(256, 1) void conv3x3_ws_kernel(ConvArgs a, BnBwdArgs bb) {
+    static_assert(!BNBWD || (F32OUT && !STATS && FI == 16), "the BatchNorm-backward sums ride on the fp32 data gradient of the 16-wide layer");
     using G = WsGeom<FI>;
     constexpr int TT = G::TT, COLS = G::COLS;
     typedef __attribute__((address_space(3))) void* lptr_t;
@@ -271,9 +277,19 @@
 
     constexpr int NS = F32OUT ? 4 : 8;
     float ssum[NS], ssq[NS];
-    if (STATS) {
+    if (STATS || BNBWD) {
 #pragma unroll
         for (int e = 0; e < NS; ++e) { ssum[e] = 0.f; ssq[e] = 0.f; }
+    }
+    float bk1[4], bk0[4];
+    if (BNBWD) {
+#pragma unroll
+        for (int e = 0; e < 4; ++e) {
+            const int c = (lane & 15) * 4 + e;
+            const float sc = bb.scale[c], inv = sc != 0.f ? 1.f / sc : 0.f;
+            bk1[e] = inv * bb.rstd[c];
+            bk0[e] = sc != 0.f ? -(bb.shift[c] * inv + bb.mean[c]) * bb.rstd[c] : 0.f;
+        }
     }
 
     int tile = blockIdx.x, cur = 0;
@@ -356,6 +372,46 @@
                     }
             }
             asm volatile("s_waitcnt lgkmcnt(0)" ::: "memory");
+            if (BNBWD) {
+                auto sums = [&](auto with_dxl) {
+                    constexpr bool DXL = decltype(with_dxl)::value;
+                    const int c = lane & 15;
+#pragma unroll
+                    for (int i = 0; i < 2; ++i) {
+                        const char* const st = stg + i * 32 * OPIX;
+                        const int grow = g0 + (2 * wave + i) * (32 / FI);
+#pragma unroll
+                        for (int hb = 0; hb < 2; ++hb) {
+                            const bool stored = grow + hb < a.rows_total;
+                            const int row = min(grow + hb, a.rows_total - 1);
+                            const bf16* const prow = bb.P + (long)row * (FI * CH) + 4 * lane;
+                            const float* const xrow = DXL ? bb.dxl + (long)(row / a.Ti) * (FI * CH) + 4 * lane : nullptr;
+                            bf16x4 pa[4];
+                            f32x4 gx[4];
+#pragma unroll
+                            for (int k = 0; k < 4; ++k) {
+                                pa[k] = *reinterpret_cast<const bf16x4*>(prow + 256 * k);
+                                if (DXL) gx[k] = *reinterpret_cast<const f32x4*>(xrow + 256 * k);
+                            }
+#pragma unroll
+                            for (int k = 0; k < 4; ++k) {
+                                const int p = (hb * 4 + k) * 4 + (lane >> 4);
+                                const f32x4 v = *reinterpret_cast<const f32x4*>(st + p * 256 + ((c ^ (p & 15)) << 4));
+#pragma unroll
+                                for (int e = 0; e < 4; ++e) {
+                                    float g = v[e];
+                                    if (DXL) g += gx[k][e] * bb.inv_To;
+                                    const float av = (float)pa[k][e];
+                                    const float da = (stored && av > 0.f) ? g : 0.f;
+                                    ssum[e] += da;
+                                    ssq[e] += da * (av * bk1[e] + bk0[e]);
+                                }
+                            }
+                        }
+                    }
+                };
+                if (bb.dxl) sums(std::true_type{}); else sums(std::false_type{});
+            }
 #pragma unroll
             for (int i = 0; i < 2; ++i) {
                 const char* const st = stg + i * 32 * OPIX;
@@ -401,6 +457,24 @@
         __builtin_amdgcn_s_barrier();
     }
     if (rts) rts[2] = __builtin_amdgcn_s_memrealtime();
+    if (BNBWD) {
+#pragma unroll
+        for (int e = 0; e < NS; ++e) {
+            float s = ssum[e], q = ssq[e];
+#pragma unroll
+            for (int o = 64 / NS; o < 64; o <<= 1) { s += __shfl_xor(s, o, 64); q += __shfl_xor(q, o, 64); }
+            if (lane < 64 / NS) {
+                const int co = lane * NS + e;
+                red[(wave * 64 + co) * 2] = s; red[(wave * 64 + co) * 2 + 1] = q;
+            }
+        }
+        __syncthreads();
+        if (threadIdx.x < 128) {
+            const int kind = threadIdx.x >> 6, c = threadIdx.x & 63;
+            const float t = (red[c * 2 + kind] + red[(64 + c) * 2 + kind]) + (red[(128 + c) * 2 + kind] + red[(192 + c) * 2 + kind]);
+            atomicAdd(&bb.stat[128 + (blockIdx.x & 31) * 128 + kind * 64 + c], t);
+        }
+    }
     if (STATS) {
 #pragma unroll
         for (int e = 0; e < NS; ++e) {
@@ -616,7 +690,7 @@
     do {                                                                                                  \
         const size_t lds = 2 * WsGeom<FI_>::BYTES + sizeof(float) * (64 + 4 * 64 * 2) + 4 * 64 * (F32_ ? 256 : 128) + 512; \
         if (!wattr[SLOT]) { if (set_lds(conv3x3_ws_kernel<FI_, ST_, F32_>, lds)) return ASSL_ELAUNCH; wattr[SLOT] = true; } \
-        hipLaunchKernelGGL((conv3x3_ws_kernel<FI_, ST_, F32_>), dim3(grid), dim3(256), lds, s, a);       \
+        hipLaunchKernelGGL((conv3x3_ws_kernel<FI_, ST_, F32_>), dim3(grid), dim3(256), lds, s, a, BnBwdArgs{}); \
     } while (0)
         if (Fi == 32) {
             if (sum && !(conv_dbg & 16)) { if (out_f32) WS_LAUNCH(32, true, true, 0); else WS_LAUNCH(32, true, false, 1); }
@@ -639,6 +713,25 @@
     if (Fi == 32) { if (nw == 8) CONV_LAUNCH(32, 8, 0); else CONV_LAUNCH(32, 4, 1); }
     else          { if (nw == 8) CONV_LAUNCH(16, 8, 2); else CONV_LAUNCH(16, 4, 3); }
 #undef CONV_LAUNCH
+    ASSL_LAUNCH_CHECK();
+}
+
+extern "C" int audiossl_conv3x3_dgrad_bnstats(const void* dY, const void* Wd, void* dPin, const void* P, const float* dxl,
+                                              const float* scale, const float* shift, const float* mean, const float* rstd,
+                                              float* stat, int N, int Ti, int Fi, void* stream) {
+    ASSL_REQUIRE(dY && Wd && dPin && P && scale && shift && mean && rstd && stat && N > 0 && Ti > 0 && Fi == 16);
+    if (!ASSL_ALIGNED16(dY) || !ASSL_ALIGNED16(Wd) || !ASSL_ALIGNED16(dPin) || !ASSL_ALIGNED16(P) || !ASSL_ALIGNED16(dxl)) return ASSL_EALIGN;
+    const long rows_l = (long)N * Ti;
+    ASSL_REQUIRE(rows_l * Fi * 128 < 0x7FFFFF00L);
+    hipStream_t s = static_cast<hipStream_t>(stream);
+    const int rows = (int)rows_l, TT = 256 / 16, tiles = (rows + TT - 1) / TT;
+    ConvArgs a{static_cast<const bf16*>(dY), static_cast<const bf16*>(Wd), nullptr, static_cast<bf16*>(dPin), nullptr, nullptr, Ti, rows, tiles, 1, 0, 1};
+    BnBwdArgs bb{static_cast<const bf16*>(P), dxl, scale, shift, mean, rstd, stat, 1.f / (float)Ti};
+    const int grid = tiles < 256 ? tiles : 256;
+    const size_t lds = 2 * WsGeom<16>::BYTES + sizeof(float) * (64 + 4 * 64 * 2) + 4 * 64 * 256 + 512;
+    static bool attr = false;
+    if (!attr) { if (set_lds(conv3x3_ws_kernel<16, false, true, 2, true>, lds)) return ASSL_ELAUNCH; attr = true; }
+    hipLaunchKernelGGL((conv3x3_ws_kernel<16, false, true, 2, true>), dim3(grid), dim3(256), lds, s, a, bb);
     ASSL_LAUNCH_CHECK();
 }
 
diff --git a/audio-ssl_amd/csrc/conv1.hip b/audio-ssl_amd/csrc/conv1.hip
--- a/audio-ssl_amd/csrc/conv1.hip
+++ b/audio-ssl_amd/csrc/conv1.hip
@@ -1,3 +1,4 @@
+#include <atomic>
 #include <cstdlib>
 #include "common.h"
 
@@ -476,16 +477,56 @@
     }
 }
 
-template <bool SLAB, typename TP>
+template <int NT, bool SC1>
+__device__ __forceinline__ void stem_bwd_finalize(double* s11, const float* acc, const double* __restrict__ mom,
+                                                  const float* __restrict__ w, const float* __restrict__ bias,
+                                                  const float* __restrict__ gamma, const float* __restrict__ mean,
+                                                  const float* __restrict__ rstd, double count, float* dW, float* dgamma,
+                                                  float* dbeta, const float* __restrict__ gstat, float* lstat) {
+    for (int i = threadIdx.x; i < 704; i += NT) {
+        double t = 0.0;
+        for (int r = 0; r < 32; ++r)
+            t += (double)(SC1 ? __hip_atomic_load(const_cast<float*>(acc) + r * 704 + i, __ATOMIC_RELAXED, __HIP_MEMORY_SCOPE_AGENT)
+                              : acc[r * 704 + i]);
+        s11[i] = t;
+    }
+    __syncthreads();
+    if (lstat) {
+        for (int i = threadIdx.x; i < 64; i += NT) { lstat[i] = (float)s11[i * 11 + 9]; lstat[64 + i] = (float)s11[i * 11 + 10]; }
+        return;
+    }
+    for (int i = threadIdx.x; i < 576; i += NT) {
+        const int c = i / 9, t = i - c * 9;
+        const double db = gstat ? (double)gstat[c] : s11[c * 11 + 9], dg = gstat ? (double)gstat[64 + c] : s11[c * 11 + 10];
+        const double rs = rstd[c], mu = mean[c], gm = gamma[c];
+        double wS2 = 0.0;
+        for (int a = 0; a < 9; ++a) wS2 += (double)w[c * 9 + a] * mom[9 + (a <= t ? tri(a, t) : tri(t, a))];
+        const double yhat_x = rs * (wS2 + ((double)bias[c] - mu) * mom[t]);
+        const double v = gm * rs * (s11[c * 11 + t] - db / count * mom[t] - dg / count * yhat_x);
+        dW[c * 9 + t] += (float)v;
+    }
+    for (int i = threadIdx.x; i < 64; i += NT) {
+        dgamma[i] += (float)s11[i * 11 + 10];
+        dbeta[i] += (float)s11[i * 11 + 9];
+    }
+}
+
+constexpr int BWD_TICKETS = 256;
+__device__ unsigned int g_conv1_bwd_done[BWD_TICKETS];
+struct StemFin {
+    const double* mom; const float* gamma; double count; float *dW, *dgamma, *dbeta; int ticket;
+};
+
+template <bool SLAB, typename TP, bool FIN = false>
 __global__ __launch_bounds__(256, 3) void conv1_bwd_mfma_kernel(const float* __restrict__ img, const float* __restrict__ w,
                                                              const float* __restrict__ bias, const float* __restrict__ scale,
                                                              const float* __restrict__ shift, const float* __restrict__ mean,
                                                              const float* __restrict__ rstd, const TP* __restrict__ dP,
                                                              const float* __restrict__ dxl, float inv_To, float* __restrict__ accg,
-                                                             int N, int F, int T) {
+                                                             int N, int F, int T, StemFin fin) {
     extern __shared__ __attribute__((aligned(1024))) float dyn[];
     float* const patch = dyn + (SLAB ? 2 * 2048 : 0);
-    __shared__ float red[4][64][11];
+    __shared__ __attribute__((aligned(16))) float red[4][64][11];
     const int lane = threadIdx.x & 63, wv = threadIdx.x >> 6, half = lane >> 5, l31 = lane & 31;
     const int To = T / 2, Fo = F / 2;
     Vec8<bf16> wb[2];
@@ -627,6 +668,28 @@
         const int c = i / 11, k = i - c * 11;
         atomicAdd(&accg[(blockIdx.x & 31) * 704 + i], red[0][c][k] + red[1][c][k] + red[2][c][k] + red[3][c][k]);
     }
+    if constexpr (FIN) {
+        __shared__ int last_s;
+        unsigned int* const done = &g_conv1_bwd_done[fin.ticket];
+        asm volatile("s_waitcnt vmcnt(0)" ::: "memory");
+        __syncthreads();
+        if (threadIdx.x == 0) {
+            __builtin_amdgcn_fence(__ATOMIC_RELEASE, "agent");
+            asm volatile("s_waitcnt vmcnt(0)" ::: "memory");
+            const unsigned int prev = __hip_atomic_fetch_add(done, 1u, __ATOMIC_RELAXED, __HIP_MEMORY_SCOPE_AGENT);
+            const int last = prev == gridDim.x - 1;
+            if (last) {
+                __builtin_amdgcn_fence(__ATOMIC_ACQUIRE, "agent");
+                asm volatile("s_waitcnt vmcnt(0)" ::: "memory");
+            }
+            last_s = last;
+        }
+        __syncthreads();
+        if (!last_s) return;
+        stem_bwd_finalize<256, true>(reinterpret_cast<double*>(&red[0][0][0]), accg, fin.mom, w, bias, fin.gamma, mean, rstd, fin.count,
+                                     fin.dW, fin.dgamma, fin.dbeta, nullptr, nullptr);
+        if (threadIdx.x == 0) __hip_atomic_store(done, 0u, __ATOMIC_RELAXED, __HIP_MEMORY_SCOPE_AGENT);
+    }
 }
 
 __global__ __launch_bounds__(704) void conv1_bwd_finalize_kernel(const float* __restrict__ acc, const double* __restrict__ mom,
@@ -635,31 +698,7 @@
                                           const float* __restrict__ rstd, double count, float* dW, float* dbias,
                                           float* dgamma, float* dbeta, const float* __restrict__ gstat, float* lstat) {
     __shared__ double s11[704];
-    const int i = threadIdx.x;
-    if (i < 704) {
-        double t = 0.0;
-        for (int r = 0; r < 32; ++r) t += (double)acc[r * 704 + i];
-        s11[i] = t;
-    }
-    __syncthreads();
-    if (lstat) {
-        if (i < 64) { lstat[i] = (float)s11[i * 11 + 9]; lstat[64 + i] = (float)s11[i * 11 + 10]; }
-        return;
-    }
-    if (i < 576) {
-        const int c = i / 9, t = i - c * 9;
-        const double db = gstat ? (double)gstat[c] : s11[c * 11 + 9], dg = gstat ? (double)gstat[64 + c] : s11[c * 11 + 10];
-        const double rs = rstd[c], mu = mean[c], gm = gamma[c];
-        double wS2 = 0.0;
-        for (int a = 0; a < 9; ++a) wS2 += (double)w[c * 9 + a] * mom[9 + (a <= t ? tri(a, t) : tri(t, a))];
-        const double yhat_x = rs * (wS2 + ((double)bias[c] - mu) * mom[t]);
-        const double v = gm * rs * (s11[c * 11 + t] - db / count * mom[t] - dg / count * yhat_x);
-        dW[c * 9 + t] += (float)v;
-    }
-    if (i < 64) {
-        dgamma[i] += (float)s11[i * 11 + 10];
-        dbeta[i] += (float)s11[i * 11 + 9];
-    }
+    stem_bwd_finalize<704, false>(s11, acc, mom, w, bias, gamma, mean, rstd, count, dW, dgamma, dbeta, gstat, lstat);
     (void)dbias;
 }
 
@@ -768,8 +807,9 @@
 static int conv1_bwd_main(int dtype, int conv_dtype, const float* img, int N, int F, int T, const float* w, const float* bias,
                                   const float* gamma, const float* scale, const float* shift, const float* mean,
                                   const float* rstd, const double* mom, const void* dP, const void* dxl, float* acc,
-                                  void* stream) {
+                                  void* stream, const StemFin* fin = nullptr) {
     ASSL_REQUIRE(img && w && bias && gamma && scale && shift && mean && rstd && mom && dP && acc);
+    ASSL_REQUIRE(!fin || conv_dtype == 1);
     ASSL_REQUIRE(N > 0 && F >= 2 && F <= 64 && T >= 2 && (F % 2) == 0 && (dtype == 0 || dtype == 1));
     hipStream_t s = static_cast<hipStream_t>(stream);
     ASSL_ZERO(acc, sizeof(float) * 32 * 64 * 11, s);
@@ -777,18 +817,17 @@
     const int grid = min(N * (T / 2), bwd_grid);
     const size_t lds = sizeof(float) * (F + 2) * 4;
     const float inv_To = 1.f / (float)(T / 2);
-    if (conv_dtype == 1 && F == 64 && dtype == 0)
-        hipLaunchKernelGGL((conv1_bwd_mfma_kernel<true, float>), dim3(grid), dim3(256), lds + 2 * 2048 * sizeof(float), s, img, w, bias, scale,
-                           shift, mean, rstd, static_cast<const float*>(dP), static_cast<const float*>(dxl), inv_To, acc, N, F, T);
-    else if (conv_dtype == 1 && F == 64)
-        hipLaunchKernelGGL((conv1_bwd_mfma_kernel<true, bf16>), dim3(grid), dim3(256), lds + 2 * 2048 * sizeof(float), s, img, w, bias, scale,
-                           shift, mean, rstd, static_cast<const bf16*>(dP), static_cast<const float*>(dxl), inv_To, acc, N, F, T);
-    else if (conv_dtype == 1 && dtype == 0)
-        hipLaunchKernelGGL((conv1_bwd_mfma_kernel<false, float>), dim3(grid), dim3(256), lds, s, img, w, bias, scale, shift, mean, rstd,
-                           static_cast<const float*>(dP), static_cast<const float*>(dxl), inv_To, acc, N, F, T);
-    else if (conv_dtype == 1)
-        hipLaunchKernelGGL((conv1_bwd_mfma_kernel<false, bf16>), dim3(grid), dim3(256), lds, s, img, w, bias, scale, shift, mean, rstd,
-                           static_cast<const bf16*>(dP), static_cast<const float*>(dxl), inv_To, acc, N, F, T);
+#define BWD_MFMA(SLAB_, TP_, FIN_)                                                                                           \
+    hipLaunchKernelGGL((conv1_bwd_mfma_kernel<SLAB_, TP_, FIN_>), dim3(grid), dim3(256), lds + (SLAB_ ? 2 * 2048 * sizeof(float) : 0), s, \
+                       img, w, bias, scale, shift, mean, rstd, static_cast<const TP_*>(dP), static_cast<const float*>(dxl), inv_To, acc, \
+                       N, F, T, FIN_ ? *fin : StemFin{})
+#define BWD_MFMA2(SLAB_, TP_) do { if (fin) BWD_MFMA(SLAB_, TP_, true); else BWD_MFMA(SLAB_, TP_, false); } while (0)
+    if (conv_dtype == 1 && F == 64 && dtype == 0) BWD_MFMA2(true, float);
+    else if (conv_dtype == 1 && F == 64) BWD_MFMA2(true, bf16);
+    else if (conv_dtype == 1 && dtype == 0) BWD_MFMA2(false, float);
+    else if (conv_dtype == 1) BWD_MFMA2(false, bf16);
+#undef BWD_MFMA2
+#undef BWD_MFMA
     else if (dtype == 0)
         hipLaunchKernelGGL(conv1_bwd_kernel<float>, dim3(grid), dim3(256), lds, s, img, w, bias, scale, shift, mean, rstd,
                            static_cast<const float*>(dP), static_cast<const float*>(dxl), inv_To, acc, N, F, T);
@@ -803,6 +842,14 @@
                                   const float* rstd, const double* mom, const void* dP, const void* dxl, float* acc,
                                   float* dW, float* dbias, float* dgamma, float* dbeta, void* stream) {
     ASSL_REQUIRE(dW && dgamma && dbeta);
+    const char* const fused_env = getenv("AUDIOSSL_CONV1_BWD_FUSED");
+    if (conv_dtype == 1 && !(fused_env && atoi(fused_env) == 0)) {
+        static std::atomic<unsigned int> next_ticket{0};
+        const StemFin fin{mom, gamma, (double)N * F * T, dW, dgamma, dbeta, (int)(next_ticket.fetch_add(1) % BWD_TICKETS)};
+        const int rc = conv1_bwd_main(dtype, conv_dtype, img, N, F, T, w, bias, gamma, scale, shift, mean, rstd, mom, dP, dxl, acc, stream, &fin);
+        if (rc != ASSL_OK) return rc;
+        ASSL_LAUNCH_CHECK();
+    }
     const int rc = conv1_bwd_main(dtype, conv_dtype, img, N, F, T, w, bias, gamma, scale, shift, mean, rstd, mom, dP, dxl, acc, stream);
     if (rc != ASSL_OK) return rc;
     hipLaunchKernelGGL(conv1_bwd_finalize_kernel, dim3(1), dim3(704), 0, static_cast<hipStream_t>(stream), acc, mom, w, bias, gamma, mean,
diff --git a/audio-ssl_amd/src/engine.py b/audio-ssl_amd/src/engine.py
--- a/audio-ssl_amd/src/engine.py
+++ b/audio-ssl_amd/src/engine.py
@@ -265,6 +265,7 @@
 STAT_REPLICAS = 8
 LOSS_REPLICAS = 32
 _BN_STATS_P = os.environ.get("AUDIOSSL_BN_STATS_P", "1") != "0"
+_BN_STATS_EPI = os.environ.get("AUDIOSSL_BN_STATS_EPI", "1") != "0"
 _DP1_BF16 = os.environ.get("AUDIOSSL_DP1_BF16", "1") != "0"
 
 
@@ -419,14 +420,21 @@
     return x1, x2, x3, c.H2.view(Nimg, T3, d), c
 
 
-def _conv_block_bwd(dtype, Y, dP, dxl, st, Nimg, Ti, Fi, Pin, Wd, G_w, G_gamma, G_beta, need_dx, col, keep, dx_bf16=False, Pout=None):
+def _bn_stats_from_pooled(dtype, Pout):
+    return SYNC_BN is None and Pout is not None and _BN_STATS_P and Pout.dtype == N.torch_dtype(dtype)
+
+
+def _conv_block_bwd(dtype, Y, dP, dxl, st, Nimg, Ti, Fi, Pin, Wd, G_w, G_gamma, G_beta, need_dx, col, keep, dx_bf16=False, Pout=None,
+                    stat_filled=None, below=None):
     td = N.torch_dtype(dtype)
     scale, shift, mean, rstd = st
     M = Nimg * Ti * Fi
     dY = torch.empty((M, 64), dtype=td, device=Y.device)
-    stat = ARENA.scratch((33 * 128,), torch.float32, Y)
+    stat = stat_filled if stat_filled is not None else ARENA.scratch((33 * 128,), torch.float32, Y)
     yd = N.F32 if Y.dtype == torch.float32 else dtype
-    if SYNC_BN is None and Pout is not None and _BN_STATS_P and Pout.dtype == td:
+    if stat_filled is not None:
+        N.call("bn_relu_pool_bwd_apply_folded", dtype, yd, GD, Y, dP, dxl, scale, shift, mean, rstd, stat, dY, G_gamma, G_beta, Nimg, Ti, Fi)
+    elif SYNC_BN is None and Pout is not None and _BN_STATS_P and Pout.dtype == td:
         N.call("bn_relu_pool_bwd_p", dtype, yd, GD, Y, Pout, dP, dxl, scale, shift, mean, rstd, stat, dY, G_gamma, G_beta, Nimg, Ti, Fi)
     elif SYNC_BN is None:
         N.call("bn_relu_pool_bwd", dtype, yd, GD, Y, dP, dxl, scale, shift, mean, rstd, stat, dY, G_gamma, G_beta, Nimg, Ti, Fi)
@@ -453,7 +461,10 @@
         return None
     dx_bf16 = dx_bf16 and fused
     dPin = _empty((Nimg, Ti, Fi, 64), torch.bfloat16 if dx_bf16 else torch.float32, like=Y)
-    if fused:
+    if below is not None:
+        assert fused and not dx_bf16 and Fi == 16
+        N.call("conv3x3_dgrad_bnstats", dY, Wd, dPin, Pin, below[0], *below[1], below[2], Nimg, Ti, Fi)
+    elif fused:
         N.call("conv3x3_fwd", dY, Wd, None, dPin, 0 if dx_bf16 else 1, None, None, 1, Nimg, Ti, Fi)
     else:
         N.call("im2col3x3", dtype, dY, col, Nimg, Ti, Fi)
@@ -485,11 +496,16 @@
         dx1, dx2, dx3 = dx_late()
     col = _col_buffer(dtype, Nimg, T1, F1, c.H2)
     keep = []
+    stat2 = None
+    if (_BN_STATS_EPI and dtype == N.BF16 and not HP and F2 == 16 and GD == N.F32 and _bn_stats_from_pooled(dtype, c.P3)
+            and _bn_stats_from_pooled(dtype, c.P2) and (dx2 is None or (dx2.dtype == torch.float32 and dx2.is_contiguous()))):
+        stat2 = ARENA.zeros((33 * 128,), torch.float32, device=dev)
     dP2 = _conv_block_bwd(dtype, c.Y3, dP3, dx3, c.st3, Nimg, T2, F2, c.P2, c.W3d, G["features_3.0.weight"],
-                          G["features_3.1.weight"], G["features_3.1.bias"], True, col, keep, Pout=c.P3)
+                          G["features_3.1.weight"], G["features_3.1.bias"], True, col, keep, Pout=c.P3,
+                          below=None if stat2 is None else (dx2, c.st2, stat2))
     dP1 = _conv_block_bwd(dtype, c.Y2, dP2, dx2, c.st2, Nimg, T1, F1, c.P1, c.W2d, G["features_2.0.weight"],
                           G["features_2.1.weight"], G["features_2.1.bias"], True, col, keep, dx_bf16=bool(c.stem_mfma) and _DP1_BF16,
-                          Pout=c.P2)
+                          Pout=c.P2, stat_filled=stat2)
     gd1 = N.BF16 if dP1.dtype == torch.bfloat16 else GD
     acc = ARENA.scratch((32 * 64 * 11,), torch.float32, c.H2)
     P = c.P
diff --git a/include/audiossl_hip.h b/include/audiossl_hip.h
--- a/include/audiossl_hip.h
+++ b/include/audiossl_hip.h
@@ -84,6 +84,9 @@
 int audiossl_bn_relu_pool_bwd_p(int dtype, int ydtype, int gdtype, const void* Y, const void* P, const void* dP, const void* dxl,
                                 const float* scale, const float* shift, const float* mean, const float* rstd, float* stat, void* dY,
                                 float* dgamma, float* dbeta, int N, int Ti, int Fi, void* stream);
+int audiossl_bn_relu_pool_bwd_apply_folded(int dtype, int ydtype, int gdtype, const void* Y, const void* dP, const void* dxl,
+                                           const float* scale, const float* shift, const float* mean, const float* rstd, float* stat,
+                                           void* dY, float* dgamma, float* dbeta, int N, int Ti, int Fi, void* stream);
 int audiossl_conv1_moments(const float* img, int N, int F, int T, double* mom, void* stream);
 int audiossl_conv1_finalize(double* mom_totals, const float* w, const float* bias, const float* gamma, const float* beta,
                             float* running_mean, float* running_var, float momentum, float eps, double count, float* scale,
@@ -114,6 +117,9 @@
 
 int audiossl_conv3x3_fwd(const void* X, const void* W, const float* bias, void* Y, int out_f32, double* sum,
                          double* sumsq, int stat_replicas, int N, int Ti, int Fi, void* stream);
+int audiossl_conv3x3_dgrad_bnstats(const void* dY, const void* Wd, void* dPin, const void* P, const float* dxl, const float* scale,
+                                   const float* shift, const float* mean, const float* rstd, float* stat, int N, int Ti, int Fi,
+                                   void* stream);
 int audiossl_conv3x3_wgrad(const void* dY, const void* X, float* dWp, float* workspace, long workspace_floats, int N, int Ti,
                            int Fi, void* stream);
 
```

New measurement: 271,100 clips/s. 0.99x the previous value.
